# yimin-pan/hair-gs

Measured on AMD Instinct MI355X. Metric: train_iters_per_sec, higher is better.
Workload: dtype f32; 1 GPU; north_star: 100000 strand-Gaussians, 32 views @ 1920x1080, 1 view(s)/GPU/optimizer step (1 views/step), RGB+mask+orientation raster fwd+bwd + L1/DSSIM/mask/orientation/smoothness losses + Adam; gaussians=100000, views=32, width=1920, height=1080, parallelism=view-parallel x1, views_per_optimizer_step=1, forward_mode=async-capacity, dispatch=hip-graph replay, optimizer_steps_per_graph_launch=8, adam_in_backward_lanes=True, raster_passes_per_iter=1

## Files before the change

### hair-gs_amd/csrc/hgs_api.hip

```cpp
#include <stdarg.h>
#include <stdio.h>
#include <string.h>

#include "hgs_common.h"
#include "hgs_prologue.h"

static thread_local char g_err[512] = "";

void hgs_set_error(const char* fmt, ...) {
  va_list ap;
  va_start(ap, fmt);
  vsnprintf(g_err, sizeof(g_err), fmt, ap);
  va_end(ap);
}

#include <vector>
namespace {
struct ProfRec { hipEvent_t a, b; int id; };
bool g_prof_on = false;
std::vector<ProfRec> g_prof_log;
std::vector<hipEvent_t> g_prof_pool;
hipEvent_t g_prof_open = nullptr;
int g_prof_open_id = -1;
const char* kKernelNames[HGS_K_COUNT] = {"preprocess_fwd_kernel", "scan_kernel", "scatter_kernel", "sort_tiles_kernel",
                                         "blend_fwd_kernel", "blend_bwd_kernel", "preprocess_bwd_kernel", "dist2_kernels",
                                         "ssim_l1_fwd_kernel", "ssim_l1_bwd_kernel", "strand_fwd_kernel",
                                         "strand_bwd_kernel", "ori_fwd_kernel", "ori_bwd_kernel", "adam_kernel",
                                         "smooth_kernels", "head_tail_kernel", "misc_kernels"};
hipEvent_t prof_event() {
  if (!g_prof_pool.empty()) { hipEvent_t e = g_prof_pool.back(); g_prof_pool.pop_back(); return e; }
  hipEvent_t e = nullptr;
  (void)hipEventCreate(&e);
  return e;
}
}
void hgs_prof_begin(hipStream_t s, int kernel_id) {
  if (!g_prof_on) return;
  g_prof_open = prof_event();
  g_prof_open_id = kernel_id;
  (void)hipEventRecord(g_prof_open, s);
}
void hgs_prof_end(hipStream_t s) {
  if (!g_prof_on || !g_prof_open) return;
  hipEvent_t b = prof_event();
  (void)hipEventRecord(b, s);
  g_prof_log.push_back({g_prof_open, b, g_prof_open_id});
  g_prof_open = nullptr;
}

__global__ __launch_bounds__(256) void hgs_zero_kernel(uint32_t* __restrict__ p, size_t n_words) {
  const size_t stride = (size_t)gridDim.x * 256;
  for (size_t i = (size_t)blockIdx.x * 256 + threadIdx.x; i < n_words; i += stride) p[i] = 0u;
}
int hgs_zero_async(hipStream_t s, void* ptr, size_t bytes) {
  if (bytes == 0) return 0;
  if (((size_t)ptr & 3) || (bytes & 3)) { hgs_set_error("hgs_zero_async: pointer/size must be 4-byte multiples"); return 1; }
  const size_t n = bytes / 4;
  const unsigned blocks = (unsigned)((n + 255) / 256 < 2048 ? (n + 255) / 256 : 2048);
  hipLaunchKernelGGL(hgs_zero_kernel, dim3(blocks), dim3(256), 0, s, (uint32_t*)ptr, n);
  HGS_CHECK_LAUNCH();
  return 0;
}

__global__ __launch_bounds__(256) void select_view_kernel(HgsPrologue p) { hgs_prologue_block(p, blockIdx.x, gridDim.x); }

struct HgsViewQueueArgs { int v[HGS_VIEW_QUEUE_MAX]; };
__global__ void set_view_queue_kernel(int* __restrict__ queue, int n, HgsViewQueueArgs a, float lr, float* __restrict__ lr_slot) {
  if ((int)threadIdx.x < n) queue[threadIdx.x] = a.v[threadIdx.x];
  if (threadIdx.x == 0 && lr_slot) *lr_slot = lr;
}
__global__ void select_view_queued_kernel(const HgsViewTargets* __restrict__ table, int n_views,
                                          const int* __restrict__ view_index, HgsViewTargets* __restrict__ slot,
                                          const float* __restrict__ lr_slot, float* __restrict__ lr_dst) {
  int view = *view_index;
  if (view < 0 || view >= n_views) view = 0;
  const uint32_t* src = (const uint32_t*)(table + view);
  uint32_t* dst = (uint32_t*)slot;
  for (int i = threadIdx.x; i < (int)(sizeof(HgsViewTargets) / 4); i += 64) dst[i] = src[i];
  if (threadIdx.x == 0 && lr_dst && lr_slot) *lr_dst = *lr_slot;
}

__global__ __launch_bounds__(256) void densify_stats_kernel(int P, const int* __restrict__ radii,
                                                            const float* __restrict__ g, int stride,
                                                            float* __restrict__ max_radii, float* __restrict__ accum,
                                                            float* __restrict__ denom) {
  const int i = blockIdx.x * 256 + threadIdx.x;
  if (i >= P) return;
  const int r = radii[i];
  if (r <= 0) return;
  max_radii[i] = fmaxf(max_radii[i], (float)r);
  const float gx = g[(size_t)i * stride], gy = g[(size_t)i * stride + 1];
  accum[i] += sqrtf(gx * gx + gy * gy);
  denom[i] += 1.f;
}

static int check_aligned(const void* p, const char* what) {
  if (!p || ((size_t)p & (HGS_ALIGN - 1))) {
    hgs_set_error("%s must be a non-null %d-byte aligned device pointer", what, HGS_ALIGN);
    return 1;
  }
  return 0;
}

extern "C" {

int hgs_abi_version(void) { return HGS_ABI_VERSION; }
const char* hgs_last_error(void) { return g_err; }

size_t hgs_geom_bytes(int P) { HgsGeom g; return hgs_geom_carve(nullptr, (size_t)(P > 0 ? P : 0), g, nullptr); }
size_t hgs_image_bytes(int W, int H) { HgsImage im; return hgs_image_carve(nullptr, (size_t)W, (size_t)H, im, nullptr); }
size_t hgs_binning_bytes(int R, int channels) {
  if (channels != 3 && channels != 7) return 0;
  HgsBinning b;
  return hgs_binning_carve(nullptr, (size_t)(R > 0 ? R : 0), b, nullptr, channels);
}
size_t hgs_backward_scratch_bytes(int P, int R, int channels) {
  const size_t p = (size_t)(P > 0 ? P : 0), r = (size_t)(R > 0 ? R : 0);
  if (channels == 3) return hgs_align_up(r * HGS_INST_GRAD_FLOATS * sizeof(float)) + HGS_ALIGN;
  if (channels == 7) return hgs_align_up(r * 16 * sizeof(float)) + hgs_align_up(hgs_row_reduce_floats(p, r) * sizeof(float)) + HGS_ALIGN;
  return 0;
}
int hgs_geom_layout(int P, size_t* offsets) { HgsGeom g; hgs_geom_carve(nullptr, (size_t)P, g, offsets); return 0; }
int hgs_image_zero_range(int W, int H, size_t* offset, size_t* bytes) {
  if (W <= 0 || H <= 0 || !offset || !bytes) { hgs_set_error("hgs_image_zero_range: bad arguments"); return 1; }
  HgsImage im;
  hgs_image_carve(nullptr, (size_t)W, (size_t)H, im, nullptr);
  const size_t T = (size_t)((W + HGS_TILE - 1) / HGS_TILE) * ((H + HGS_TILE - 1) / HGS_TILE);
  *offset = (size_t)((char*)im.tile_count - (char*)nullptr);
  *bytes = hgs_image_zero_words(T) * sizeof(uint32_t);
  return 0;
}
int hgs_image_layout(int W, int H, size_t* offsets) { HgsImage im; hgs_image_carve(nullptr, (size_t)W, (size_t)H, im, offsets); return 0; }
int hgs_binning_layout(int R, size_t* offsets) { HgsBinning b; hgs_binning_carve(nullptr, (size_t)R, b, offsets); return 0; }

static_assert(HGS_FUSED_PREPROCESS_MAX_TILES == HGS_FUSED_SCAN_MAX_T, "include/hgs.h states the scatter kernel's scan limit");
struct HairSrc {
  const float* endpoints; const long long* pairs; const float* width; float f; const float* opacity_raw; const float* mask_raw;
  float* xyz; float* scale; float* quat; float* opacity; float* extra4; const HgsStrandFusion* fusion;
  const float* scaling_raw; const float* rotation_raw;
};
static int forward_preprocess_impl(void* stream, int P, int D, int M, int W, int H, const float* means3D, const float* shs,
                                   const float* colors_precomp, const float* opacities, const float* scales,
                                   float scale_modifier, const float* rotations, const float* cov3D_precomp,
                                   const float* viewmatrix, const float* projmatrix, const float* campos, float tan_fovx,
                                   float tan_fovy, int prefiltered, void* geom_buf, void* image_buf, int* radii,
                                   int* num_rendered_host, unsigned int* max_rendered, const HairSrc* hair);

int hgs_forward_preprocess(void* stream, int P, int D, int M, int W, int H, const float* means3D, const float* shs,
                           const float* colors_precomp, const float* opacities, const float* scales,
                           float scale_modifier, const float* rotations, const float* cov3D_precomp,
                           const float* viewmatrix, const float* projmatrix, const float* campos, float tan_fovx,
                           float tan_fovy, int prefiltered, void* geom_buf, void* image_buf, int* radii,
                           int* num_rendered_host, unsigned int* max_rendered) {
  return forward_preprocess_impl(stream, P, D, M, W, H, means3D, shs, colors_precomp, opacities, scales, scale_modifier,
                                 rotations, cov3D_precomp, viewmatrix, projmatrix, campos, tan_fovx, tan_fovy, prefiltered,
                                 geom_buf, image_buf, radii, num_rendered_host, max_rendered, nullptr);
}

int hgs_hair_forward_preprocess(void* stream, int P, int D, int M, int W, int H, const float* endpoints,
                                const long long* endpoint_pairs, const float* width, float dist_to_scale_factor,
                                const float* opacity_raw, const float* mask_raw, const float* shs, float* xyz, float* scale,
                                float* quat, float* opacity, float* extra4, const float* viewmatrix, const float* projmatrix,
                                const float* campos, float tan_fovx, float tan_fovy, int flags, void* geom_buf,
                                void* image_buf, int* radii, unsigned int* max_rendered, const HgsStrandFusion* fusion) {
  if (P > 0 && (!endpoints || !endpoint_pairs || !width || !opacity_raw || !mask_raw || !xyz || !scale || !quat || !opacity ||
                !extra4 || ((size_t)quat & 15) || ((size_t)extra4 & 15))) {
    hgs_set_error("hgs_hair_forward_preprocess: null (or, quat / extra4, not 16-byte aligned) argument");
    return 1;
  }
  if (!max_rendered) { hgs_set_error("hgs_hair_forward_preprocess: capacity mode only (max_rendered must be given)"); return 1; }
  const HairSrc hair = {endpoints, endpoint_pairs, width, dist_to_scale_factor, opacity_raw, mask_raw, xyz, scale, quat, opacity,
                        extra4, fusion, nullptr, nullptr};
  return forward_preprocess_impl(stream, P, D, M, W, H, xyz, shs, nullptr, opacity, scale, 1.f, quat, nullptr, viewmatrix,
                                 projmatrix, campos, tan_fovx, tan_fovy, flags, geom_buf, image_buf, radii, nullptr,
                                 max_rendered, &hair);
}

int hgs_cloud_forward_preprocess(void* stream, int P, int D, int M, int W, int H, const float* means3D, const float* scaling_raw,
                                 const float* rotation_raw, const float* opacity_raw, const float* mask_raw, const float* shs,
                                 float* scale, float* quat, float* opacity, float* extra4, const float* viewmatrix,
                                 const float* projmatrix, const float* campos, float tan_fovx, float tan_fovy, int flags,
                                 void* geom_buf, void* image_buf, int* radii, unsigned int* max_rendered,
                                 const HgsStrandFusion* fusion) {
  if (P > 0 && (!means3D || !scaling_raw || !rotation_raw || !opacity_raw || !mask_raw || !scale || !quat || !opacity || !extra4 ||
                ((size_t)rotation_raw & 15) || ((size_t)quat & 15) || ((size_t)extra4 & 15))) {
    hgs_set_error("hgs_cloud_forward_preprocess: null (or, rotation_raw / quat / extra4, not 16-byte aligned) argument");
    return 1;
  }
  if (!max_rendered) { hgs_set_error("hgs_cloud_forward_preprocess: capacity mode only (max_rendered must be given)"); return 1; }
  const HairSrc cloud = {nullptr, nullptr, nullptr, 0.f, opacity_raw, mask_raw, nullptr, scale, quat, opacity, extra4, fusion,
                         scaling_raw, rotation_raw};
  return forward_preprocess_impl(stream, P, D, M, W, H, means3D, shs, nullptr, opacity, scale, 1.f, quat, nullptr, viewmatrix,
                                 projmatrix, campos, tan_fovx, tan_fovy, flags, geom_buf, image_buf, radii, nullptr,
                                 max_rendered, &cloud);
}

static int forward_preprocess_impl(void* stream, int P, int D, int M, int W, int H, const float* means3D, const float* shs,
                                   const float* colors_precomp, const float* opacities, const float* scales,
                                   float scale_modifier, const float* rotations, const float* cov3D_precomp,
                                   const float* viewmatrix, const float* projmatrix, const float* campos, float tan_fovx,
                                   float tan_fovy, int prefiltered, void* geom_buf, void* image_buf, int* radii,
                                   int* num_rendered_host, unsigned int* max_rendered, const HairSrc* hair) {
  hipStream_t s = (hipStream_t)stream;
  if (P < 0 || W <= 0 || H <= 0) { hgs_set_error("bad sizes P=%d W=%d H=%d", P, W, H); return 1; }
  if ((size_t)((W + HGS_TILE - 1) / HGS_TILE) * ((H + HGS_TILE - 1) / HGS_TILE) > HGS_MAX_TILES) { hgs_set_error("%dx%d: more than 2^24 tiles", W, H); return 1; }
  if ((unsigned)P > HGS_MAX_GAUSSIANS) { hgs_set_error("P=%d: at most 2^28 Gaussians per pass (instance key layout)", P); return 1; }
  if (D < 0 || D > 3) { hgs_set_error("sh degree %d unsupported (0..3)", D); return 1; }
  if (check_aligned(image_buf, "image_buf")) return 1;
  HgsImage im;
  hgs_image_carve((char*)image_buf, (size_t)W, (size_t)H, im, nullptr);
  const int T = ((W + HGS_TILE - 1) / HGS_TILE) * ((H + HGS_TILE - 1) / HGS_TILE);
  if (!(prefiltered & HGS_IMAGE_PREZEROED) &&
      hgs_zero_async(s, im.tile_count, hgs_image_zero_words((size_t)T) * sizeof(uint32_t))) return 1;
  const HgsPrologue* rider = (hair && hair->fusion && hair->fusion->prologue.table) ? &hair->fusion->prologue : nullptr;
  if (rider && (!rider->slot || rider->view < 0 || ((size_t)rider->zero_ptr & 3) || (rider->zero_bytes & 3) ||
                (rider->zero_bytes && !rider->zero_ptr))) {
    hgs_set_error("hgs_hair/cloud_forward_preprocess: bad prologue group");
    return 1;
  }
  if (hair && T > HGS_FUSED_SCAN_MAX_T) {
    hgs_set_error("hgs_hair_forward_preprocess: %d tiles, at most %d (the tile counters are cleared by the scatter kernel's scan)", T, HGS_FUSED_SCAN_MAX_T);
    return 1;
  }
  if (P == 0 && rider &&
      hgs_iteration_prologue(stream, rider->table, rider->view, rider->slot, rider->lr, rider->lr_dst, rider->zero_ptr, rider->zero_bytes,
                             rider->adam_prep)) return 1;
  if (P == 0) {
    HgsGeom none = {};
    if (hgs_launch_scan(s, 0, T, none, im, nullptr)) return 1;
    if (num_rendered_host) { HGS_CHECK_HIP(hipStreamSynchronize(s)); *num_rendered_host = 0; }
    return 0;
  }
  if (check_aligned(geom_buf, "geom_buf")) return 1;
  if (!means3D || !opacities || !viewmatrix || !projmatrix || !campos || !radii) { hgs_set_error("null required input"); return 1; }
  if ((shs == nullptr) == (colors_precomp == nullptr)) { hgs_set_error("provide exactly one of shs / colors_precomp"); return 1; }
  if (((scales == nullptr) || (rotations == nullptr)) == (cov3D_precomp == nullptr)) {
    hgs_set_error("provide exactly one of (scales, rotations) / cov3D_precomp"); return 1;
  }
  if (shs && M < (D + 1) * (D + 1)) { hgs_set_error("M=%d SH coefficients < (D+1)^2 for D=%d", M, D); return 1; }
  HgsGeom g;
  hgs_geom_carve((char*)geom_buf, (size_t)P, g, nullptr);
  HgsFwdArgs a;
  a.P = P; a.D = D; a.M = M; a.W = W; a.H = H;
  a.means3D = means3D; a.shs = shs; a.colors_precomp = colors_precomp; a.opacities = opacities; a.scales = scales;
  a.rotations = rotations; a.cov3D_precomp = cov3D_precomp; a.viewmatrix = viewmatrix; a.projmatrix = projmatrix;
  a.campos = campos; a.scale_modifier = scale_modifier; a.tan_fovx = tan_fovx; a.tan_fovy = tan_fovy;
  a.prefiltered = prefiltered & 1;
  a.tile_cull = (prefiltered & HGS_TILE_CULL) ? 1 : 0;
  a.row_runs = (prefiltered & HGS_COUNT_ROW_RUNS) ? 1 : 0;
  const bool fused_scan = !num_rendered_host && max_rendered && T <= HGS_FUSED_SCAN_MAX_T && P <= HGS_FUSED_SCAN_MAX_P;
  a.fused_scan_ptr = fused_scan ? (unsigned long long)(size_t)max_rendered : 0ull;
  if (hair) {
    if (!fused_scan) { hgs_set_error("hgs_hair_forward_preprocess: the scan must be the scatter kernel's (sizes beyond its limits)"); return 1; }
    HgsStrandFusion fu = hair->fusion ? *hair->fusion : HgsStrandFusion{};
    if (!(fu.smooth_pairs && fu.n_smooth > 0 && fu.smooth_partials)) fu.n_smooth = 0;
    if (hair->scaling_raw) {
      if (hgs_launch_cloud_preprocess_fwd(s, a, g, im, radii, hair->scaling_raw, hair->rotation_raw, hair->opacity_raw,
                                          hair->mask_raw, hair->scale, hair->quat, hair->opacity, hair->extra4, fu.prologue)) return 1;
    } else if (hgs_launch_hair_preprocess_fwd(s, a, g, im, radii, hair->endpoints, hair->pairs, hair->width, hair->f,
                                              hair->opacity_raw, hair->mask_raw, hair->xyz, hair->scale, hair->quat,
                                              hair->opacity, hair->extra4, fu)) return 1;
  } else if (hgs_launch_preprocess_fwd(s, a, g, im, radii)) return 1;
  if (!fused_scan && hgs_launch_scan(s, P, T, g, im, max_rendered, a.row_runs)) return 1;
  if (num_rendered_host) {
    uint32_t r = 0;
    HGS_CHECK_HIP(hipMemcpyAsync(&r, im.status, sizeof(uint32_t), hipMemcpyDeviceToHost, s));
    HGS_CHECK_HIP(hipStreamSynchronize(s));
    *num_rendered_host = (int)r;
  }
  return 0;
}

int hgs_forward_render(void* stream, int P, int W, int H, int R_capacity, int n_extra, int flags, const float* bg,
                       const float* colors_precomp, const float* extra, void* geom_buf, void* binning_buf, void* image_buf,
                       float* out_color) {
  hipStream_t s = (hipStream_t)stream;
  if (check_aligned(image_buf, "image_buf")) return 1;
  if (!bg || !out_color) { hgs_set_error("null bg/out_color"); return 1; }
  if (n_extra != 0 && n_extra != 4) { hgs_set_error("n_extra must be 0 or 4 (got %d)", n_extra); return 1; }
  if (n_extra && P > 0 && (!extra || ((size_t)extra & 15))) { hgs_set_error("extra colours must be a 16-byte aligned [P,4] array"); return 1; }
  if ((flags & HGS_RECORDS_PACKED) && (flags & HGS_RECORDS_LAZY)) { hgs_set_error("HGS_RECORDS_PACKED and HGS_RECORDS_LAZY exclude each other"); return 1; }
  const int channels = 3 + n_extra;
  HgsImage im;
  hgs_image_carve((char*)image_buf, (size_t)W, (size_t)H, im, nullptr);
  HgsGeom g = {};
  HgsBinning b = {};
  if (P > 0) {
    if (check_aligned(geom_buf, "geom_buf")) return 1;
    hgs_geom_carve((char*)geom_buf, (size_t)P, g, nullptr);
    if (R_capacity > 0) {
      if (check_aligned(binning_buf, "binning_buf")) return 1;
      hgs_binning_carve((char*)binning_buf, (size_t)R_capacity, b, nullptr, channels);
      b.grec = g.grec;
      const long long tiles = (long long)((W + HGS_TILE - 1) / HGS_TILE) * ((H + HGS_TILE - 1) / HGS_TILE);
      b.lazy = (flags & HGS_RECORDS_LAZY) ? 1 : (flags & HGS_RECORDS_PACKED) ? 0 : ((long long)R_capacity >= (long long)HGS_LAZY_MIN_MEAN_LIST * tiles ? 1 : 0);
    }
    const float* feat = colors_precomp ? colors_precomp : g.rgb;
    if (hgs_launch_scatter(s, P, W, H, R_capacity > 0 ? R_capacity : 0, feat, extra, n_extra, g, im, b)) return 1;
  }
  if (hgs_launch_sort_tiles(s, W, H, R_capacity > 0 ? R_capacity : 0, n_extra, g, im, b)) return 1;
  return hgs_launch_blend_fwd(s, W, H, R_capacity > 0 ? R_capacity : 0, channels, bg, im, b, out_color);
}

#define HGS_RR_AUTO_RATIO 8

static int backward_impl(void* stream, int P, int D, int M, int R, int W, int H, int n_extra, int flags, const float* bg,
                         const float* means3D, const float* shs, const float* colors_precomp, const float* scales,
                         float scale_modifier, const float* rotations, const float* cov3D_precomp, const float* viewmatrix,
                         const float* projmatrix, const float* campos, float tan_fovx, float tan_fovy, const int* radii,
                         const void* geom_buf, const void* binning_buf, const void* image_buf,
                         const float* const* dL_dpix_planes, void* scratch, float* dL_dextra, float* dL_dmeans2D, float* dL_dconic,
                         float* dL_dopacity, float* dL_dcolors, float* dL_dmeans3D, float* dL_dcov3D, float* dL_dsh,
                         float* dL_dscales, float* dL_drotations, const HgsParamBackward* pb) {
  hipStream_t s = (hipStream_t)stream;
  if (n_extra != 0 && n_extra != 4) { hgs_set_error("n_extra must be 0 or 4 (got %d)", n_extra); return 1; }
  if ((flags & HGS_ROWS_INLINE) && (flags & HGS_ROWS_REDUCE)) { hgs_set_error("HGS_ROWS_INLINE and HGS_ROWS_REDUCE exclude each other"); return 1; }
  if (P == 0) return 0;
  if (check_aligned(geom_buf, "geom_buf") || check_aligned(image_buf, "image_buf")) return 1;
  if (!dL_dpix_planes || !radii || !means3D || !viewmatrix || !projmatrix || !campos) { hgs_set_error("null required input"); return 1; }
  for (int k = 0; k < 3 + n_extra; k++)
    if (!dL_dpix_planes[k]) { hgs_set_error("null dL_dpix plane %d", k); return 1; }
  if (!pb && (!dL_dmeans2D || !dL_dconic || !dL_dopacity || !dL_dcolors || !dL_dmeans3D || !dL_dcov3D || !dL_dscales ||
              !dL_drotations || (n_extra && !dL_dextra))) { hgs_set_error("null gradient output"); return 1; }
  if (shs && !dL_dsh) { hgs_set_error("null gradient output"); return 1; }
  const int channels = 3 + n_extra;
  HgsGeom g;
  HgsImage im;
  HgsBinning b = {};
  hgs_geom_carve((char*)geom_buf, (size_t)P, g, nullptr);
  hgs_image_carve((char*)image_buf, (size_t)W, (size_t)H, im, nullptr);
  float* inst_grad = nullptr;
  const bool reduce_rows = n_extra && R > 0 &&
                           ((flags & HGS_ROWS_REDUCE) || (!(flags & HGS_ROWS_INLINE) && (long long)R >= (long long)HGS_RR_AUTO_RATIO * P));
  if (R > 0) {
    if (check_aligned(binning_buf, "binning_buf") || check_aligned(scratch, "scratch")) return 1;
    hgs_binning_carve((char*)binning_buf, (size_t)R, b, nullptr, channels);
    b.grec = g.grec;
    inst_grad = (float*)scratch;
    if (hgs_launch_blend_bwd(s, W, H, R, channels, bg, im, b, dL_dpix_planes, inst_grad, reduce_rows ? 1 : 0)) return 1;
  }
  float *row_sums = nullptr, *row_partials = nullptr;
  if (reduce_rows) {
    row_sums = (float*)((char*)scratch + hgs_align_up((size_t)R * 16 * sizeof(float)));
    row_partials = row_sums + (size_t)P * 16;
    if (hgs_launch_row_reduce(s, P, R, inst_grad, im.status, row_sums, row_partials)) return 1;
  }
  HgsBwdArgs a;
  a.P = P; a.D = D; a.M = M; a.W = W; a.H = H;
  a.means3D = means3D; a.shs = shs; a.colors_precomp = colors_precomp; a.scales = scales; a.rotations = rotations;
  a.cov3D_precomp = cov3D_precomp; a.viewmatrix = viewmatrix; a.projmatrix = projmatrix; a.campos = campos;
  a.scale_modifier = scale_modifier; a.tan_fovx = tan_fovx; a.tan_fovy = tan_fovy; a.radii = radii;
  a.dL_dmeans2D = dL_dmeans2D; a.dL_dconic = dL_dconic; a.dL_dopacity = dL_dopacity; a.dL_dcolors = dL_dcolors;
  a.dL_dmeans3D = dL_dmeans3D; a.dL_dcov3D = dL_dcov3D; a.dL_dsh = dL_dsh; a.dL_dscales = dL_dscales;
  a.dL_drotations = dL_drotations;
  a.n_extra = n_extra; a.dL_dextra = dL_dextra;
  a.row_sums = row_sums; a.row_partials = row_partials;
  return hgs_launch_preprocess_bwd(s, a, g, b, inst_grad, R, im.status, pb);
}

size_t hgs_param_backward_bytes(void) { return sizeof(HgsParamBackward); }
size_t hgs_adam_prep_bytes(void) { return sizeof(HgsAdamPrep); }
size_t hgs_adam_inline_bytes(void) { return sizeof(HgsAdamInline); }
static int check_adam_inline(const HgsAdamInline& a, int n_slots, const char* who) {
  for (int k = 0; k < 6; k++) {
    const HgsAdamSlot& sl = a.slot[k];
    if (!sl.p) continue;
    if (k >= n_slots || !sl.m || !sl.v || !sl.coef) { hgs_set_error("%s: incomplete Adam slot %d", who, k); return 1; }
  }
  return 0;
}
int hgs_backward_multi_params(void* stream, int P, int D, int M, int R, int W, int H, int flags, const float* bg7,
                              const float* means3D, const float* shs, const float* scales, const float* rotations,
                              const float* viewmatrix, const float* projmatrix, const float* campos, float tan_fovx,
                              float tan_fovy, const int* radii, const void* geom_buf, const void* binning_buf, const void* image_buf,
                              const float* const* dL_dpix_planes7, void* scratch, float* dL_dsh, const HgsParamBackward* pb) {
  if (!pb || (pb->kind != HGS_PARAMS_HAIR && pb->kind != HGS_PARAMS_CLOUD)) { hgs_set_error("hgs_backward_multi_params: params->kind must be HGS_PARAMS_HAIR or HGS_PARAMS_CLOUD"); return 1; }
  if (P == 0 && pb->head_tail.out) { hgs_set_error("hgs_backward_multi_params: a deferred loss-head tail needs a launch (P > 0)"); return 1; }
  if (P == 0) return 0;
  if (!shs || !scales || !rotations || !dL_dsh) { hgs_set_error("hgs_backward_multi_params: SH colours and (scales, rotations) are required"); return 1; }
  if (!pb->extra4 || !pb->d_opacity_raw || !pb->d_mask_raw || ((size_t)pb->extra4 & 15)) { hgs_set_error("hgs_backward_multi_params: null (or, extra4, unaligned) argument in params"); return 1; }
  if ((pb->max_radii2D || pb->grad_accum || pb->denom) && !(pb->max_radii2D && pb->grad_accum && pb->denom)) {
    hgs_set_error("hgs_backward_multi_params: incomplete statistics group");
    return 1;
  }
  if (pb->kind == HGS_PARAMS_HAIR) {
    if (!pb->endpoints || !pb->endpoint_pairs || !pb->seg_contrib || !pb->d_width || ((size_t)pb->seg_contrib & 15)) {
      hgs_set_error("hgs_backward_multi_params: null (or, seg_contrib, unaligned) hair argument"); return 1;
    }
    if (pb->head_tail.out) { hgs_set_error("hgs_backward_multi_params: the strand model's deferred tail rides in hgs_hair_endpoint_gather"); return 1; }
  } else if (!pb->rotation_raw || !pb->d_means3D || !pb->d_scaling_raw || !pb->d_rotation_raw || ((size_t)pb->rotation_raw & 15) ||
             ((size_t)pb->d_rotation_raw & 15)) {
    hgs_set_error("hgs_backward_multi_params: null (or, rotation_raw / d_rotation_raw, unaligned) cloud argument"); return 1;
  }
  if (check_adam_inline(pb->adam, pb->kind == HGS_PARAMS_HAIR ? 4 : 6, "hgs_backward_multi_params")) return 1;
  HgsParamBackward p = *pb;
  return backward_impl(stream, P, D, M, R, W, H, 4, flags, bg7, means3D, shs, nullptr, scales, 1.f, rotations, nullptr, viewmatrix,
                       projmatrix, campos, tan_fovx, tan_fovy, radii, geom_buf, binning_buf, image_buf, dL_dpix_planes7, scratch,
                       nullptr, p.dL_dmeans2D_rgb, nullptr, nullptr, nullptr, nullptr, nullptr, dL_dsh, nullptr, nullptr, &p);
}

int hgs_backward(void* stream, int P, int D, int M, int R, int W, int H, int n_extra, int flags, const float* bg,
                 const float* means3D, const float* shs, const float* colors_precomp, const float* scales, float scale_modifier,
                 const float* rotations, const float* cov3D_precomp, const float* viewmatrix, const float* projmatrix,
                 const float* campos, float tan_fovx, float tan_fovy, const int* radii, const void* geom_buf,
                 const void* binning_buf, const void* image_buf, const float* const* dL_dpix_planes, void* scratch,
                 float* dL_dextra, float* dL_dmeans2D, float* dL_dconic, float* dL_dopacity, float* dL_dcolors,
                 float* dL_dmeans3D, float* dL_dcov3D, float* dL_dsh, float* dL_dscales, float* dL_drotations) {
  return backward_impl(stream, P, D, M, R, W, H, n_extra, flags, bg, means3D, shs, colors_precomp, scales, scale_modifier,
                       rotations, cov3D_precomp, viewmatrix, projmatrix, campos, tan_fovx, tan_fovy, radii, geom_buf, binning_buf,
                       image_buf, dL_dpix_planes, scratch, dL_dextra, dL_dmeans2D, dL_dconic, dL_dopacity, dL_dcolors,
                       dL_dmeans3D, dL_dcov3D, dL_dsh, dL_dscales, dL_drotations, nullptr);
}

int hgs_mark_visible(void* stream, int P, const float* means3D, const float* viewmatrix, const float* projmatrix,
                     uint8_t* present) {
  (void)projmatrix;
  if (P == 0) return 0;
  if (!means3D || !viewmatrix || !present) { hgs_set_error("null input"); return 1; }
  return hgs_launch_mark_visible((hipStream_t)stream, P, means3D, viewmatrix, present);
}

__global__ void hgs_empty_kernel() {}
static float g_prof_bracket_ms = -1.f;
static int prof_calibrate() {
  hipEvent_t a = nullptr, b = nullptr;
  HGS_CHECK_HIP(hipEventCreate(&a));
  HGS_CHECK_HIP(hipEventCreate(&b));
  float best1 = 1e9f, best2 = 1e9f;
  for (int rep = 0; rep < 24; rep++) {
    for (int n = 1; n <= 2; n++) {
      HGS_CHECK_HIP(hipDeviceSynchronize());
      HGS_CHECK_HIP(hipEventRecord(a, nullptr));
      for (int k = 0; k < n; k++) hipLaunchKernelGGL(hgs_empty_kernel, dim3(1), dim3(64), 0, nullptr);
      HGS_CHECK_HIP(hipEventRecord(b, nullptr));
      HGS_CHECK_HIP(hipEventSynchronize(b));
      float ms = 0.f;
      HGS_CHECK_HIP(hipEventElapsedTime(&ms, a, b));
      if (rep >= 4) { if (n == 1) best1 = ms < best1 ? ms : best1; else best2 = ms < best2 ? ms : best2; }
    }
  }
  (void)hipEventDestroy(a);
  (void)hipEventDestroy(b);
  const float kernel = best2 - best1 > 0.f ? best2 - best1 : 0.f;
  g_prof_bracket_ms = best1 - kernel > 0.f ? best1 - kernel : 0.f;
  return 0;
}
int hgs_prof_enable(int on) {
  if (on && g_prof_bracket_ms < 0.f && prof_calibrate()) return 1;
  g_prof_on = on != 0;
  return 0;
}
double hgs_prof_bracket_overhead_ms(void) { return g_prof_bracket_ms < 0.f ? 0.0 : (double)g_prof_bracket_ms; }
const char* hgs_prof_kernel_name(int id) { return (id >= 0 && id < HGS_K_COUNT) ? kKernelNames[id] : ""; }
int hgs_prof_collect(double* total_ms, long long* launches) {
  for (auto& r : g_prof_log) {
    HGS_CHECK_HIP(hipEventSynchronize(r.b));
    float ms = 0.f;
    HGS_CHECK_HIP(hipEventElapsedTime(&ms, r.a, r.b));
    ms -= g_prof_bracket_ms > 0.f ? g_prof_bracket_ms : 0.f;
    if (ms < 0.f) ms = 0.f;
    if (total_ms) total_ms[r.id] += ms;
    if (launches) launches[r.id] += 1;
    g_prof_pool.push_back(r.a);
    g_prof_pool.push_back(r.b);
  }
  g_prof_log.clear();
  return 0;
}

size_t hgs_dist2_scratch_bytes(int P) { return hgs_dist2_scratch(P > 0 ? P : 0); }
int hgs_dist2(void* stream, int P, const float* points, float* out, void* scratch, size_t scratch_bytes) {
  if (P == 0) return 0;
  if (!points || !out) { hgs_set_error("null input"); return 1; }
  return hgs_launch_dist2((hipStream_t)stream, P, points, out, scratch, scratch_bytes);
}

size_t hgs_view_targets_bytes(void) { return sizeof(HgsViewTargets); }
size_t hgs_head_params_bytes(void) { return sizeof(HgsHeadParams); }
size_t hgs_strand_fusion_bytes(void) { return sizeof(HgsStrandFusion); }

int hgs_iteration_prologue(void* stream, const HgsViewTargets* table, int view, HgsViewTargets* slot, float lr, float* lr_dst,
                           void* zero_ptr, size_t zero_bytes, const HgsAdamPrep* adam_prep) {
  if (!table || !slot || view < 0) { hgs_set_error("hgs_iteration_prologue: bad arguments"); return 1; }
  if (((size_t)zero_ptr & 3) || (zero_bytes & 3) || (zero_bytes && !zero_ptr)) { hgs_set_error("hgs_iteration_prologue: zero range must be 4-byte multiples"); return 1; }
  hipStream_t s = (hipStream_t)stream;
  const HgsPrologue p = {table, view, slot, lr, lr_dst, zero_ptr, zero_bytes, adam_prep};
  {
    HgsProfScope _prof(s, HGS_K_MISC);
    hipLaunchKernelGGL(select_view_kernel, dim3(hgs_prologue_blocks(zero_bytes / 4)), dim3(256), 0, s, p);
  }
  HGS_CHECK_LAUNCH();
  return 0;
}
int hgs_select_view(void* stream, const HgsViewTargets* table, int view, HgsViewTargets* slot, float lr, float* lr_dst) {
  return hgs_iteration_prologue(stream, table, view, slot, lr, lr_dst, nullptr, 0, nullptr);
}

int hgs_graph_find_prologues(void* graph, int max_nodes, void** nodes_out, float* lr_out, int* n_out) {
  if (!graph || !nodes_out || !n_out || max_nodes < 1) { hgs_set_error("hgs_graph_find_prologues: bad arguments"); return 1; }
  size_t n = 0;
  HGS_CHECK_HIP(hipGraphGetNodes((hipGraph_t)graph, nullptr, &n));
  std::vector<hipGraphNode_t> nodes(n);
  if (n) HGS_CHECK_HIP(hipGraphGetNodes((hipGraph_t)graph, nodes.data(), &n));
  int count = 0;
  for (size_t i = 0; i < n; i++) {
    hipGraphNodeType t;
    HGS_CHECK_HIP(hipGraphNodeGetType(nodes[i], &t));
    if (t != hipGraphNodeTypeKernel) continue;
    hipKernelNodeParams kp;
    HGS_CHECK_HIP(hipGraphKernelNodeGetParams(nodes[i], &kp));
    int n_params = 1;
    if (kp.func != (void*)select_view_kernel && !hgs_strands_prologue_kernel(kp.func, &n_params) &&
        !hgs_preprocess_prologue_kernel(kp.func, &n_params)) continue;
    if (!kp.kernelParams) continue;
    const HgsPrologue* pro = (const HgsPrologue*)kp.kernelParams[n_params - 1];
    if (!pro->table) continue;
    if (count < max_nodes) {
      nodes_out[count] = (void*)nodes[i];
      if (lr_out) lr_out[count] = pro->lr;
    }
    count++;
  }
  *n_out = count;
  if (count > max_nodes) { hgs_set_error("hgs_graph_find_prologues: the graph holds %d prologue launches (room for %d)", count, max_nodes); return 1; }
  return 0;
}
int hgs_graph_find_prologue(void* graph, void** node_out) {
  int n = 0;
  if (!node_out) { hgs_set_error("hgs_graph_find_prologue: bad arguments"); return 1; }
  if (hgs_graph_find_prologues(graph, 1, node_out, nullptr, &n)) return 1;
  if (n != 1) { hgs_set_error("hgs_graph_find_prologue: the graph holds %d prologue launches (need exactly 1)", n); return 1; }
  return 0;
}
int hgs_graph_set_prologue(void* graph_exec, void* node, const HgsViewTargets* table, int view, HgsViewTargets* slot, float lr,
                           float* lr_dst, void* zero_ptr, size_t zero_bytes) {
  if (!graph_exec || !node || !table || !slot || view < 0) { hgs_set_error("hgs_graph_set_prologue: bad arguments"); return 1; }
  hipKernelNodeParams kp;
  HGS_CHECK_HIP(hipGraphKernelNodeGetParams((hipGraphNode_t)node, &kp));
  int n_params = 1;
  if (kp.func != (void*)select_view_kernel && !hgs_strands_prologue_kernel(kp.func, &n_params) &&
      !hgs_preprocess_prologue_kernel(kp.func, &n_params)) {
    hgs_set_error("hgs_graph_set_prologue: not a prologue node");
    return 1;
  }
  if (((const HgsPrologue*)kp.kernelParams[n_params - 1])->zero_bytes != zero_bytes) {
    hgs_set_error("hgs_graph_set_prologue: the zero range differs from the captured one");
    return 1;
  }
  HgsPrologue p = {table, view, slot, lr, lr_dst, zero_ptr, zero_bytes,
                   ((const HgsPrologue*)kp.kernelParams[n_params - 1])->adam_prep};
  void* args[32];
  for (int i = 0; i < n_params - 1; i++) args[i] = kp.kernelParams[i];
  args[n_params - 1] = &p;
  kp.kernelParams = args;
  kp.extra = nullptr;
  HGS_CHECK_HIP(hipGraphExecKernelNodeSetParams((hipGraphExec_t)graph_exec, (hipGraphNode_t)node, &kp));
  return 0;
}

int hgs_set_view_queue(void* stream, int* queue, int n, const int* views_host, float lr, float* lr_slot) {
  if (!queue || !views_host || n < 1 || n > HGS_VIEW_QUEUE_MAX) { hgs_set_error("hgs_set_view_queue: bad arguments (1 <= n <= %d)", HGS_VIEW_QUEUE_MAX); return 1; }
  HgsViewQueueArgs a = {};
  for (int i = 0; i < n; i++) a.v[i] = views_host[i];
  hipStream_t s = (hipStream_t)stream;
  {
    HgsProfScope _prof(s, HGS_K_MISC);
    hipLaunchKernelGGL(set_view_queue_kernel, dim3(1), dim3(64), 0, s, queue, n, a, lr, lr_slot);
  }
  HGS_CHECK_LAUNCH();
  return 0;
}

int hgs_select_view_queued(void* stream, const HgsViewTargets* table, int n_views, const int* view_index,
                           HgsViewTargets* slot, const float* lr_slot, float* lr_dst) {
  if (!table || !slot || !view_index || n_views < 1) { hgs_set_error("hgs_select_view_queued: bad arguments"); return 1; }
  hipStream_t s = (hipStream_t)stream;
  {
    HgsProfScope _prof(s, HGS_K_MISC);
    hipLaunchKernelGGL(select_view_queued_kernel, dim3(1), dim3(64), 0, s, table, n_views, view_index, slot, lr_slot, lr_dst);
  }
  HGS_CHECK_LAUNCH();
  return 0;
}

int hgs_densify_stats(void* stream, int P, const int* radii, const float* dL_dmean2D, int stride, float* max_radii2D,
                      float* xyz_gradient_accum, float* denom) {
  if (P <= 0) return 0;
  if (!radii || !dL_dmean2D || stride < 2 || !max_radii2D || !xyz_gradient_accum || !denom) {
    hgs_set_error("hgs_densify_stats: bad arguments");
    return 1;
  }
  hipStream_t s = (hipStream_t)stream;
  {
    HgsProfScope _prof(s, HGS_K_MISC);
    hipLaunchKernelGGL(densify_stats_kernel, dim3((P + 255) / 256), dim3(256), 0, s, P, radii, dL_dmean2D, stride, max_radii2D,
                       xyz_gradient_accum, denom);
  }
  HGS_CHECK_LAUNCH();
  return 0;
}

}
```

### hair-gs_amd/csrc/hgs_losses.hip

```cpp
#include "hgs_common.h"
#include "hgs_head_tail.h"

namespace {

#define LT 32
#define HALO 5
#define TILE (LT + 2 * HALO)
#define HP (LT + 1)

struct SsimWin { float w[11]; };

#ifndef HGS_SSIM_TRACE
#define HGS_SSIM_TRACE 0
#endif
#if HGS_SSIM_TRACE
__device__ unsigned long long* g_ssim_trace[2] = {nullptr, nullptr};
struct SsimTrace {
  unsigned long long* buf; unsigned long long last, acc[8], first; unsigned nb = 0, nf = 0;
  __device__ SsimTrace(int which) : buf(g_ssim_trace[which] ? g_ssim_trace[which] + 16 * (size_t)blockIdx.x : nullptr) {
    for (int i = 0; i < 8; i++) acc[i] = 0;
    first = last = __builtin_amdgcn_s_memrealtime();
  }
  __device__ void phase(int k) { const unsigned long long n = __builtin_amdgcn_s_memrealtime(); acc[k] += n - last; last = n; }
  __device__ void block(bool filtered) { nb++; nf += filtered ? 1u : 0u; }
  __device__ ~SsimTrace() {
    if (buf && threadIdx.x == 0) {
      buf[0] = nb; buf[1] = nf;
      for (int i = 0; i < 8; i++) buf[2 + i] = acc[i];
      buf[10] = first; buf[11] = __builtin_amdgcn_s_memrealtime();
    }
  }
};
#else
struct SsimTrace {
  __device__ SsimTrace(int) {}
  __device__ void phase(int) {}
  __device__ void block(bool) {}
};
#endif

__device__ __forceinline__ float block_sum(float v, float* red4) {
#pragma unroll
  for (int d = 32; d >= 1; d >>= 1) v += __shfl_xor(v, d, 64);
  __syncthreads();
  if ((threadIdx.x & 63) == 0) red4[threadIdx.x >> 6] = v;
  __syncthreads();
  return (red4[0] + red4[1]) + (red4[2] + red4[3]);
}
__device__ __forceinline__ void block_sum2(float& a, float& b, float* red) {
#pragma unroll
  for (int d = 32; d >= 1; d >>= 1) { a += __shfl_xor(a, d, 64); b += __shfl_xor(b, d, 64); }
  __syncthreads();
  if ((threadIdx.x & 63) == 0) { red[threadIdx.x >> 6] = a; red[4 + (threadIdx.x >> 6)] = b; }
  __syncthreads();
  a = (red[0] + red[1]) + (red[2] + red[3]);
  b = (red[4] + red[5]) + (red[6] + red[7]);
}

#define XOFF 8
#define TW (LT + 2 * XOFF)
#define TPW (TW + 1)
template <int NP, typename PtrOf>
__device__ __forceinline__ void load_tiles(float (*t)[TILE][TPW], int H, int W, int bx0, int by0, PtrOf plane_ptr) {
  if ((W & 3) == 0) {
    for (int i = threadIdx.x; i < TILE * (TW / 4); i += 256) {
      const int r = i / (TW / 4), c4 = (i - r * (TW / 4)) * 4;
      const int y = by0 + r - HALO, x = bx0 - XOFF + c4;
      const bool in = (unsigned)y < (unsigned)H && x >= 0 && x < W;
#pragma unroll
      for (int p = 0; p < NP; p++) {
        float4 v = make_float4(0.f, 0.f, 0.f, 0.f);
        if (in) v = hgs_load4(plane_ptr(p) + (size_t)y * W + x);
        t[p][r][c4] = v.x; t[p][r][c4 + 1] = v.y; t[p][r][c4 + 2] = v.z; t[p][r][c4 + 3] = v.w;
      }
    }
  } else {
    for (int i = threadIdx.x; i < TILE * TW; i += 256) {
      const int r = i / TW, c = i - r * TW;
      const int y = by0 + r - HALO, x = bx0 - XOFF + c;
      const bool in = (unsigned)y < (unsigned)H && (unsigned)x < (unsigned)W;
#pragma unroll
      for (int p = 0; p < NP; p++) t[p][r][c] = in ? plane_ptr(p)[(size_t)y * W + x] : 0.f;
    }
  }
}

template <int NQ, int NO, typename F>
__device__ __forceinline__ void row_item(const SsimWin& win, float (*hz)[TILE][HP], F load, int r, int x0) {
  float acc[NQ][NO];
#pragma unroll
  for (int q = 0; q < NQ; q++)
#pragma unroll
    for (int o = 0; o < NO; o++) acc[q][o] = 0.f;
#pragma unroll
  for (int k = 0; k < NO + 10; k++) {
    float val[NQ];
    load(r, x0 + k, val);
#pragma unroll
    for (int o = 0; o < NO; o++) {
      const int tap = k - o;
      if (tap >= 0 && tap < 11) {
#pragma unroll
        for (int q = 0; q < NQ; q++) acc[q][o] += win.w[tap] * val[q];
      }
    }
  }
#pragma unroll
  for (int q = 0; q < NQ; q++)
#pragma unroll
    for (int o = 0; o < NO; o++) hz[q][r][x0 + o] = acc[q][o];
}
template <int NQ, typename F>
__device__ __forceinline__ void row_pass(const SsimWin& win, float (*hz)[TILE][HP], F load) {
  constexpr int ITEMS = TILE * (LT / 4);
  static_assert(ITEMS > 256 && 2 * (ITEMS - 256) <= 256, "row-pass split assumes 256 < items <= 384");
  {
    const int it = threadIdx.x;
    const int r = it / (LT / 4), x0 = (it - r * (LT / 4)) * 4;
    row_item<NQ, 4>(win, hz, load, r, x0);
  }
  if (threadIdx.x < 2 * (ITEMS - 256)) {
    const int it = 256 + (threadIdx.x >> 1);
    const int r = it / (LT / 4), x0 = (it - r * (LT / 4)) * 4 + 2 * (threadIdx.x & 1);
    row_item<NQ, 2>(win, hz, load, r, x0);
  }
}
template <int NQ, int NO, typename F>
__device__ __forceinline__ void row_item_regs(const SsimWin& win, F load, int r, int x0, float (*acc)[NO]) {
#pragma unroll
  for (int q = 0; q < NQ; q++)
#pragma unroll
    for (int o = 0; o < NO; o++) acc[q][o] = 0.f;
#pragma unroll
  for (int k = 0; k < NO + 10; k++) {
    float val[NQ];
    load(r, x0 + k, val);
#pragma unroll
    for (int o = 0; o < NO; o++) {
      const int tap = k - o;
      if (tap >= 0 && tap < 11) {
#pragma unroll
        for (int q = 0; q < NQ; q++) acc[q][o] += win.w[tap] * val[q];
      }
    }
  }
}
template <int NQ> struct RowRegs { float a4[NQ][4], a2[NQ][2]; };
template <int NQ, typename F>
__device__ __forceinline__ void row_pass_regs(const SsimWin& win, F load, RowRegs<NQ>& rr) {
  constexpr int ITEMS = TILE * (LT / 4);
  {
    const int it = threadIdx.x;
    const int r = it / (LT / 4), x0 = (it - r * (LT / 4)) * 4;
    row_item_regs<NQ, 4>(win, load, r, x0, rr.a4);
  }
  if (threadIdx.x < 2 * (ITEMS - 256)) {
    const int it = 256 + (threadIdx.x >> 1);
    const int r = it / (LT / 4), x0 = (it - r * (LT / 4)) * 4 + 2 * (threadIdx.x & 1);
    row_item_regs<NQ, 2>(win, load, r, x0, rr.a2);
  }
}
template <int NQ>
__device__ __forceinline__ void row_store(float (*hz)[TILE][HP], const RowRegs<NQ>& rr) {
  constexpr int ITEMS = TILE * (LT / 4);
  {
    const int it = threadIdx.x;
    const int r = it / (LT / 4), x0 = (it - r * (LT / 4)) * 4;
#pragma unroll
    for (int q = 0; q < NQ; q++)
#pragma unroll
      for (int o = 0; o < 4; o++) hz[q][r][x0 + o] = rr.a4[q][o];
  }
  if (threadIdx.x < 2 * (ITEMS - 256)) {
    const int it = 256 + (threadIdx.x >> 1);
    const int r = it / (LT / 4), x0 = (it - r * (LT / 4)) * 4 + 2 * (threadIdx.x & 1);
#pragma unroll
    for (int q = 0; q < NQ; q++)
#pragma unroll
      for (int o = 0; o < 2; o++) hz[q][r][x0 + o] = rr.a2[q][o];
  }
}
template <int NQ>
__device__ __forceinline__ void col_pass(const SsimWin& win, float (*hz)[TILE][HP], int lx, int y0, float (*out)[4]) {
#pragma unroll
  for (int q = 0; q < NQ; q++)
#pragma unroll
    for (int o = 0; o < 4; o++) out[q][o] = 0.f;
#pragma unroll
  for (int k = 0; k < 14; k++) {
#pragma unroll
    for (int q = 0; q < NQ; q++) {
      const float v = hz[q][y0 + k][lx];
#pragma unroll
      for (int o = 0; o < 4; o++) {
        const int tap = k - o;
        if (tap >= 0 && tap < 11) out[q][o] += win.w[tap] * v;
      }
    }
  }
}

struct SsimGrid { int nbx, nby, C, chunk, total, sub; };
struct SsimBlock { int c, bx0, by0, logical; };
__device__ __forceinline__ void ssim_block_decode(const SsimGrid& gd, int logical, SsimBlock& o) {
  o.logical = logical;
  const int per = gd.nbx * gd.nby;
  o.c = logical / per;
  const int r = logical - o.c * per;
  const int by = r / gd.nbx;
  o.by0 = by * LT;
  o.bx0 = (r - by * gd.nbx) * LT;
}
__device__ __forceinline__ bool ssim_block(const SsimGrid& gd, int j, SsimBlock& o) {
  const int q = j / gd.sub;
  o.logical = (q * 8 + (int)(blockIdx.x & 7)) * gd.sub + (j - q * gd.sub);
  if (j >= gd.chunk || o.logical >= gd.total) return false;
  const int per = gd.nbx * gd.nby;
  o.c = o.logical / per;
  const int r = o.logical - o.c * per;
  const int by = r / gd.nbx;
  o.by0 = by * LT;
  o.bx0 = (r - by * gd.nbx) * LT;
  return true;
}
#ifndef SSIM_SUBBANDS
#define SSIM_SUBBANDS 32
#endif
static inline SsimGrid ssim_grid(int C, int H, int W) {
  SsimGrid gd;
  gd.nbx = (W + LT - 1) / LT; gd.nby = (H + LT - 1) / LT; gd.C = C;
  gd.total = gd.nbx * gd.nby * C;
  gd.sub = (gd.total + SSIM_SUBBANDS - 1) / SSIM_SUBBANDS;
  gd.chunk = gd.sub * (SSIM_SUBBANDS / 8);
  return gd;
}
#ifndef HGS_SSIM_FWD_WAVES
#define HGS_SSIM_FWD_WAVES 5
#endif
#ifndef HGS_SSIM_FWD_ALIAS
#define HGS_SSIM_FWD_ALIAS 1
#endif
#define SSIM_FWD_WG_PER_XCD (32 * HGS_SSIM_FWD_WAVES)
#ifndef HGS_SSIM_BWD_WAVES
#define HGS_SSIM_BWD_WAVES 4
#endif
#define SSIM_BWD_WG_PER_XCD (32 * HGS_SSIM_BWD_WAVES)
static inline unsigned ssim_grid_size(const SsimGrid& gd, int per_xcd) { return 8u * (unsigned)(gd.chunk < per_xcd ? gd.chunk : per_xcd); }

#define ST_F4 (TILE * (TW / 4))
template <int NP> struct TileStage { float4 v[NP][2]; unsigned in; };
template <int NP, typename PtrOf>
__device__ __forceinline__ void stage_load(TileStage<NP>& st, int H, int W, int bx0, int by0, PtrOf plane_ptr) {
  st.in = 0u;
#pragma unroll
  for (int u = 0; u < 2; u++) {
    const int i = threadIdx.x + 256 * u;
    const int r = i / (TW / 4), c4 = (i - r * (TW / 4)) * 4;
    const int y = by0 + r - HALO, x = bx0 - XOFF + c4;
    const bool in = i < ST_F4 && (unsigned)y < (unsigned)H && x >= 0 && x < W;
    st.in |= in ? 1u << u : 0u;
    const size_t at = (size_t)min(max(y, 0), H - 1) * W + min(max(x, 0), W - 4);
#pragma unroll
    for (int p = 0; p < NP; p++) st.v[p][u] = hgs_load4(plane_ptr(p) + at);
  }
}
template <int NP>
__device__ __forceinline__ void stage_store(const TileStage<NP>& st, float (*t)[TILE][TPW]) {
#pragma unroll
  for (int u = 0; u < 2; u++) {
    const int i = threadIdx.x + 256 * u;
    if (i < ST_F4) {
      const int r = i / (TW / 4), c4 = (i - r * (TW / 4)) * 4;
      const bool in = (st.in >> u) & 1u;
#pragma unroll
      for (int p = 0; p < NP; p++) {
        const float4 v = st.v[p][u];
        t[p][r][c4] = in ? v.x : 0.f; t[p][r][c4 + 1] = in ? v.y : 0.f; t[p][r][c4 + 2] = in ? v.z : 0.f; t[p][r][c4 + 3] = in ? v.w : 0.f;
      }
    }
  }
}

__device__ __forceinline__ void ssim_zero_maps(float* m) {
  float C1 = 0.01f * 0.01f, C2 = 0.03f * 0.03f;
  asm volatile("" : "+v"(C1), "+v"(C2));
  const float iB1 = __builtin_amdgcn_rcpf(C1), iB2 = __builtin_amdgcn_rcpf(C2);
  const float inv = iB1 * iB2;
  const float S = (C1 * C2) * inv;
  m[0] = 0.f; m[1] = -S * iB2; m[2] = 2.f * C1 * inv;
}

__global__ __launch_bounds__(256) __attribute__((amdgpu_waves_per_eu(HGS_SSIM_FWD_WAVES, HGS_SSIM_FWD_WAVES))) void ssim_l1_fwd_kernel(int H, int W, SsimGrid gd, SsimWin win, const float* __restrict__ img1,
                                                          const float* __restrict__ img2_, const HgsViewTargets* __restrict__ tgt,
                                                          float* __restrict__ dmap, float* __restrict__ partials,
                                                          unsigned char* __restrict__ zero_flags) {
#if HGS_SSIM_FWD_ALIAS
  __shared__ float smem[4 * TILE * HP];
  static_assert(4 * TILE * HP >= 2 * TILE * TPW, "filtered planes cover the tile");
  float (*t)[TILE][TPW] = (float (*)[TILE][TPW])smem;
  float (*hz)[TILE][HP] = (float (*)[TILE][HP])smem;
#else
  __shared__ float t[2][TILE][TPW];
  __shared__ float hz[4][TILE][HP];
#endif
  __shared__ float red[8];
  const size_t plane = (size_t)H * W, cp = (size_t)gd.C * plane;
  const HGS_GLOBAL float* im1 = hgs_global(img1);
  const HGS_GLOBAL float* im2 = tgt ? hgs_global(tgt->image) : hgs_global(img2_);
  const bool fast = (W & 3) == 0;
  const int nwg = gridDim.x >> 3;
  int j = blockIdx.x >> 3;
  SsimBlock bk, nx;
  bool have = ssim_block(gd, j, bk);
  TileStage<2> st;
  if (fast && have) stage_load<2>(st, H, W, bk.bx0, bk.by0, [&](int p) { return (p == 0 ? im1 : im2) + bk.c * plane; });
  const int lx = threadIdx.x & (LT - 1), y0 = (threadIdx.x >> 5) * 4;
  SsimTrace tr(0);
  while (have) {
    tr.phase(7);
    int nz = 1;
#if HGS_SSIM_FWD_ALIAS
    __syncthreads();
#endif
    if (fast) {
      stage_store<2>(st, t);
      if (zero_flags) {
        nz = 0;
#pragma unroll
        for (int p = 0; p < 2; p++)
#pragma unroll
          for (int u = 0; u < 2; u++)
            if ((st.in >> u) & 1u) nz |= (st.v[p][u].x != 0.f) | (st.v[p][u].y != 0.f) | (st.v[p][u].z != 0.f) | (st.v[p][u].w != 0.f);
      }
    } else {
      load_tiles<2>(t, H, W, bk.bx0, bk.by0, [&](int p) { return (p == 0 ? im1 : im2) + bk.c * plane; });
    }
    const int any_nz = __syncthreads_or(nz);
    tr.phase(0);
    tr.block(any_nz != 0);
    j += nwg;
    const bool have_next = ssim_block(gd, j, nx);
    if (fast && have_next) stage_load<2>(st, H, W, nx.bx0, nx.by0, [&](int p) { return (p == 0 ? im1 : im2) + nx.c * plane; });
    float f[4][4];
#if HGS_SSIM_FWD_ALIAS
    float l1c[4];
#pragma unroll
    for (int o = 0; o < 4; o++) l1c[o] = fabsf(t[0][y0 + o + HALO][lx + XOFF] - t[1][y0 + o + HALO][lx + XOFF]);
#endif
    if (any_nz) {
#if HGS_SSIM_FWD_ALIAS
      {
        RowRegs<4> rr;
        row_pass_regs<4>(win, [&](int r, int x, float* v) {
          const float a = t[0][r][x + XOFF - HALO], b = t[1][r][x + XOFF - HALO];
          v[0] = a; v[1] = b; v[2] = a * a + b * b; v[3] = a * b;
        }, rr);
        __syncthreads();
        row_store<4>(hz, rr);
      }
#else
      row_pass<4>(win, hz, [&](int r, int x, float* v) {
        const float a = t[0][r][x + XOFF - HALO], b = t[1][r][x + XOFF - HALO];
        v[0] = a; v[1] = b; v[2] = a * a + b * b; v[3] = a * b;
      });
#endif
      __syncthreads();
      tr.phase(1);
      col_pass<4>(win, hz, lx, y0, f);
      tr.phase(2);
    } else {
#pragma unroll
      for (int q = 0; q < 4; q++)
#pragma unroll
        for (int o = 0; o < 4; o++) f[q][o] = 0.f;
    }
    if (zero_flags && threadIdx.x == 0) zero_flags[bk.logical] = any_nz ? 0 : 1;
    const float C1 = 0.01f * 0.01f, C2 = 0.03f * 0.03f;
    const int px = bk.bx0 + lx;
    float ssim_v = 0.f, l1_v = 0.f;
#pragma unroll
    for (int o = 0; o < 4; o++) {
      const int py = bk.by0 + y0 + o;
      if (px < W && py < H) {
        const float mu1 = f[0][o], mu2 = f[1][o];
        const float mu1_sq = mu1 * mu1, mu2_sq = mu2 * mu2, mu12 = mu1 * mu2;
        const float s_sum = f[2][o] - (mu1_sq + mu2_sq), s12 = f[3][o] - mu12;
        const float A1 = 2.f * mu12 + C1, A2 = 2.f * s12 + C2, B1 = mu1_sq + mu2_sq + C1, B2 = s_sum + C2;
        const float iB1 = __builtin_amdgcn_rcpf(B1), iB2 = __builtin_amdgcn_rcpf(B2);
        const float inv = iB1 * iB2;
        const float S = (A1 * A2) * inv;
        ssim_v += S;
#if HGS_SSIM_FWD_ALIAS
        l1_v += l1c[o];
#else
        l1_v += fabsf(t[0][y0 + o + HALO][lx + XOFF] - t[1][y0 + o + HALO][lx + XOFF]);
#endif
        if (any_nz) {
          const size_t oo = bk.c * plane + (size_t)py * W + px;
          dmap[oo] = 2.f * mu2 * (A2 - A1) * inv - S * (2.f * mu1 * iB1 - 2.f * mu1 * iB2);
          dmap[cp + oo] = -S * iB2;
          dmap[2 * cp + oo] = 2.f * A1 * inv;
        }
      }
    }
    tr.phase(3);
    block_sum2(ssim_v, l1_v, red);
    if (threadIdx.x == 0) {
      partials[2 * (size_t)bk.logical] = ssim_v;
      partials[2 * (size_t)bk.logical + 1] = l1_v;
    }
    tr.phase(4);
    bk = nx;
    have = have_next;
  }
}


__global__ __launch_bounds__(256) __attribute__((amdgpu_waves_per_eu(HGS_SSIM_BWD_WAVES, HGS_SSIM_BWD_WAVES))) void ssim_l1_bwd_kernel(int H, int W, SsimGrid gd, SsimWin win, const float* __restrict__ img1,
                                                          const float* __restrict__ img2_, const HgsViewTargets* __restrict__ tgt,
                                                          const float* __restrict__ dmap,
                                                          const float* __restrict__ g_ssim_mean,
                                                          const float* __restrict__ g_l1_mean, const float* __restrict__ go,
                                                          float* __restrict__ dimg1, float* __restrict__ zero_buf,
                                                          int zero_n, const int* __restrict__ lists,
                                                          const unsigned char* __restrict__ zero_flags) {
  for (int i = blockIdx.x * 256 + threadIdx.x; i < zero_n; i += gridDim.x * 256) zero_buf[i] = 0.f;
#ifndef HGS_SSIM_BWD_ALIAS
#define HGS_SSIM_BWD_ALIAS 1
#endif
#if HGS_SSIM_BWD_ALIAS
  __shared__ float smem[3 * TILE * TPW];
  float (*t)[TILE][TPW] = (float (*)[TILE][TPW])smem;
  float (*hz)[TILE][HP] = (float (*)[TILE][HP])smem;
#else
  __shared__ float t[3][TILE][TPW];
  __shared__ float hz[3][TILE][HP];
#endif
  const HGS_GLOBAL float* im1 = hgs_global(img1);
  const HGS_GLOBAL float* im2 = tgt ? hgs_global(tgt->image) : hgs_global(img2_);
  const HGS_GLOBAL float* dmg = hgs_global(dmap);
  const size_t plane = (size_t)H * W, cp = (size_t)gd.C * plane;
  const float n = 1.f / (float)((size_t)gd.C * plane);
  const float up = go ? *go : 1.f;
  const float gs = *g_ssim_mean * up * n, gl = *g_l1_mean * up * n;
  const bool fast = (W & 3) == 0;
  const int nwg = gridDim.x >> 3;
  const int lx = threadIdx.x & (LT - 1), y0 = (threadIdx.x >> 5) * 4;
  int j = blockIdx.x >> 3;
  SsimBlock bk, nx;
  const int xcd = blockIdx.x & 7;
  int lo = 0, hi = 0;
  const int* work = nullptr;
  if (lists) {
    const int n_work = lists[0], n_skip = lists[1];
    work = lists + 4;
    const int* skipped = work + gd.total;
    lo = (int)(((long long)n_work * xcd) >> 3);
    hi = (int)(((long long)n_work * (xcd + 1)) >> 3);
    for (int q = blockIdx.x; q < n_skip; q += gridDim.x) {
      SsimBlock z;
      ssim_block_decode(gd, skipped[q], z);
      const int px = z.bx0 + lx;
#pragma unroll
      for (int o = 0; o < 4; o++) {
        const int py = z.by0 + y0 + o;
        if (px < W && py < H) dimg1[z.c * plane + (size_t)py * W + px] = 0.f;
      }
    }
  }
  const int jstep = nwg, j0 = j;
  int idv = 0, idbase = 0;
  auto refill = [&](int k0) {
    idbase = k0;
    const int jj = j0 + (k0 + (int)(threadIdx.x & 63)) * jstep;
    idv = (work && lo + jj < hi) ? work[lo + jj] : 0;
  };
  int kblk = 0;
  auto block_at = [&](int jj, int k, SsimBlock& o) {
    if (!work) return ssim_block(gd, jj, o);
    if (lo + jj >= hi) return false;
    if (k - idbase >= 64) refill(k);
    ssim_block_decode(gd, __builtin_amdgcn_readlane(idv, k - idbase), o);
    return true;
  };
  refill(0);
  bool have = block_at(j, 0, bk);
  TileStage<3> st;
  float x1[4], x2[4];
  auto centre = [&](const SsimBlock& q) {
#pragma unroll
    for (int o = 0; o < 4; o++) {
      const int px = q.bx0 + lx, py = q.by0 + y0 + o;
      x1[o] = 0.f; x2[o] = 0.f;
      if (px < W && py < H) { const size_t oo = q.c * plane + (size_t)py * W + px; x1[o] = im1[oo]; x2[o] = im2[oo]; }
    }
  };
  float zm[3];
  ssim_zero_maps(zm);
  unsigned char fl[2] = {0, 0};
  auto stage = [&](const SsimBlock& q) {
    stage_load<3>(st, H, W, q.bx0, q.by0, [&](int p) { return dmg + p * cp + q.c * plane; });
    if (!zero_flags) return;
    const int per = gd.nbx * gd.nby;
#pragma unroll
    for (int u = 0; u < 2; u++) {
      const int i = threadIdx.x + 256 * u;
      const int r = i / (TW / 4), c4 = (i - r * (TW / 4)) * 4;
      const int y = q.by0 + r - HALO, x = q.bx0 - XOFF + c4;
      fl[u] = zero_flags[q.c * per + (min(max(y, 0), H - 1) / LT) * gd.nbx + min(max(x, 0), W - 4) / LT];
    }
  };
  auto apply_flags = [&]() {
#pragma unroll
    for (int u = 0; u < 2; u++)
      if (fl[u] && ((st.in >> u) & 1u)) {
#pragma unroll
        for (int p = 0; p < 3; p++) st.v[p][u] = make_float4(zm[p], zm[p], zm[p], zm[p]);
      }
  };
  if (have && fast) stage(bk);
  SsimTrace tr(1);
  while (have) {
    tr.phase(7);
    tr.block(true);
#if HGS_SSIM_BWD_ALIAS
    __syncthreads();
#endif
    if (fast) { apply_flags(); stage_store<3>(st, t); }
    else load_tiles<3>(t, H, W, bk.bx0, bk.by0, [&](int p) { return dmg + p * cp + bk.c * plane; });
    __syncthreads();
    tr.phase(0);
    centre(bk);
    j += nwg;
    kblk++;
    const bool have_next = block_at(j, kblk, nx);
    if (have_next && fast) stage(nx);
#if HGS_SSIM_BWD_ALIAS
    {
      RowRegs<3> rr;
      row_pass_regs<3>(win, [&](int r, int x, float* v) {
        v[0] = t[0][r][x + XOFF - HALO]; v[1] = t[1][r][x + XOFF - HALO]; v[2] = t[2][r][x + XOFF - HALO];
      }, rr);
      __syncthreads();
      row_store<3>(hz, rr);
    }
#else
    row_pass<3>(win, hz, [&](int r, int x, float* v) {
      v[0] = t[0][r][x + XOFF - HALO]; v[1] = t[1][r][x + XOFF - HALO]; v[2] = t[2][r][x + XOFF - HALO];
    });
#endif
    __syncthreads();
    tr.phase(1);
    float f[3][4];
    col_pass<3>(win, hz, lx, y0, f);
    tr.phase(2);
    const int px = bk.bx0 + lx;
#pragma unroll
    for (int o = 0; o < 4; o++) {
      const int py = bk.by0 + y0 + o;
      if (px < W && py < H) {
        const size_t oo = bk.c * plane + (size_t)py * W + px;
        const float d = x1[o] - x2[o];
        const float sgn = d > 0.f ? 1.f : (d < 0.f ? -1.f : 0.f);
        dimg1[oo] = gs * (f[0][o] + 2.f * x1[o] * f[1][o] + x2[o] * f[2][o]) + gl * sgn;
      }
    }
    tr.phase(4);
    bk = nx;
    have = have_next;
  }
}

struct OriParams { const float* view; float bg0, bg1, bg2; float min_val; int has_mask; };

__device__ __forceinline__ bool ori_pixel(const OriParams& p, float o0, float o1, float o2, float& px, float& py, float& r,
                                          float& n, float& x, float& y, float& yq, float& theta) {
  const float* v = p.view;
  px = o0 * v[0] + o1 * v[4] + o2 * v[8];
  py = o0 * v[1] + o1 * v[5] + o2 * v[9];
  r = sqrtf(px * px + py * py);
  n = r + p.min_val;
  const float in = __builtin_amdgcn_rcpf(n);
  x = px * in;
  y = py * in;
  yq = y < p.min_val ? y + p.min_val : y;
  theta = atan2f(x, yq);
  if (theta < 0.f) theta += 3.14159265358979323846f;
  return true;
}

__global__ __launch_bounds__(256) void ori_fwd_kernel(int N, OriParams p, const float* __restrict__ omap,
                                                      const float* __restrict__ gt, const float* __restrict__ conf,
                                                      const uint8_t* __restrict__ mask, float* __restrict__ partials) {
  __shared__ float red[4];
  const int i = blockIdx.x * 256 + threadIdx.x;
  float s = 0.f, cnt = 0.f;
  if (i < N) {
    const float o0 = omap[i], o1 = omap[(size_t)N + i], o2 = omap[2 * (size_t)N + i];
    const bool m = p.has_mask ? mask[i] != 0 : (o0 != p.bg0 || o1 != p.bg1 || o2 != p.bg2);
    if (m) {
      float px, py, r, n, x, y, yq, th;
      ori_pixel(p, o0, o1, o2, px, py, r, n, x, y, yq, th);
      const float hp = 1.57079632679489661923f;
      const float diff = hp - fabsf(fabsf(th - gt[i]) - hp);
      s = diff * conf[i];
      cnt = 1.f;
    }
  }
  const float bs = block_sum(s, red);
  const float bc = block_sum(cnt, red);
  if (threadIdx.x == 0) { partials[2 * blockIdx.x] = bs; partials[2 * blockIdx.x + 1] = bc; }
}

__global__ __launch_bounds__(256) void ori_bwd_kernel(int N, OriParams p, const float* __restrict__ omap,
                                                      const float* __restrict__ gt, const float* __restrict__ conf,
                                                      const uint8_t* __restrict__ mask, const float* __restrict__ g_loss,
                                                      const float* __restrict__ mask_count, float* __restrict__ d_omap) {
  const int i = blockIdx.x * 256 + threadIdx.x;
  if (i >= N) return;
  const float o0 = omap[i], o1 = omap[(size_t)N + i], o2 = omap[2 * (size_t)N + i];
  const bool m = p.has_mask ? mask[i] != 0 : (o0 != p.bg0 || o1 != p.bg1 || o2 != p.bg2);
  float g0 = 0.f, g1 = 0.f, g2 = 0.f;
  if (m) {
    float px, py, r, n, x, y, yq, th;
    ori_pixel(p, o0, o1, o2, px, py, r, n, x, y, yq, th);
    {
      const float hp = 1.57079632679489661923f;
      const float e = th - gt[i];
      const float u = fabsf(e) - hp;
      const float sg = (u > 0.f ? 1.f : (u < 0.f ? -1.f : 0.f)) * (e > 0.f ? 1.f : (e < 0.f ? -1.f : 0.f));
      const float dth = -sg * conf[i] * (*g_loss) / (*mask_count);
      const float den = x * x + yq * yq;
      const float dx = dth * (yq / den), dy = dth * (-x / den);
      const float inv_n = 1.f / n, inv_n2 = inv_n * inv_n, ir = r > 0.f ? 1.f / r : 0.f;
      const float dn = -(dx * px + dy * py) * inv_n2;
      const float dpx = dx * inv_n + dn * px * ir, dpy = dy * inv_n + dn * py * ir;
      const float* v = p.view;
      g0 = dpx * v[0] + dpy * v[1]; g1 = dpx * v[4] + dpy * v[5]; g2 = dpx * v[8] + dpy * v[9];
    }
  }
  d_omap[i] = g0; d_omap[(size_t)N + i] = g1; d_omap[2 * (size_t)N + i] = g2;
}


struct HeadFlags { int bce, ori; };

__device__ __forceinline__ void ori_pixel_grad(const OriParams& p, float px, float py, float r, float n, float x, float yq,
                                               float th, float gt, float conf, float scale, float& g0, float& g1, float& g2) {
  const float hp = 1.57079632679489661923f;
  const float e = th - gt;
  const float u = fabsf(e) - hp;
  const float sg = (u > 0.f ? 1.f : (u < 0.f ? -1.f : 0.f)) * (e > 0.f ? 1.f : (e < 0.f ? -1.f : 0.f));
  const float dth = -sg * conf * scale;
  const float iden = __builtin_amdgcn_rcpf(x * x + yq * yq);
  const float dx = dth * (yq * iden), dy = dth * (-x * iden);
  const float inv_n = __builtin_amdgcn_rcpf(n), inv_n2 = inv_n * inv_n, ir = r > 0.f ? __builtin_amdgcn_rcpf(r) : 0.f;
  const float dn = -(dx * px + dy * py) * inv_n2;
  const float dpx = dx * inv_n + dn * px * ir, dpy = dy * inv_n + dn * py * ir;
  const float* v = p.view;
  g0 = dpx * v[0] + dpy * v[1]; g1 = dpx * v[4] + dpy * v[5]; g2 = dpx * v[8] + dpy * v[9];
}

struct HeadReduce { int nb_ssim, nb_pix, nb_smooth; float inv_chw, inv_hw; float l_dssim, l_mask, l_ori, l_smooth; int bce, ori; };

__device__ __forceinline__ void head_part1(const HeadReduce& h, const float* __restrict__ p_ssim,
                                           const float* __restrict__ p_smooth, float* __restrict__ out) {
  __shared__ float red4[4][4];
  float sv[4] = {0.f, 0.f, 0.f, 0.f};
  const float2* ps = (const float2*)p_ssim;
  const float2* pm = (const float2*)p_smooth;
  float2 w[4];
#pragma unroll
  for (int u = 0; u < 4; u++) {
    const int i = u * 256 + (int)threadIdx.x;
    w[u] = h.nb_smooth > 0 ? pm[min(i, h.nb_smooth - 1)] : make_float2(0.f, 0.f);
  }
  for (int base = 0; base < h.nb_ssim; base += 12 * 256) {
    float2 v[12];
#pragma unroll
    for (int u = 0; u < 12; u++) v[u] = ps[min(base + u * 256 + (int)threadIdx.x, h.nb_ssim - 1)];
#pragma unroll
    for (int u = 0; u < 12; u++)
      if (base + u * 256 + (int)threadIdx.x < h.nb_ssim) { sv[0] += v[u].x; sv[1] += v[u].y; }
  }
#pragma unroll
  for (int u = 0; u < 4; u++)
    if (u * 256 + (int)threadIdx.x < h.nb_smooth) { sv[2] += w[u].x; sv[3] += w[u].y; }
  for (int i = 4 * 256 + (int)threadIdx.x; i < h.nb_smooth; i += 256) { sv[2] += pm[i].x; sv[3] += pm[i].y; }
#pragma unroll
  for (int q = 0; q < 4; q++)
#pragma unroll
    for (int d = 32; d >= 1; d >>= 1) sv[q] += __shfl_xor(sv[q], d, 64);
  if ((threadIdx.x & 63) == 0)
#pragma unroll
    for (int q = 0; q < 4; q++) red4[q][threadIdx.x >> 6] = sv[q];
  __syncthreads();
  if (threadIdx.x != 0) return;
#pragma unroll
  for (int q = 0; q < 4; q++) sv[q] = (red4[q][0] + red4[q][1]) + (red4[q][2] + red4[q][3]);
  const float ssim_s = sv[0], l1_s = sv[1], sm_s = sv[2], sm_c = sv[3];
  const float l1 = l1_s * h.inv_chw, dssim = 1.f - ssim_s * h.inv_chw;
  const float w_l1 = fmaxf(0.f, 1.f - h.l_dssim);
  out[HGS_HEAD_TOTAL] = out[HGS_HEAD_TOTAL_FWD] = fmaf(h.l_dssim, dssim, w_l1 * l1);
  out[HGS_HEAD_L1] = l1; out[HGS_HEAD_DSSIM] = dssim;
  out[HGS_HEAD_SMOOTH] = h.nb_smooth > 0 ? sm_s / fmaxf(sm_c, 1.f) : 0.f;
  out[HGS_HEAD_SMOOTH_COUNT] = sm_c;
  out[HGS_HEAD_G_SSIM] = -h.l_dssim; out[HGS_HEAD_G_L1] = w_l1;
  out[HGS_HEAD_G_MASK] = h.bce ? h.l_mask * h.inv_hw : 0.f;
  out[HGS_HEAD_G_ORI] = h.ori ? h.l_ori : 0.f;
  out[HGS_HEAD_G_SMOOTH] = h.nb_smooth > 0 ? h.l_smooth : 0.f;
}

#ifndef HGS_PIX_TRACE
#define HGS_PIX_TRACE 0
#endif
#define HEAD_MAX_TILES 45056
#define HEAD_MAX_FLAGGED 32768
static_assert(HEAD_MAX_FLAGGED % (32 * 256) == 0, "whole 32-block words per thread of the list builder");
static_assert(HEAD_MAX_TILES % 32 == 0 && HEAD_MAX_TILES >= 4 * (HEAD_MAX_FLAGGED / 3), "2 x 2 tiles per block of 3 channels");
__device__ __forceinline__ unsigned even_bits(unsigned long long x) {
  x &= 0x5555555555555555ull;
  x = (x | (x >> 1)) & 0x3333333333333333ull;
  x = (x | (x >> 2)) & 0x0F0F0F0F0F0F0F0Full;
  x = (x | (x >> 4)) & 0x00FF00FF00FF00FFull;
  x = (x | (x >> 8)) & 0x0000FFFF0000FFFFull;
  x = (x | (x >> 16)) & 0x00000000FFFFFFFFull;
  return (unsigned)x;
}

__device__ __forceinline__ void build_block_lists(const SsimGrid& gd, const unsigned char* __restrict__ zero_flags,
                                                  int* __restrict__ lists, const unsigned int* __restrict__ tile_used,
                                                  int tiles_x, int tiles_y) {
#if HGS_PIX_TRACE
#define BL_STAMP(k) do { __syncthreads(); if (threadIdx.x == 0) lists[4 + 2 * gd.total + 7 + (k)] = (int)(unsigned)__builtin_amdgcn_s_memrealtime(); } while (0)
#else
#define BL_STAMP(k) do { } while (0)
#endif
  constexpr int WPT = HEAD_MAX_FLAGGED / 32 / 256;
  __shared__ unsigned zbits[HEAD_MAX_FLAGGED / 32];
  __shared__ unsigned tbits[HEAD_MAX_TILES / 32 + 2];
  __shared__ int wsum[4], zsum[4];
  const int total = gd.total, nwords = (total + 31) >> 5;
  const unsigned* zf = (const unsigned*)zero_flags;
  const int n_tiles = tiles_x * tiles_y;
  const uint4* tu4 = (const uint4*)tile_used;
  const int n4 = (n_tiles + 3) >> 2;
  uint4 tv[8];
  if (tile_used) {
    for (int i = threadIdx.x; i < HEAD_MAX_TILES / 32 + 2; i += 256) tbits[i] = 0u;
#pragma unroll
    for (int u = 0; u < 8; u++) tv[u] = tu4[min(u * 256 + (int)threadIdx.x, n4 - 1)];
  }
#pragma unroll 1
  for (int w = threadIdx.x; w < nwords; w += 256) {
    unsigned v[8];
#pragma unroll
    for (int u = 0; u < 8; u++) v[u] = zf[8 * w + u];
    unsigned bits = 0;
#pragma unroll
    for (int u = 0; u < 8; u++) bits |= (((v[u] & 0x01010101u) * 0x00204081u) >> 21 & 0xFu) << (4 * u);
    const int left = total - 32 * w;
    if (left < 32) bits |= ~((1u << left) - 1u);
    zbits[w] = bits;
  }
  if (tile_used) {
    __syncthreads();
    for (int base = 0; base < n4; base += 8 * 256) {
      if (base) {
#pragma unroll
        for (int u = 0; u < 8; u++) tv[u] = tu4[min(base + u * 256 + (int)threadIdx.x, n4 - 1)];
      }
#pragma unroll
      for (int u = 0; u < 8; u++) {
        const int q = base + u * 256 + (int)threadIdx.x, t = 4 * q;
        if (q < n4) {
          unsigned nib = (tv[u].x != 0u ? 1u : 0u) | (tv[u].y != 0u ? 2u : 0u) | (tv[u].z != 0u ? 4u : 0u) | (tv[u].w != 0u ? 8u : 0u);
          if (t + 4 > n_tiles) nib &= (1u << (n_tiles - t)) - 1u;
          if (nib) atomicOr(&tbits[t >> 5], nib << (t & 31));
        }
      }
    }
  }
  __syncthreads();
  BL_STAMP(0);
  const int per = gd.nbx * gd.nby, nbx = gd.nbx;
  auto zfetch = [&](int start) -> unsigned {
    const int wi = start >> 5, sh = start & 31;
    const unsigned lo = (wi >= 0 && wi < nwords) ? zbits[wi] : 0xFFFFFFFFu;
    const unsigned hi = (wi + 1 >= 0 && wi + 1 < nwords) ? zbits[wi + 1] : 0xFFFFFFFFu;
    return sh ? (lo >> sh) | (hi << (32 - sh)) : lo;
  };
  auto tfetch = [&](int start) -> unsigned long long {
    const int wi = start >> 5, sh = start & 31;
    const unsigned long long a = tbits[wi], b = tbits[wi + 1], c = tbits[wi + 2];
    const unsigned long long lo = a | (b << 32);
    return sh ? (lo >> sh) | (c << (64 - sh)) : lo;
  };
  unsigned work_w[WPT], fill_w[WPT];
  int cnt = 0, cnt_z = 0;
  const int wpt = (nwords + 255) >> 8, w_first = threadIdx.x * wpt;
#pragma unroll
  for (int q = 0; q < WPT; q++) {
    work_w[q] = 0u; fill_w[q] = 0u;
    const int w = w_first + q;
    if (q >= wpt || w >= nwords) continue;
    const int b0 = 32 * w;
    unsigned L = 0u, R = 0u, T = 0u, Bm = 0u, used = tile_used ? 0u : 0xFFFFFFFFu;
    int r = b0 % per, by = r / nbx, bx = r - by * nbx;
    for (int i = 0; i < 32;) {
      const int len = min(32 - i, nbx - bx);
      const unsigned seg = (len == 32 ? 0xFFFFFFFFu : ((1u << len) - 1u)) << i;
      if (bx == 0) L |= 1u << i;
      if (bx + len == nbx) R |= 1u << (i + len - 1);
      if (by == 0) T |= seg;
      if (by == gd.nby - 1) Bm |= seg;
      if (tile_used) {
#pragma unroll
        for (int ty = 0; ty < 2; ty++) {
          const int Y = 2 * by + ty;
          if (Y < tiles_y) {
            unsigned long long v = tfetch(Y * tiles_x + 2 * bx);
            const int nt = min(2 * len, tiles_x - 2 * bx);
            if (nt < 64) v &= (1ull << nt) - 1ull;
            used |= (even_bits(v | (v >> 1)) & (len == 32 ? 0xFFFFFFFFu : ((1u << len) - 1u))) << i;
          }
        }
      }
      i += len; bx = 0;
      if (++by == gd.nby) by = 0;
    }
    auto H = [&](int start) { return zfetch(start) & (zfetch(start - 1) | L) & (zfetch(start + 1) | R); };
    const unsigned zero = H(b0) & (H(b0 - nbx) | T) & (H(b0 + nbx) | Bm);
    const int left = total - b0;
    const unsigned valid = left >= 32 ? 0xFFFFFFFFu : ((1u << left) - 1u);
    work_w[q] = used & ~zero & valid;
    fill_w[q] = used & zero & valid;
    cnt += __popc(work_w[q]); cnt_z += __popc(fill_w[q]);
  }
  BL_STAMP(1);
  int inc = cnt, inc_z = cnt_z;
#pragma unroll
  for (int d = 1; d < 64; d <<= 1) {
    const int v = __shfl_up(inc, d, 64), vz = __shfl_up(inc_z, d, 64);
    if ((int)(threadIdx.x & 63) >= d) { inc += v; inc_z += vz; }
  }
  if ((threadIdx.x & 63) == 63) { wsum[threadIdx.x >> 6] = inc; zsum[threadIdx.x >> 6] = inc_z; }
  __syncthreads();
  int base = 0, all = 0, base_z = 0, all_z = 0;
#pragma unroll
  for (int k = 0; k < 4; k++) {
    const int v = wsum[k], vz = zsum[k];
    if (k < (int)(threadIdx.x >> 6)) { base += v; base_z += vz; }
    all += v; all_z += vz;
  }
  int w = base + inc - cnt, z = base_z + inc_z - cnt_z;
  int* work = lists + 4;
  int* skipped = work + total;
  BL_STAMP(2);
#pragma unroll
  for (int q = 0; q < WPT; q++) {
    unsigned mw = work_w[q], mz = fill_w[q];
    const int id0 = 32 * (w_first + q);
    while (mw) { const int bpos = __ffs(mw) - 1; mw &= mw - 1u; work[w++] = id0 + bpos; }
    while (mz) { const int bpos = __ffs(mz) - 1; mz &= mz - 1u; skipped[z++] = id0 + bpos; }
  }
  if (threadIdx.x == 0) { lists[0] = all; lists[1] = all_z; }
}

#define PIX_SIDE_WGS 2
__global__ __launch_bounds__(256) __attribute__((amdgpu_waves_per_eu(8))) void pix_fwd_kernel(int N, HeadFlags fl, float bg0, float bg1, float bg2, float min_val,
                                                      const float* __restrict__ mask_img, const float* __restrict__ omap,
                                                      const HgsViewTargets* __restrict__ tgt, float* __restrict__ partials,
                                                      float g_mask, float g_ori, float* __restrict__ d_unit, SsimGrid gd,
                                                      const unsigned char* __restrict__ zero_flags,
                                                      int* __restrict__ lists, HeadReduce h,
                                                      const float* __restrict__ p_ssim, const float* __restrict__ p_smooth,
                                                      float* __restrict__ out, const unsigned int* __restrict__ tile_used,
                                                      int tiles_x, int tiles_y, int W, float inv_w) {
  __shared__ float red[4];
  if (blockIdx.x < PIX_SIDE_WGS) {
#if HGS_PIX_TRACE
    const unsigned long long t0 = __builtin_amdgcn_s_memrealtime();
#endif
    if (blockIdx.x == 0) { if (lists) build_block_lists(gd, zero_flags, lists, tile_used, tiles_x, tiles_y); }
    else head_part1(h, p_ssim, p_smooth, out);
#if HGS_PIX_TRACE
    __syncthreads();
    if (threadIdx.x == 0 && lists) { lists[4 + 2 * gd.total + 2 * blockIdx.x] = (int)(unsigned)t0; lists[4 + 2 * gd.total + 2 * blockIdx.x + 1] = (int)(unsigned)__builtin_amdgcn_s_memrealtime(); }
#endif
    return;
  }
  const int blk = blockIdx.x - PIX_SIDE_WGS;
  const int i = blk * 256 + threadIdx.x;
  float s = 0.f, cnt = 0.f, b = 0.f;
  if (i < N) {
    const bool has_mask = tgt->mask != nullptr;
    float xm = 0.f, ym = 0.f, o0 = 0.f, o1 = 0.f, o2 = 0.f, gt = 0.f, cf = 0.f;
    unsigned char mk = 0;
    unsigned used = 1u;
    if (fl.bce) { xm = mask_img[i]; ym = hgs_global(tgt->float_mask)[i]; }
    if (fl.ori) {
      o0 = omap[i]; o1 = omap[(size_t)N + i]; o2 = omap[2 * (size_t)N + i];
      gt = hgs_global(tgt->orientation)[i]; cf = hgs_global(tgt->confidence)[i];
      mk = (has_mask ? hgs_global(tgt->mask) : (const HGS_GLOBAL unsigned char*)hgs_global(omap))[i];
    }
    if (d_unit && tile_used) {
      int y = N < (1 << 24) ? (int)(((float)i + 0.5f) * inv_w) : i / W;
      int x = i - y * W;
      if (x < 0) { y--; x += W; } else if (x >= W) { y++; x -= W; }
      static_assert(HGS_TILE == 16, "pixel -> tile by a shift of 4");
      used = tile_used[(y >> 4) * tiles_x + (x >> 4)];
    }
    float gm = 0.f, g0 = 0.f, g1 = 0.f, g2 = 0.f;
    if (fl.bce) {
      const float x = xm, y = ym;
      const float en = __expf(-fabsf(x));
      b = fmaxf(x, 0.f) - x * y + __logf(1.f + en);
      if (d_unit) { const float r1 = __builtin_amdgcn_rcpf(1.f + en); gm = g_mask * ((x >= 0.f ? r1 : en * r1) - y); }
    }
    if (fl.ori) {
      OriParams p;
      p.view = tgt->viewmatrix; p.bg0 = bg0; p.bg1 = bg1; p.bg2 = bg2; p.min_val = min_val; p.has_mask = has_mask;
      const bool m = p.has_mask ? mk != 0 : (o0 != p.bg0 || o1 != p.bg1 || o2 != p.bg2);
      if (m) {
        float px, py, r, n, x, y, yq, th;
        ori_pixel(p, o0, o1, o2, px, py, r, n, x, y, yq, th);
        const float hp = 1.57079632679489661923f;
        s = (hp - fabsf(fabsf(th - gt) - hp)) * cf;
        cnt = 1.f;
        if (d_unit) ori_pixel_grad(p, px, py, r, n, x, yq, th, gt, cf, g_ori / tgt->mask_count, g0, g1, g2);
      }
    }
    if (d_unit && used) {
      d_unit[i] = gm; d_unit[(size_t)N + i] = g0; d_unit[2 * (size_t)N + i] = g1; d_unit[3 * (size_t)N + i] = g2;
    }
  }
  const float bs = block_sum(s, red);
  const float bc = block_sum(cnt, red);
  const float bb = block_sum(b, red);
  if (threadIdx.x == 0) { partials[3 * blk] = bs; partials[3 * blk + 1] = bc; partials[3 * blk + 2] = bb; }
#if HGS_PIX_TRACE
  if (threadIdx.x == 0 && lists && (blk == 0 || blk == (int)gridDim.x - PIX_SIDE_WGS - 1 || blk == 4000))
    lists[4 + 2 * gd.total + 4 + (blk == 0 ? 0 : (blk == 4000 ? 1 : 2))] = (int)(unsigned)__builtin_amdgcn_s_memrealtime();
#endif
}

__global__ __launch_bounds__(256) void pix_bwd_kernel(int N, HeadFlags fl, float bg0, float bg1, float bg2, float min_val,
                                                      const float* __restrict__ mask_img, const float* __restrict__ omap,
                                                      const HgsViewTargets* __restrict__ tgt, const float* __restrict__ out,
                                                      const float* __restrict__ go, float* __restrict__ d_mask_img,
                                                      float* __restrict__ d_omap) {
  const int i = blockIdx.x * 256 + threadIdx.x;
  if (i >= N) return;
  const float up = *go;
  float gm = 0.f;
  if (fl.bce) {
    const float x = mask_img[i], y = hgs_global(tgt->float_mask)[i];
    gm = out[HGS_HEAD_G_MASK] * up * (1.f / (1.f + expf(-x)) - y);
  }
  d_mask_img[i] = gm;
  float g0 = 0.f, g1 = 0.f, g2 = 0.f;
  if (fl.ori) {
    OriParams p;
    p.view = tgt->viewmatrix; p.bg0 = bg0; p.bg1 = bg1; p.bg2 = bg2; p.min_val = min_val; p.has_mask = tgt->mask != nullptr;
    const float o0 = omap[i], o1 = omap[(size_t)N + i], o2 = omap[2 * (size_t)N + i];
    const bool m = p.has_mask ? hgs_global(tgt->mask)[i] != 0 : (o0 != p.bg0 || o1 != p.bg1 || o2 != p.bg2);
    if (m) {
      float px, py, r, n, x, y, yq, th;
      ori_pixel(p, o0, o1, o2, px, py, r, n, x, y, yq, th);
      ori_pixel_grad(p, px, py, r, n, x, yq, th, hgs_global(tgt->orientation)[i], hgs_global(tgt->confidence)[i],
                     (out[HGS_HEAD_G_ORI] * up) / out[HGS_HEAD_ORI_COUNT], g0, g1, g2);
    }
  }
  d_omap[i] = g0; d_omap[(size_t)N + i] = g1; d_omap[2 * (size_t)N + i] = g2;
}


__global__ __launch_bounds__(256) void head_tail_kernel(HgsHeadTail t) { hgs_head_tail_block(t); }

}

#if HGS_SSIM_TRACE
extern "C" int hgs_debug_set_ssim_trace(void* fwd, void* bwd) {
  void* p[2] = {fwd, bwd};
  HGS_CHECK_HIP(hipMemcpyToSymbol(HIP_SYMBOL(g_ssim_trace), p, sizeof(p)));
  return 0;
}
#endif

extern "C" {

size_t hgs_ssim_l1_scratch_floats(int C, int H, int W) {
  const size_t nb = (size_t)((W + LT - 1) / LT) * ((H + LT - 1) / LT) * C;
  return 3 * (size_t)C * H * W + 2 * nb;
}
int hgs_ssim_l1_num_blocks(int C, int H, int W) { return ((W + LT - 1) / LT) * ((H + LT - 1) / LT) * C; }

int hgs_ssim_l1_forward(void* stream, int C, int H, int W, const float* window11_host, const float* img1, const float* img2,
                        float* dmaps, float* partials) {
  if (!window11_host || !img1 || !img2 || !dmaps || !partials || C <= 0 || H <= 0 || W <= 0) {
    hgs_set_error("hgs_ssim_l1_forward: bad arguments");
    return 1;
  }
  SsimWin win;
  for (int k = 0; k < 11; k++) win.w[k] = window11_host[k];
  hipStream_t s = (hipStream_t)stream;
  {
    HgsProfScope _prof(s, HGS_K_SSIM_FWD);
    hipLaunchKernelGGL(ssim_l1_fwd_kernel, dim3(ssim_grid_size(ssim_grid(C, H, W), SSIM_FWD_WG_PER_XCD)), dim3(256), 0, s, H, W, ssim_grid(C, H, W), win, img1,
                       img2, (const HgsViewTargets*)nullptr, dmaps, partials, (unsigned char*)nullptr);
  }
  HGS_CHECK_LAUNCH();
  return 0;
}

int hgs_ssim_l1_backward(void* stream, int C, int H, int W, const float* window11_host, const float* img1, const float* img2,
                         const float* dmaps, const float* g_ssim_mean, const float* g_l1_mean, float* dL_dimg1) {
  if (!window11_host || !img1 || !img2 || !dmaps || !g_ssim_mean || !g_l1_mean || !dL_dimg1) {
    hgs_set_error("hgs_ssim_l1_backward: bad arguments");
    return 1;
  }
  SsimWin win;
  for (int k = 0; k < 11; k++) win.w[k] = window11_host[k];
  hipStream_t s = (hipStream_t)stream;
  {
    HgsProfScope _prof(s, HGS_K_SSIM_BWD);
    hipLaunchKernelGGL(ssim_l1_bwd_kernel, dim3(ssim_grid_size(ssim_grid(C, H, W), SSIM_BWD_WG_PER_XCD)), dim3(256), 0, s, H, W, ssim_grid(C, H, W), win, img1,
                       img2, (const HgsViewTargets*)nullptr, dmaps, g_ssim_mean, g_l1_mean, (const float*)nullptr, dL_dimg1,
                       (float*)nullptr, 0, (const int*)nullptr, (const unsigned char*)nullptr);
  }
  HGS_CHECK_LAUNCH();
  return 0;
}

static OriParams ori_params(const float* viewmatrix, const float* bg3_host, float min_val, const uint8_t* mask) {
  OriParams p;
  p.view = viewmatrix;
  p.bg0 = bg3_host[0]; p.bg1 = bg3_host[1]; p.bg2 = bg3_host[2];
  p.min_val = min_val;
  p.has_mask = mask != nullptr;
  return p;
}

int hgs_orientation_loss_num_blocks(int H, int W) { return (int)(((size_t)H * W + 255) / 256); }

int hgs_orientation_loss_forward(void* stream, int H, int W, const float* omap, const float* viewmatrix,
                                 const float* bg3_host, float min_val, const float* gt_theta, const float* confidence,
                                 const uint8_t* mask, float* partials) {
  if (!omap || !viewmatrix || !bg3_host || !gt_theta || !confidence || !partials) { hgs_set_error("hgs_orientation_loss_forward: null argument"); return 1; }
  const int N = H * W;
  hipStream_t s = (hipStream_t)stream;
  {
    HgsProfScope _prof(s, HGS_K_ORI_FWD);
    hipLaunchKernelGGL(ori_fwd_kernel, dim3((N + 255) / 256), dim3(256), 0, s, N, ori_params(viewmatrix, bg3_host, min_val, mask),
                       omap, gt_theta, confidence, mask, partials);
  }
  HGS_CHECK_LAUNCH();
  return 0;
}

int hgs_orientation_loss_backward(void* stream, int H, int W, const float* omap, const float* viewmatrix,
                                  const float* bg3_host, float min_val, const float* gt_theta, const float* confidence,
                                  const uint8_t* mask, const float* g_loss, const float* mask_count, float* d_omap) {
  if (!omap || !viewmatrix || !bg3_host || !gt_theta || !confidence || !g_loss || !mask_count || !d_omap) { hgs_set_error("hgs_orientation_loss_backward: null argument"); return 1; }
  const int N = H * W;
  hipStream_t s = (hipStream_t)stream;
  {
    HgsProfScope _prof(s, HGS_K_ORI_BWD);
    hipLaunchKernelGGL(ori_bwd_kernel, dim3((N + 255) / 256), dim3(256), 0, s, N, ori_params(viewmatrix, bg3_host, min_val, mask),
                       omap, gt_theta, confidence, mask, g_loss, mask_count, d_omap);
  }
  HGS_CHECK_LAUNCH();
  return 0;
}

static inline int head_nb_ssim(const HgsHeadParams* p) { return ((p->W + LT - 1) / LT) * ((p->H + LT - 1) / LT) * 3; }
static inline int head_nb_pix(const HgsHeadParams* p) { return (int)(((size_t)p->H * p->W + 255) / 256); }
static inline int head_nb_smooth(const HgsHeadParams* p) { return p->lambda_smooth > 0.f ? (p->n_smooth + 255) / 256 : 0; }
static inline size_t head_flags_offset(const HgsHeadParams* p) {
  return 9 * (size_t)p->H * p->W + 2 * (size_t)head_nb_ssim(p) + 3 * (size_t)head_nb_pix(p) + 2 * (size_t)head_nb_smooth(p) + 8;
}
static inline size_t head_flag_floats(const HgsHeadParams* p) { return ((size_t)head_nb_ssim(p) + 3) / 4 + 4; }
static inline unsigned char* head_zero_flags(const HgsHeadParams* p, float* scratch) { return (unsigned char*)(scratch + head_flags_offset(p)); }
static inline int* head_block_lists(const HgsHeadParams* p, float* scratch) {
  if (head_nb_ssim(p) > HEAD_MAX_FLAGGED) return nullptr;
  return (int*)(scratch + head_flags_offset(p) + 2 * head_flag_floats(p));
}
size_t hgs_loss_head_scratch_floats(const HgsHeadParams* p) {
  return head_flags_offset(p) + 2 * head_flag_floats(p) + 4 + 2 * (size_t)head_nb_ssim(p) + 12;
}

int hgs_loss_head_tail(const HgsHeadParams* p, const float* scratch, float* out, HgsHeadTail* tail) {
  if (!p || !scratch || !out || !tail) { hgs_set_error("hgs_loss_head_tail: null argument"); return 1; }
  tail->pix_partials = scratch + 9 * (size_t)p->H * p->W + 2 * (size_t)head_nb_ssim(p);
  tail->nb_pix = head_nb_pix(p);
  tail->out = out;
  tail->inv_hw = 1.f / (float)((size_t)p->H * p->W);
  tail->l_mask = p->lambda_mask; tail->l_ori = p->lambda_orientation; tail->l_smooth = p->lambda_smooth;
  tail->bce = p->lambda_mask > 0.f; tail->ori = p->lambda_orientation > 0.f; tail->smooth = head_nb_smooth(p) > 0;
  return 0;
}

int hgs_loss_head_forward(void* stream, const HgsHeadParams* p, const float* image, const float* mask_img,
                          const float* omap, const HgsViewTargets* targets, const float* endpoints,
                          const long long* smooth_pairs, float* scratch, float* out, float* d_extra_unit,
                          const float* smooth_partials_ext) {
  if (!p || !image || !mask_img || !omap || !targets || !scratch || !out || p->H <= 0 || p->W <= 0) {
    hgs_set_error("hgs_loss_head_forward: bad arguments");
    return 1;
  }
  const int H = p->H, W = p->W, N = H * W;
  if (p->tile_used && (p->tiles_x != (W + HGS_TILE - 1) / HGS_TILE || p->tiles_y != (H + HGS_TILE - 1) / HGS_TILE)) {
    hgs_set_error("hgs_loss_head_forward: tile_used given with tiles_x / tiles_y = %d x %d, the %d x %d frame has %d x %d tiles", p->tiles_x,
                  p->tiles_y, W, H, (W + HGS_TILE - 1) / HGS_TILE, (H + HGS_TILE - 1) / HGS_TILE);
    return 1;
  }
  if (p->tile_used && (((size_t)p->tile_used & 15) ||
                       (head_nb_ssim(p) <= HEAD_MAX_FLAGGED && (size_t)p->tiles_x * p->tiles_y > HEAD_MAX_TILES))) {
    hgs_set_error("hgs_loss_head_forward: tile_used %p covers %d x %d tiles, it must be 16-byte aligned and cover at most %d", (const void*)p->tile_used,
                  p->tiles_x, p->tiles_y, HEAD_MAX_TILES);
    return 1;
  }
  const int nbs = head_nb_ssim(p), nbp = head_nb_pix(p), nbm = head_nb_smooth(p);
  if (nbm > 0 && !smooth_partials_ext && (!endpoints || !smooth_pairs)) { hgs_set_error("hgs_loss_head_forward: smoothness term without endpoints"); return 1; }
  float* dmaps = scratch;
  float* p_ssim = dmaps + 9 * (size_t)N;
  float* p_pix = p_ssim + 2 * (size_t)nbs;
  const float* p_smooth = smooth_partials_ext ? smooth_partials_ext : p_pix + 3 * (size_t)nbp;
  SsimWin win;
  for (int k = 0; k < 11; k++) win.w[k] = p->window[k];
  hipStream_t s = (hipStream_t)stream;
  int* lists = head_block_lists(p, scratch);
  {
    HgsProfScope _prof(s, HGS_K_SSIM_FWD);
    hipLaunchKernelGGL(ssim_l1_fwd_kernel, dim3(ssim_grid_size(ssim_grid(3, H, W), SSIM_FWD_WG_PER_XCD)), dim3(256), 0, s, H, W, ssim_grid(3, H, W), win, image,
                       (const float*)nullptr, targets, dmaps, p_ssim, lists ? head_zero_flags(p, scratch) : nullptr);
  }
  HeadFlags fl;
  fl.bce = p->lambda_mask > 0.f; fl.ori = p->lambda_orientation > 0.f;
  if (nbm > 0 && !smooth_partials_ext &&
      hgs_launch_smooth_fwd(s, p->n_smooth, endpoints, smooth_pairs, p->cos_threshold, p->eps, p_pix + 3 * (size_t)nbp)) return 1;
  HeadReduce h;
  h.nb_ssim = nbs; h.nb_pix = nbp; h.nb_smooth = nbm;
  h.inv_chw = 1.f / (3.f * (float)N); h.inv_hw = 1.f / (float)N;
  h.l_dssim = p->lambda_dssim; h.l_mask = p->lambda_mask; h.l_ori = p->lambda_orientation; h.l_smooth = p->lambda_smooth;
  h.bce = fl.bce; h.ori = fl.ori;
  {
    HgsProfScope _prof(s, HGS_K_ORI_FWD);
    hipLaunchKernelGGL(pix_fwd_kernel, dim3(nbp + PIX_SIDE_WGS), dim3(256), 0, s, N, fl, p->bg[0], p->bg[1], p->bg[2], p->min_val, mask_img,
                       omap, targets, p_pix, fl.bce ? p->lambda_mask / (float)N : 0.f, fl.ori ? p->lambda_orientation : 0.f,
                       d_extra_unit, ssim_grid(3, H, W), (const unsigned char*)head_zero_flags(p, scratch), lists, h,
                       (const float*)p_ssim, p_smooth, out, p->tile_used, p->tiles_x, p->tiles_y, W, 1.f / (float)W);
  }
  if (!p->defer_tail) {
    HgsHeadTail t;
    hgs_loss_head_tail(p, scratch, out, &t);
    HgsProfScope _prof(s, HGS_K_HEAD);
    hipLaunchKernelGGL(head_tail_kernel, dim3(1), dim3(256), 0, s, t);
  }
  HGS_CHECK_LAUNCH();
  return 0;
}

int hgs_loss_head_backward(void* stream, const HgsHeadParams* p, const float* image, const float* mask_img,
                           const float* omap, const HgsViewTargets* targets, const float* endpoints,
                           const long long* smooth_pairs, const float* scratch, const float* out,
                           const float* grad_out, int skip, float* d_image, float* d_mask_img,
                           float* d_omap, float* d_endpoints) {
  const int skip_pixel_pass = skip & HGS_HEAD_SKIP_PIXELS;
  if (!p || !image || !mask_img || !omap || !targets || !scratch || !out || !grad_out || !d_image ||
      (!skip_pixel_pass && (!d_mask_img || !d_omap))) {
    hgs_set_error("hgs_loss_head_backward: bad arguments");
    return 1;
  }
  const int H = p->H, W = p->W, N = H * W;
  const int nbp = head_nb_pix(p), nbm = head_nb_smooth(p);
  const float* dmaps = scratch;
  SsimWin win;
  for (int k = 0; k < 11; k++) win.w[k] = p->window[k];
  hipStream_t s = (hipStream_t)stream;
  if (p->defer_tail && !skip_pixel_pass) {
    HgsHeadTail t;
    hgs_loss_head_tail(p, scratch, (float*)out, &t);
    HgsProfScope _prof(s, HGS_K_HEAD);
    hipLaunchKernelGGL(head_tail_kernel, dim3(1), dim3(256), 0, s, t);
  }
  {
    HgsProfScope _prof(s, HGS_K_SSIM_BWD);
    hipLaunchKernelGGL(ssim_l1_bwd_kernel, dim3(ssim_grid_size(ssim_grid(3, H, W), SSIM_BWD_WG_PER_XCD)), dim3(256), 0, s, H, W, ssim_grid(3, H, W), win, image,
                       (const float*)nullptr, targets, dmaps, out + HGS_HEAD_G_SSIM, out + HGS_HEAD_G_L1, grad_out, d_image,
                       d_endpoints, d_endpoints ? p->n_endpoints * 3 : 0, head_block_lists(p, (float*)scratch),
                       head_block_lists(p, (float*)scratch) ? (const unsigned char*)head_zero_flags(p, (float*)scratch) : nullptr);
  }
  HeadFlags fl;
  fl.bce = p->lambda_mask > 0.f; fl.ori = p->lambda_orientation > 0.f;
  if (!skip_pixel_pass) {
    HgsProfScope _prof(s, HGS_K_ORI_BWD);
    hipLaunchKernelGGL(pix_bwd_kernel, dim3(nbp), dim3(256), 0, s, N, fl, p->bg[0], p->bg[1], p->bg[2], p->min_val, mask_img,
                       omap, targets, out, grad_out, d_mask_img, d_omap);
  }
  if (d_endpoints && !(skip & HGS_HEAD_SKIP_SMOOTH)) {
    if (nbm > 0 && hgs_launch_smooth_bwd(s, p->n_smooth, endpoints, smooth_pairs, p->cos_threshold, p->eps,
                                         out + HGS_HEAD_G_SMOOTH, out + HGS_HEAD_SMOOTH_COUNT, grad_out, d_endpoints)) return 1;
  }
  HGS_CHECK_LAUNCH();
  return 0;
}

}
```

### hair-gs_amd/csrc/hgs_prologue.h

```cpp
#pragma once
#include "hgs_common.h"
#include "hgs_adam.h"

__host__ __device__ static inline unsigned hgs_prologue_blocks(size_t zero_words) {
  const size_t b = (zero_words + 1023) / 1024;
  return 1u + (unsigned)(b < 1024 ? b : 1024);
}

__device__ __forceinline__ void hgs_prologue_block(const HgsPrologue& p, unsigned wg, unsigned nwg, const uint32_t* keep = nullptr) {
  if (wg == 0) {
    const uint32_t* src = (const uint32_t*)(p.table + p.view);
    uint32_t* dst = (uint32_t*)p.slot;
    for (int i = threadIdx.x; i < (int)(sizeof(HgsViewTargets) / 4); i += 256) dst[i] = src[i];
    if (threadIdx.x == 0 && p.lr_dst) *p.lr_dst = p.lr;
    if (p.adam_prep) {
      __syncthreads();
      hgs_adam_prepare_block(p.adam_prep);
    }
    return;
  }
  uint32_t* z = (uint32_t*)p.zero_ptr;
  const size_t words = p.zero_bytes / 4, stride = (size_t)(nwg - 1) * 256;
  const uint32_t* keep1 = keep ? keep + 1 : nullptr;
  for (size_t i = (size_t)(wg - 1) * 256 + threadIdx.x; i < words; i += stride)
    if (z + i != keep && z + i != keep1) z[i] = 0u;
}

bool hgs_strands_prologue_kernel(const void* func, int* n_params);
bool hgs_preprocess_prologue_kernel(const void* func, int* n_params);
```

### hair-gs_amd/hgs_runtime/__init__.py

```python
import ctypes as C
import os
import subprocess

_PKG_ROOT = os.path.dirname(os.path.dirname(os.path.abspath(__file__)))
LIB_PATH = os.environ.get("HGS_LIB") or os.path.join(_PKG_ROOT, "libhgs.so")
CSRC = os.path.join(_PKG_ROOT, "csrc")
_lib = None

vp, ci, cf, sz = C.c_void_p, C.c_int, C.c_float, C.c_size_t

SIGNATURES = {
    "hgs_abi_version": (ci, []),
    "hgs_last_error": (C.c_char_p, []),
    "hgs_geom_bytes": (sz, [ci]),
    "hgs_image_bytes": (sz, [ci, ci]),
    "hgs_binning_bytes": (sz, [ci, ci]),
    "hgs_backward_scratch_bytes": (sz, [ci, ci, ci]),
    "hgs_forward_preprocess": (ci, [vp, ci, ci, ci, ci, ci, vp, vp, vp, vp, vp, cf, vp, vp, vp, vp, vp, cf, cf, ci,
                                    vp, vp, vp, vp, vp]),
    "hgs_forward_render": (ci, [vp, ci, ci, ci, ci, ci, ci, vp, vp, vp, vp, vp, vp, vp]),
    "hgs_backward": (ci, [vp, ci, ci, ci, ci, ci, ci, ci, ci, vp, vp, vp, vp, vp, cf, vp, vp, vp, vp, vp, cf, cf, vp, vp, vp,
                          vp, vp, vp, vp, vp, vp, vp, vp, vp, vp, vp, vp, vp]),
    "hgs_param_backward_bytes": (sz, []),
    "hgs_backward_multi_params": (ci, [vp, ci, ci, ci, ci, ci, ci, ci, vp, vp, vp, vp, vp, vp, vp, vp, cf, cf, vp, vp, vp, vp, vp,
                                       vp, vp, vp]),
    "hgs_hair_endpoint_gather": (ci, [vp, ci, vp, vp, vp, vp, vp]),
    "hgs_mark_visible": (ci, [vp, ci, vp, vp, vp, vp]),
    "hgs_dist2_scratch_bytes": (sz, [ci]),
    "hgs_dist2": (ci, [vp, ci, vp, vp, vp, sz]),
    "hgs_ssim_l1_scratch_floats": (sz, [ci, ci, ci]),
    "hgs_ssim_l1_num_blocks": (ci, [ci, ci, ci]),
    "hgs_ssim_l1_forward": (ci, [vp, ci, ci, ci, vp, vp, vp, vp, vp]),
    "hgs_ssim_l1_backward": (ci, [vp, ci, ci, ci, vp, vp, vp, vp, vp, vp, vp]),
    "hgs_orientation_loss_num_blocks": (ci, [ci, ci]),
    "hgs_orientation_loss_forward": (ci, [vp, ci, ci, vp, vp, vp, cf, vp, vp, vp, vp]),
    "hgs_orientation_loss_backward": (ci, [vp, ci, ci, vp, vp, vp, cf, vp, vp, vp, vp, vp, vp]),
    "hgs_adam_step": (ci, [vp, ci, vp, vp, vp, vp, vp, vp, vp, cf, cf, cf, vp]),
    "hgs_smoothness_num_blocks": (ci, [ci]),
    "hgs_smoothness_forward": (ci, [vp, ci, vp, vp, cf, cf, vp]),
    "hgs_smoothness_backward": (ci, [vp, ci, ci, vp, vp, cf, cf, vp, vp, vp]),
    "hgs_strand_geometry_forward": (ci, [vp, ci, vp, vp, vp, cf, vp, vp, vp, vp]),
    "hgs_strand_geometry_backward": (ci, [vp, ci, ci, vp, vp, vp, cf, vp, vp, vp, vp, vp, vp]),
    "hgs_view_targets_bytes": (sz, []),
    "hgs_head_params_bytes": (sz, []),
    "hgs_strand_fusion_bytes": (sz, []),
    "hgs_select_view": (ci, [vp, vp, ci, vp, cf, vp]),
    "hgs_iteration_prologue": (ci, [vp, vp, ci, vp, cf, vp, vp, sz, vp]),
    "hgs_adam_prep_bytes": (sz, []),
    "hgs_adam_inline_bytes": (sz, []),
    "hgs_image_zero_range": (ci, [ci, ci, vp, vp]),
    "hgs_graph_find_prologue": (ci, [vp, vp]),
    "hgs_graph_find_prologues": (ci, [vp, ci, vp, vp, vp]),
    "hgs_graph_set_prologue": (ci, [vp, vp, vp, ci, vp, cf, vp, vp, sz]),
    "hgs_set_view_queue": (ci, [vp, vp, ci, vp, cf, vp]),
    "hgs_select_view_queued": (ci, [vp, vp, ci, vp, vp, vp, vp]),
    "hgs_hair_params_forward": (ci, [vp, ci, vp, vp, vp, cf, vp, vp, vp, vp, vp, vp, vp, vp, vp]),
    "hgs_hair_params_backward": (ci, [vp, ci, ci, vp, vp, vp, cf, vp, vp, vp, vp, vp, vp, vp, vp, ci, vp, vp, vp, vp, vp]),
    "hgs_cloud_params_forward": (ci, [vp, ci, vp, vp, vp, vp, vp, vp, vp, vp, vp]),
    "hgs_cloud_forward_preprocess": (ci, [vp, ci, ci, ci, ci, ci, vp, vp, vp, vp, vp, vp, vp, vp, vp, vp, vp, vp, vp,
                                          cf, cf, ci, vp, vp, vp, vp, vp]),
    "hgs_hair_forward_preprocess": (ci, [vp, ci, ci, ci, ci, ci, vp, vp, vp, cf, vp, vp, vp, vp, vp, vp, vp, vp, vp, vp, vp,
                                         cf, cf, ci, vp, vp, vp, vp, vp]),
    "hgs_cloud_params_backward": (ci, [vp, ci, vp, vp, vp, vp, vp, vp, vp, vp, vp, vp, vp, vp, vp]),
    "hgs_loss_head_scratch_floats": (sz, [vp]),
    "hgs_loss_head_tail": (ci, [vp, vp, vp, vp]),
    "hgs_loss_head_forward": (ci, [vp, vp, vp, vp, vp, vp, vp, vp, vp, vp, vp, vp]),
    "hgs_loss_head_backward": (ci, [vp, vp, vp, vp, vp, vp, vp, vp, vp, vp, vp, ci, vp, vp, vp, vp]),
    "hgs_densify_stats": (ci, [vp, ci, vp, vp, ci, vp, vp, vp]),
    "hgs_radius_pairs": (ci, [vp, ci, vp, vp, cf, cf, ci, ci, vp, vp, vp, ci]),
    "hgs_knn3": (ci, [vp, ci, vp, vp, vp]),
    "hgs_nearest_distance_f64": (ci, [vp, ci, ci, vp, vp, vp]),
    "hgs_pointcloud_normals_scratch_bytes": (sz, [ci, ci]),
    "hgs_pointcloud_normals": (ci, [vp, ci, ci, vp, vp, vp, vp, sz]),
    "hgs_strand_walk_ends": (ci, [vp, ci, ci, vp, vp, vp, vp, vp, vp]),
    "hgs_strand_walk_fill": (ci, [vp, ci, vp, vp, vp, vp, vp, vp, vp]),
    "hgs_strand_grow_plan": (ci, [vp, ci, vp, vp, vp, ci, vp, ci, ci, ci, cf, vp, vp, vp]),
    "hgs_strand_grow_fill": (ci, [vp, ci, vp, vp, vp, ci, vp, vp, vp, ci, vp, ci, cf, vp, vp, vp, ci, vp, vp, vp, vp, vp, vp, vp, vp,
                                  vp, vp]),
    "hgs_oriented_match_scratch_bytes": (sz, [ci]),
    "hgs_oriented_match": (ci, [vp, ci, ci, ci, vp, vp, vp, vp, vp, ci, vp, vp, vp, sz]),
    "hgs_strand_votes": (ci, [vp, ci, ci, ci, vp, vp, vp, vp, vp, ci, vp, vp, ci, vp, vp, vp]),
    "hgs_orientation_scratch_bytes": (sz, [ci, ci, ci, ci, ci]),
    "hgs_orientation_field": (ci, [vp, ci, ci, ci, vp, ci, ci, vp, vp, vp, vp, vp, vp, vp, sz]),
    "hgs_orientation_confidence": (ci, [vp, ci, ci, ci, vp, vp, vp]),
    "hgs_view_stats_num_blocks": (ci, [ci, ci]),
    "hgs_view_stats": (ci, [vp, ci, ci, ci, vp, vp, vp, vp, cf, vp, vp, vp, vp, cf, vp, vp]),
    "hgs_raster_model_bytes": (sz, []),
    "hgs_raster_vertex_bytes": (sz, []),
    "hgs_raster_tiles": (ci, [ci, ci]),
    "hgs_raster_vertices": (ci, [vp, ci, ci, ci, ci, vp, vp, vp, vp]),
    "hgs_raster_count": (ci, [vp, ci, ci, ci, ci, vp, C.c_longlong, vp, ci, vp, vp, vp]),
    "hgs_raster_fill": (ci, [vp, ci, ci, ci, ci, vp, C.c_longlong, vp, ci, vp, vp, vp, vp, vp]),
    "hgs_raster_resolve": (ci, [vp, ci, ci, ci, ci, vp, vp, ci, vp, vp, vp, vp, vp, vp, vp, vp, vp, vp, vp]),
    "hgs_set_segment_policy": (ci, [ci, ci, ci]),
    "hgs_debug_set_wg_trace": (ci, [vp, vp]),
    "hgs_prof_enable": (ci, [ci]),
    "hgs_prof_bracket_overhead_ms": (C.c_double, []),
    "hgs_prof_collect": (ci, [vp, vp]),
    "hgs_prof_kernel_name": (C.c_char_p, [ci]),
    "hgs_geom_layout": (ci, [ci, vp]),
    "hgs_image_layout": (ci, [ci, ci, vp]),
    "hgs_binning_layout": (ci, [ci, vp]),
}
GEOM_FIELDS = ["depths", "clamped", "means2D", "cov3D", "conic_opacity", "rgb", "tiles_touched", "point_offsets", "rect",
               "block_sums"]
IMG_FIELDS = ["final_T", "n_contrib", "ranges", "tile_count", "tile_cursor", "tile_maxc", "status", "tile_order"]
BIN_FIELDS = ["keys", "point_list", "packed", "inv", "keys_sorted"]
PACKED_FLOATS = 12
INST_GRAD_FLOATS = 12


class HgsError(RuntimeError):
    pass


class ViewTargets(C.Structure):
    _fields_ = [("image", vp), ("float_mask", vp), ("orientation", vp), ("confidence", vp), ("mask", vp),
                ("viewmatrix", cf * 16), ("projmatrix", cf * 16), ("campos", cf * 3), ("mask_count", cf)]


class HeadParams(C.Structure):
    _fields_ = [("H", ci), ("W", ci), ("lambda_dssim", cf), ("lambda_mask", cf), ("lambda_orientation", cf),
                ("lambda_smooth", cf), ("bg", cf * 3), ("min_val", cf), ("window", cf * 11), ("n_smooth", ci),
                ("cos_threshold", cf), ("eps", cf), ("n_endpoints", ci), ("defer_tail", ci), ("tile_used", vp),
                ("tiles_x", ci), ("tiles_y", ci)]


class HeadTail(C.Structure):
    _fields_ = [("pix_partials", vp), ("nb_pix", ci), ("out", vp), ("inv_hw", cf), ("l_mask", cf), ("l_ori", cf),
                ("l_smooth", cf), ("bce", ci), ("ori", ci), ("smooth", ci)]


class Prologue(C.Structure):
    _fields_ = [("table", vp), ("view", ci), ("slot", vp), ("lr", cf), ("lr_dst", vp), ("zero_ptr", vp), ("zero_bytes", sz),
                ("adam_prep", vp)]


ADAM_MAX_TENSORS = 8


class AdamSlot(C.Structure):
    _fields_ = [("p", vp), ("m", vp), ("v", vp), ("coef", vp)]


class AdamPrep(C.Structure):
    _fields_ = [("n", ci), ("lr", vp * ADAM_MAX_TENSORS), ("step", vp * ADAM_MAX_TENSORS), ("beta1", cf), ("beta2", cf), ("coef", vp)]


class RasterModel(C.Structure):
    _fields_ = [("draw_base", C.c_longlong), ("idx_offset", C.c_longlong), ("n_prims", ci), ("kind", ci), ("width", ci), ("lit", ci),
                ("ka", C.c_double), ("kd", C.c_double)]


class AdamInline(C.Structure):
    _fields_ = [("slot", AdamSlot * 6), ("beta1", cf), ("beta2", cf), ("eps", cf)]


class StrandFusion(C.Structure):
    _fields_ = [("smooth_pairs", vp), ("n_smooth", ci), ("cos_threshold", cf), ("eps", cf), ("smooth_partials", vp),
                ("smooth_pair_grads", vp), ("head_out", vp), ("grad_out", vp), ("radii", vp), ("dmean2D", vp), ("dmean2D_stride", ci),
                ("max_radii2D", vp), ("grad_accum", vp), ("denom", vp), ("ep_segments", vp), ("ep_pairs", vp),
                ("n_endpoints", ci), ("head_tail", HeadTail), ("prologue", Prologue)]


class ParamBackward(C.Structure):
    _fields_ = [("kind", ci), ("endpoints", vp), ("endpoint_pairs", vp), ("dist_to_scale_factor", cf), ("seg_contrib", vp),
                ("d_width", vp), ("rotation_raw", vp), ("d_means3D", vp), ("d_scaling_raw", vp), ("d_rotation_raw", vp),
                ("extra4", vp), ("d_opacity_raw", vp), ("d_mask_raw", vp), ("dL_dmeans2D_rgb", vp), ("max_radii2D", vp),
                ("grad_accum", vp), ("denom", vp), ("head_tail", HeadTail), ("adam", AdamInline)]


PARAMS_HAIR, PARAMS_CLOUD = 1, 2
HEAD_SKIP_PIXELS, HEAD_SKIP_SMOOTH = 1, 2
VIEW_QUEUE_MAX = 16
HEAD_OUT = ["total", "l1", "dssim", "mask", "orientation", "smooth", "ori_count", "smooth_count", "g_ssim", "g_l1", "g_mask",
            "g_ori", "g_smooth", "total_fwd"]
HEAD_NOUT = 16
FUSED_PREPROCESS_MAX_TILES = 8192
ABI_VERSION = 10


def build(verbose=False):
    subprocess.check_call(["make", "-s", "-j8", "-C", CSRC], stdout=None if verbose else subprocess.DEVNULL)
    import c_utils
    c_utils.build()
    return LIB_PATH


def lib():
    global _lib
    if _lib is None:
        if not os.path.exists(LIB_PATH):
            raise HgsError(f"{LIB_PATH} not found: run hgs_runtime.build() (hipcc --offload-arch=gfx950). "
                           "There is no CPU fallback.")
        import torch
        L = C.CDLL(LIB_PATH)
        for name, (res, args) in SIGNATURES.items():
            fn = getattr(L, name)
            fn.restype = res
            fn.argtypes = args
        if L.hgs_abi_version() != ABI_VERSION:
            raise HgsError(f"{LIB_PATH}: ABI version {L.hgs_abi_version()}, this binding needs {ABI_VERSION}: "
                           "rebuild with hgs_runtime.build()")
        for fn, st in (("hgs_view_targets_bytes", ViewTargets), ("hgs_head_params_bytes", HeadParams),
                       ("hgs_strand_fusion_bytes", StrandFusion), ("hgs_param_backward_bytes", ParamBackward),
                       ("hgs_adam_prep_bytes", AdamPrep), ("hgs_adam_inline_bytes", AdamInline),
                       ("hgs_raster_model_bytes", RasterModel)):
            if getattr(L, fn)() != C.sizeof(st):
                raise HgsError(f"{LIB_PATH}: {fn}() = {getattr(L, fn)()} but the binding's struct has {C.sizeof(st)} bytes: "
                               "rebuild with hgs_runtime.build()")
        _lib = L
    return _lib


def check(status):
    if status != 0:
        raise HgsError(lib().hgs_last_error().decode())


def ptr(t):
    if t is None or t.numel() == 0:
        return None
    return t.data_ptr()


def current_stream():
    import torch
    return torch.cuda.current_stream().cuda_stream


def require_gpu_tensor(t, name, dtype=None):
    import torch
    if not t.is_cuda:
        raise HgsError(f"{name} must be a CUDA(HIP) tensor: libhgs.so only runs on the GPU, there is no CPU path")
    if dtype is not None and t.dtype != dtype:
        raise HgsError(f"{name} must be {dtype}, got {t.dtype}")
    return t.contiguous()


KERNEL_COUNT = 18


def prof_enable(on=True):
    lib().hgs_prof_enable(int(bool(on)))


def prof_collect():
    ms = (C.c_double * KERNEL_COUNT)()
    n = (C.c_longlong * KERNEL_COUNT)()
    check(lib().hgs_prof_collect(ms, n))
    return {lib().hgs_prof_kernel_name(i).decode(): (ms[i], n[i]) for i in range(KERNEL_COUNT)}


def layout(kind, *dims):
    n = {"geom": len(GEOM_FIELDS), "image": len(IMG_FIELDS), "binning": len(BIN_FIELDS)}[kind]
    arr = (C.c_size_t * n)()
    getattr(lib(), f"hgs_{kind}_layout")(*dims, arr)
    names = {"geom": GEOM_FIELDS, "image": IMG_FIELDS, "binning": BIN_FIELDS}[kind]
    return dict(zip(names, list(arr)))
```

### hair-gs_amd/hgs_runtime/strand_step.py

```python
import ctypes as C
import os
import math

import numpy as np
import torch

import hgs_runtime as rt
from hgs_runtime.fused import gaussian_window11

_SLOT_BYTES = C.sizeof(rt.ViewTargets)
_F_VIEW, _F_PROJ, _F_CAM = (rt.ViewTargets.viewmatrix.offset // 4, rt.ViewTargets.projmatrix.offset // 4,
                            rt.ViewTargets.campos.offset // 4)


class ViewTable:

    def __init__(self, cameras, device=None, targets=True):
        if len(cameras) == 0:
            raise rt.HgsError("ViewTable needs at least one camera")
        c0 = cameras[0]
        self.has_targets = bool(targets)
        if device is not None:
            self.device = torch.device(device)
        elif targets:
            self.device = c0.original_image.device
        else:
            self.device = c0.world_view_transform.device
        self.H, self.W = int(c0.image_height), int(c0.image_width)
        self.tanfovx, self.tanfovy = math.tan(c0.FoVx * 0.5), math.tan(c0.FoVy * 0.5)
        self.has_float_mask = targets and getattr(c0, "float_mask", None) is not None
        self.has_mask = targets and getattr(c0, "mask", None) is not None
        rows = (rt.ViewTargets * len(cameras))()
        self._keep = []
        for i, c in enumerate(cameras):
            if (int(c.image_height), int(c.image_width), c.FoVx, c.FoVy) != (self.H, self.W, c0.FoVx, c0.FoVy):
                raise rt.HgsError("all views of a ViewTable must share resolution and field of view")
            if targets and ((getattr(c, "float_mask", None) is not None) != self.has_float_mask or
                            (getattr(c, "mask", None) is not None) != self.has_mask):
                raise rt.HgsError("either every view has a mask or none")
            r = rows[i]
            keep = []
            if targets:
                img = rt.require_gpu_tensor(c.original_image, "original_image", torch.float32)
                ori = rt.require_gpu_tensor(c.orientation_field, "orientation_field", torch.float32)
                conf = rt.require_gpu_tensor(c.orientation_confidence, "orientation_confidence", torch.float32)
                keep = [img, ori, conf]
                r.image, r.orientation, r.confidence = img.data_ptr(), ori.data_ptr(), conf.data_ptr()
            if self.has_float_mask:
                fm = rt.require_gpu_tensor(c.float_mask, "float_mask", torch.float32)
                keep.append(fm)
                r.float_mask = fm.data_ptr()
            if self.has_mask:
                m = rt.require_gpu_tensor(c.mask, "mask")
                m = m.view(torch.uint8) if m.dtype == torch.bool else m.to(torch.uint8)
                keep.append(m)
                r.mask = m.data_ptr()
                r.mask_count = float(m.sum().item())
            for k, v in enumerate(c.world_view_transform.detach().float().cpu().reshape(-1).tolist()):
                r.viewmatrix[k] = v
            for k, v in enumerate(c.full_proj_transform.detach().float().cpu().reshape(-1).tolist()):
                r.projmatrix[k] = v
            for k, v in enumerate(c.camera_center.detach().float().cpu().reshape(-1).tolist()):
                r.campos[k] = v
            self._keep.append(keep)
        host = torch.from_numpy(np.frombuffer(bytes(rows), dtype=np.uint8).copy())
        self.table = host.to(self.device)
        self.slot = torch.zeros(_SLOT_BYTES, dtype=torch.uint8, device=self.device)
        f = self.slot.view(torch.float32)
        self.viewmatrix, self.projmatrix, self.campos = f[_F_VIEW:_F_VIEW + 16], f[_F_PROJ:_F_PROJ + 16], f[_F_CAM:_F_CAM + 3]
        self._cameras = list(cameras)
        self.index = {id(c): i for i, c in enumerate(cameras)}
        self.n = len(cameras)
        self.current = -1
        self.queue = torch.zeros(rt.VIEW_QUEUE_MAX, dtype=torch.int32, device=self.device)
        self.queue_lr = torch.zeros((), dtype=torch.float32, device=self.device)
        self._image, self._zero, self._image_ready = None, None, False
        self._rider = None
        self.counts_clean = False
        self._fill_behind = False
        self.adam_prep = None

    def select(self, view, lr=0.0, lr_dst=None):
        if not 0 <= int(view) < self.n:
            raise rt.HgsError(f"view {view} outside the table (0..{self.n - 1})")
        with torch.cuda.device(self.device):
            rt.check(rt.lib().hgs_select_view(rt.current_stream(), self.table.data_ptr(), int(view), self.slot.data_ptr(),
                                              float(lr), None if lr_dst is None else lr_dst.data_ptr()))
        self.current = int(view)
        self._rider = None

    def _image_zero_range(self, behind_counts=False):
        if self._image is None:
            L = rt.lib()
            self._image = torch.zeros((L.hgs_image_bytes(self.W, self.H),), dtype=torch.uint8, device=self.device)
            self.counts_clean = True
            off, nbytes = C.c_size_t(0), C.c_size_t(0)
            rt.check(L.hgs_image_zero_range(self.W, self.H, C.addressof(off), C.addressof(nbytes)))
            lay = rt.layout("image", self.W, self.H)
            assert lay["tile_count"] == off.value and off.value < lay["tile_cursor"] < off.value + nbytes.value
            skip = lay["tile_cursor"] - off.value
            self._zero = ((self._image.data_ptr() + off.value, nbytes.value),
                          (self._image.data_ptr() + off.value + skip, nbytes.value - skip))
        return self._zero[1 if behind_counts else 0]

    def fused_preprocess_possible(self):
        return ((self.W + 15) // 16) * ((self.H + 15) // 16) <= rt.FUSED_PREPROCESS_MAX_TILES

    def prologue(self, view, lr=0.0, lr_dst=None, ride=False):
        if not 0 <= int(view) < self.n:
            raise rt.HgsError(f"view {view} outside the table (0..{self.n - 1})")
        zp, zb = self._image_zero_range()
        if ride:
            self._rider = (int(view), float(lr), None if lr_dst is None else lr_dst.data_ptr())
        else:
            self._rider = None
            with torch.cuda.device(self.device):
                rt.check(rt.lib().hgs_iteration_prologue(rt.current_stream(), self.table.data_ptr(), int(view),
                                                         self.slot.data_ptr(), float(lr),
                                                         None if lr_dst is None else lr_dst.data_ptr(), zp, zb, self.adam_prep))
            self.counts_clean = True
        self.current = int(view)
        self._image_ready = True

    def fill_prologue(self, fu, behind_counts=False):
        if self._rider is None:
            return
        view, lr, lr_dst = self._rider
        adam_prep = self.adam_prep
        self._rider = None
        self._fill_behind = bool(behind_counts)
        zp, zb = self._image_zero_range(behind_counts)
        pro = fu.prologue
        pro.table, pro.view, pro.slot, pro.lr, pro.lr_dst = self.table.data_ptr(), view, self.slot.data_ptr(), lr, lr_dst
        pro.zero_ptr, pro.zero_bytes, pro.adam_prep = zp, zb, adam_prep

    def flush_prologue(self):
        if self._rider is None:
            return
        view, lr, lr_dst = self._rider
        adam_prep = self.adam_prep
        self._rider = None
        self._fill_behind = False
        zp, zb = self._image_zero_range()
        with torch.cuda.device(self.device):
            rt.check(rt.lib().hgs_iteration_prologue(rt.current_stream(), self.table.data_ptr(), view, self.slot.data_ptr(), lr,
                                                     lr_dst, zp, zb, adam_prep))
        self.counts_clean = True

    def ensure_counts_clean(self):
        if self.counts_clean or self._image is None:
            return
        (p0, _), (p1, _) = self._image_zero_range(False), self._image_zero_range(True)
        off = p0 - self._image.data_ptr()
        self._image[off:off + (p1 - p0)].zero_()
        self.counts_clean = True

    def take_image(self):
        if not self._image_ready:
            return None
        self._image_ready = False
        return self._image

    def graph_bind(self, cuda_graph, count=1):
        nodes, tags, n = (C.c_void_p * count)(), (C.c_float * count)(), C.c_int(0)
        rt.check(rt.lib().hgs_graph_find_prologues(C.c_void_p(int(cuda_graph.raw_cuda_graph())), count, nodes, tags, C.addressof(n)))
        order = sorted(range(n.value), key=lambda i: tags[i])
        if n.value != count or (count > 1 and [int(tags[i]) for i in order] != list(range(count))):
            raise rt.HgsError(f"graph_bind: expected {count} tagged prologue nodes, found {n.value} with tags {[tags[i] for i in order]}")
        return (cuda_graph, [nodes[i] for i in order], self._fill_behind)

    def graph_set(self, binding, view, lr=0.0, lr_dst=None, k=0):
        if not 0 <= int(view) < self.n:
            raise rt.HgsError(f"view {view} outside the table (0..{self.n - 1})")
        graph, nodes, behind = binding
        zp, zb = self._image_zero_range(behind)
        rt.check(rt.lib().hgs_graph_set_prologue(C.c_void_p(int(graph.raw_cuda_graph_exec())), C.c_void_p(nodes[k]),
                                                 self.table.data_ptr(), int(view), self.slot.data_ptr(), float(lr),
                                                 None if lr_dst is None else lr_dst.data_ptr(), zp, zb))
        self.current = int(view)

    def set_queue(self, views, lr=0.0):
        views = [int(v) for v in views]
        if not 1 <= len(views) <= rt.VIEW_QUEUE_MAX or any(not 0 <= v < self.n for v in views):
            raise rt.HgsError(f"view queue {views}: 1..{rt.VIEW_QUEUE_MAX} views inside the table (0..{self.n - 1})")
        arr = (C.c_int * len(views))(*views)
        with torch.cuda.device(self.device):
            rt.check(rt.lib().hgs_set_view_queue(rt.current_stream(), self.queue.data_ptr(), len(views), arr, float(lr),
                                                 self.queue_lr.data_ptr()))

    def select_queued(self, k, lr_dst=None):
        with torch.cuda.device(self.device):
            rt.check(rt.lib().hgs_select_view_queued(rt.current_stream(), self.table.data_ptr(), self.n,
                                                     self.queue[k:].data_ptr(), self.slot.data_ptr(), self.queue_lr.data_ptr(),
                                                     None if lr_dst is None else lr_dst.data_ptr()))
        self.current = -1


def _adjacency(member_ids, roles, n_targets, max_degree):
    ids = member_ids.to(torch.int64)
    if ids.numel() == 0:
        return torch.full((n_targets, max_degree), -1, dtype=torch.int32, device=ids.device)
    order = torch.argsort(ids, stable=True)
    ids_s = ids[order]
    first = torch.searchsorted(ids_s, ids_s, right=False)
    slot = torch.arange(ids.numel(), device=ids.device) - first
    if int(slot.max()) >= max_degree:
        return None
    table = torch.full((n_targets, max_degree), -1, dtype=torch.int32, device=ids.device)
    table[ids_s, slot] = order.to(torch.int32)
    return table.contiguous()


def head_params(H, W, opt, n_smooth, n_endpoints, min_val, has_float_mask, threshold_deg=30.0, eps=1e-6):
    p = rt.HeadParams()
    p.H, p.W = int(H), int(W)
    p.lambda_dssim = float(opt.lambda_dssim)
    p.lambda_mask = float(opt.lambda_mask) if has_float_mask else 0.0
    p.lambda_orientation = float(opt.lambda_orientation)
    p.lambda_smooth = float(getattr(opt, "lambda_smooth", 0.0)) if n_smooth > 0 else 0.0
    p.bg[0] = p.bg[1] = p.bg[2] = 0.0
    p.min_val = float(min_val)
    win = gaussian_window11()
    for k in range(11):
        p.window[k] = win[k]
    p.n_smooth = int(n_smooth)
    p.cos_threshold = float(np.cos(threshold_deg * np.pi / 180))
    p.eps = float(eps)
    p.n_endpoints = int(n_endpoints)
    return p


def _raster_head_forward(step, xyz, scale, quat, opacity, extra4, shs, endpoints, smooth_idx, smooth_partials, n_endpoints,
                         hair=None):
    from diff_gaussian_rasterization import _C as raster
    g, vt, hp, L = step.gaussians, step.views, step.head, rt.lib()
    dev = xyz.device
    f32 = dict(dtype=torch.float32, device=dev)
    empty = step.empty
    own_image = vt.take_image()
    R, planes, radii, geom, binning, img = raster.rasterize_gaussians_multi(
        step.bg7, xyz, empty, extra4, opacity, scale, quat, 1.0, empty, vt.viewmatrix, vt.projmatrix, vt.tanfovx,
        vt.tanfovy, vt.H, vt.W, shs, g.active_sh_degree, vt.campos, False, False, image_buffer=own_image, hair=hair)
    if own_image is not None and xyz.shape[0] > 0:
        vt.counts_clean = raster._state["last_counts_clean"]
    hp.n_endpoints = n_endpoints
    if step.skip_unread_blocks:
        if step._tile_maxc_offset is None:
            step._tile_maxc_offset = rt.layout("image", vt.W, vt.H)["tile_maxc"]
        hp.tile_used = img.data_ptr() + step._tile_maxc_offset
        hp.tiles_x, hp.tiles_y = (vt.W + 15) // 16, (vt.H + 15) // 16
    else:
        hp.tile_used = None
    scratch = torch.empty((L.hgs_loss_head_scratch_floats(C.byref(hp)),), **f32)
    out = torch.empty((rt.HEAD_NOUT,), **f32)
    d_extra = torch.empty((4, vt.H, vt.W), **f32) if (step.one_pass_pixels and vt.has_mask) else None
    if step.poison_unwritten and d_extra is not None:
        d_extra.fill_(float("nan"))
    hp.defer_tail = 1 if (step.defer_tail and xyz.shape[0] > 0) else 0
    with torch.cuda.device(dev):
        rt.check(L.hgs_loss_head_forward(rt.current_stream(), C.byref(hp), planes[0:3].data_ptr(), planes[3].data_ptr(),
                                         planes[4:7].data_ptr(), vt.slot.data_ptr(), rt.ptr(endpoints), rt.ptr(smooth_idx),
                                         rt.ptr(scratch), rt.ptr(out), rt.ptr(d_extra), rt.ptr(smooth_partials)))
    return R, planes, radii, geom, binning, img, scratch, out, d_extra


def _head_raster_backward(ctx, step, go, xyz, scale, quat, shs, planes, radii, geom, binning, img, scratch, out, endpoints,
                          d_ep, n_endpoints, params=None):
    from diff_gaussian_rasterization import _C as raster
    g, vt, hp, L = step.gaussians, step.views, step.head, rt.lib()
    dev = xyz.device
    f32 = dict(dtype=torch.float32, device=dev)
    unit_go = go is not None and go.data_ptr() == step.one.data_ptr()
    unit = ctx.d_extra is not None and unit_go
    go = step.one if go is None else go.contiguous().to(torch.float32)
    hp.n_endpoints = n_endpoints
    hp.defer_tail = 1 if ctx.defer_tail else 0
    if unit:
        d_image, d_extra = torch.empty((3, vt.H, vt.W), **f32), ctx.d_extra
    else:
        dplanes = torch.empty_like(planes)
        d_image, d_extra = dplanes[0:3], dplanes[3:7]
    if step.poison_unwritten:
        d_image.fill_(float("nan"))
    with torch.cuda.device(dev):
        rt.check(L.hgs_loss_head_backward(rt.current_stream(), C.byref(hp), planes[0:3].data_ptr(), planes[3].data_ptr(),
                                          planes[4:7].data_ptr(), vt.slot.data_ptr(), rt.ptr(endpoints),
                                          rt.ptr(step.smooth_pairs), rt.ptr(scratch), rt.ptr(out), rt.ptr(go),
                                          (rt.HEAD_SKIP_PIXELS if unit else 0) | (rt.HEAD_SKIP_SMOOTH if ctx.fused_smooth else 0),
                                          d_image.data_ptr(), d_extra[0].data_ptr(), d_extra[1:4].data_ptr(), rt.ptr(d_ep)))
    grad_planes = [d_image[k] for k in range(3)] + [d_extra[k] for k in range(4)]
    if params is not None:
        g_means2D = torch.empty((xyz.shape[0], 3), **f32)
        params.dL_dmeans2D_rgb = rt.ptr(g_means2D)
        g_sh = raster.rasterize_gaussians_multi_backward_params(
            step.bg7_backward, xyz, radii, scale, quat, vt.viewmatrix, vt.projmatrix, vt.tanfovx, vt.tanfovy, grad_planes, shs,
            g.active_sh_degree, vt.campos, geom, ctx.R, binning, img, params)
        return go, (g_means2D, None, None, None, g_sh, None, None)
    empty = step.empty
    (g_means2D, _gc, g_ex, g_opac, g_means3D, _gcov, g_sh, g_scales, g_rot) = raster.rasterize_gaussians_multi_backward(
        step.bg7_backward, xyz, radii, empty, scale, quat, 1.0, empty, vt.viewmatrix, vt.projmatrix, vt.tanfovx, vt.tanfovy,
        grad_planes, shs, g.active_sh_degree, vt.campos, geom, ctx.R, binning, img, False)
    return go, (g_means2D, g_ex, g_opac, g_means3D, g_sh, g_scales, g_rot)


def _params_stats(step, pb):
    g = step.gaussians
    step.last["stats_done"] = False
    if step.stats_in_backward:
        pb.max_radii2D, pb.grad_accum, pb.denom = g.max_radii2D.data_ptr(), g.xyz_gradient_accum.data_ptr(), g.denom.data_ptr()
        step.last["stats_done"] = True


def _tail_group(ctx, step, fu, scratch, out):
    if ctx.defer_tail:
        rt.check(rt.lib().hgs_loss_head_tail(C.byref(step.head), rt.ptr(scratch), rt.ptr(out), C.byref(fu.head_tail)))


def _stats_group(step, fu, radii, g_means2D):
    g = step.gaussians
    step.last["stats_done"] = False
    if step.stats_in_backward:
        fu.radii, fu.dmean2D, fu.dmean2D_stride = radii.data_ptr(), g_means2D.data_ptr(), int(g_means2D.shape[1])
        fu.max_radii2D, fu.grad_accum, fu.denom = g.max_radii2D.data_ptr(), g.xyz_gradient_accum.data_ptr(), g.denom.data_ptr()
        step.last["stats_done"] = True


class _StrandIteration(torch.autograd.Function):
    @staticmethod
    def forward(ctx, endpoints, width, opacity_raw, mask_raw, f_dc, f_rest, step):
        from diff_gaussian_rasterization import _C as raster
        g, vt, L = step.gaussians, step.views, rt.lib()
        endpoints = rt.require_gpu_tensor(endpoints, "endpoints", torch.float32)
        width = rt.require_gpu_tensor(width, "width", torch.float32)
        opacity_raw = rt.require_gpu_tensor(opacity_raw, "opacity", torch.float32)
        mask_raw = rt.require_gpu_tensor(mask_raw, "mask", torch.float32)
        pairs = rt.require_gpu_tensor(g.endpoint_pairs, "endpoint_pairs", torch.int64)
        dev, P, E = endpoints.device, pairs.shape[0], endpoints.shape[0]
        f32 = dict(dtype=torch.float32, device=dev)
        xyz, scale, quat = torch.empty((P, 3), **f32), torch.empty((P, 3), **f32), torch.empty((P, 4), **f32)
        opacity, extra4 = torch.empty((P, 1), **f32), torch.empty((P, 4), **f32)
        factor = float(g.dist_to_scale_factor)
        stream = rt.current_stream()
        step.refresh_inline_plan()
        ctx.use_inline = step.inline_plan() is not None
        if ctx.use_inline:
            step.inline_adam._inline_done = False
            if not (step.fuse_param_backward and P > 0 and step.ep_segments is not None and step.ep_segments.shape[0] == E):
                raise rt.HgsError("in-lane Adam is enabled but this iteration's backward cannot apply it (no segments, the fused "
                                  "parameter backward off, or an endpoint adjacency that predates a topology change: call "
                                  "refresh()); disable it with enable_inline_adam(False)")
        idx = step.smooth_pairs
        hp = step.head
        fu = rt.StrandFusion()
        smooth_partials = pair_grads = None
        if idx is not None and hp.lambda_smooth > 0:
            smooth_partials = torch.empty((2 * ((idx.shape[0] + 255) // 256),), **f32)
            fu.smooth_pairs, fu.n_smooth = idx.data_ptr(), int(idx.shape[0])
            fu.cos_threshold, fu.eps = hp.cos_threshold, hp.eps
            fu.smooth_partials = smooth_partials.data_ptr()
            if step.fuse_param_backward and step.ep_pairs is not None:
                pair_grads = torch.empty((idx.shape[0], 2, 4), **f32)
                fu.smooth_pair_grads = pair_grads.data_ptr()
        shs = f_dc if f_rest.numel() == 0 else torch.cat((f_dc, f_rest), dim=1)
        if step.fuse_preprocess:
            def fill(fused):
                if fused and not vt.counts_clean:
                    vt.flush_prologue()
                vt.fill_prologue(fu, behind_counts=fused)
            hair = raster.HairSource(endpoints, pairs, width, factor, opacity_raw, mask_raw, fu, fill)
        else:
            hair = None
            vt.fill_prologue(fu)
            with torch.cuda.device(dev):
                rt.check(L.hgs_hair_params_forward(stream, P, rt.ptr(endpoints), rt.ptr(pairs), rt.ptr(width), factor,
                                                   rt.ptr(opacity_raw), rt.ptr(mask_raw), rt.ptr(xyz), rt.ptr(scale),
                                                   rt.ptr(quat), None, rt.ptr(opacity), rt.ptr(extra4), C.byref(fu)))
        R, planes, radii, geom, binning, img, scratch, out, d_extra = _raster_head_forward(
            step, xyz, scale, quat, opacity, extra4, shs, endpoints, idx, smooth_partials, E, hair=hair)
        ctx.d_extra = d_extra
        ctx.defer_tail = bool(step.head.defer_tail)
        ctx.fused_smooth = smooth_partials is not None
        ctx.step, ctx.R, ctx.f_rest_k = step, R, f_rest.shape[1]
        ctx.set_materialize_grads(False)
        ctx.save_for_backward(endpoints, width, pairs, xyz, scale, quat, opacity, extra4, shs, planes, radii, geom, binning,
                              img, scratch, out)
        ctx.pair_grads = pair_grads
        step.last = {"planes": planes, "radii": radii, "terms": out}
        terms = out.detach()
        ctx.mark_non_differentiable(terms)
        return out[0], terms

    @staticmethod
    def backward(ctx, go, _):
        from diff_gaussian_rasterization import _C as raster
        step, L = ctx.step, rt.lib()
        g, vt, hp = step.gaussians, step.views, step.head
        (endpoints, width, pairs, xyz, scale, quat, opacity, extra4, shs, planes, radii, geom, binning, img, scratch,
         out) = ctx.saved_tensors
        dev, P, E = endpoints.device, pairs.shape[0], endpoints.shape[0]
        f32 = dict(dtype=torch.float32, device=dev)
        d_ep = torch.empty((E, 3), **f32)
        gather = step.ep_segments is not None and step.ep_segments.shape[0] == E
        d_w, d_o, d_m = torch.empty((P, 1), **f32), torch.empty((P, 1), **f32), torch.empty((P, 1), **f32)
        if gather and step.fuse_param_backward and P > 0:
            pb = rt.ParamBackward()
            seg_contrib = torch.empty((P, 2, 4), **f32)
            pb.kind, pb.endpoints, pb.endpoint_pairs = rt.PARAMS_HAIR, rt.ptr(endpoints), rt.ptr(pairs)
            pb.dist_to_scale_factor = float(g.dist_to_scale_factor)
            pb.seg_contrib, pb.d_width, pb.extra4 = rt.ptr(seg_contrib), rt.ptr(d_w), rt.ptr(extra4)
            pb.d_opacity_raw, pb.d_mask_raw = rt.ptr(d_o), rt.ptr(d_m)
            _params_stats(step, pb)
            plan = step.inline_plan() if ctx.use_inline else None
            ep_adam = None
            if plan is not None:
                plan.fill(pb.adam, (g._width, g._opacity, g._mask, g._features_dc))
                ep_adam = rt.AdamInline()
                plan.fill(ep_adam, (g._endpoints,))
            go, (g_means2D, _, _, _, g_sh, _, _) = _head_raster_backward(
                ctx, step, go, xyz, scale, quat, shs, planes, radii, geom, binning, img, scratch, out, endpoints, None, E,
                params=pb)
            fu = rt.StrandFusion()
            if ctx.fused_smooth:
                idx = step.smooth_pairs
                fu.smooth_pairs, fu.n_smooth = idx.data_ptr(), int(idx.shape[0])
                fu.cos_threshold, fu.eps = hp.cos_threshold, hp.eps
                fu.head_out, fu.grad_out = out.data_ptr(), go.data_ptr()
                if ctx.pair_grads is not None:
                    fu.smooth_pair_grads = ctx.pair_grads.data_ptr()
            _tail_group(ctx, step, fu, scratch, out)
            fu.ep_segments, fu.n_endpoints = step.ep_segments.data_ptr(), E
            fu.ep_pairs = None if step.ep_pairs is None else step.ep_pairs.data_ptr()
            with torch.cuda.device(dev):
                rt.check(L.hgs_hair_endpoint_gather(rt.current_stream(), E, rt.ptr(seg_contrib), rt.ptr(endpoints), rt.ptr(d_ep),
                                                    C.byref(fu), None if ep_adam is None else C.byref(ep_adam)))
            if plan is not None:
                plan.applied()
            step.last["dmean2D"] = g_means2D
            if ctx.f_rest_k == 0:
                d_dc, d_rest = g_sh, None
            else:
                d_dc, d_rest = g_sh[:, :1], g_sh[:, 1:]
            return d_ep, d_w, d_o, d_m, d_dc, d_rest, None
        if ctx.use_inline:
            raise rt.HgsError("the forward's prologue advanced Adam's step counters for an in-lane update this backward cannot apply")
        go, (g_means2D, g_ex, g_opac, g_means3D, g_sh, g_scales, g_rot) = _head_raster_backward(
            ctx, step, go, xyz, scale, quat, shs, planes, radii, geom, binning, img, scratch, out, endpoints,
            None if gather else d_ep, E)
        stream = rt.current_stream()
        fu = rt.StrandFusion()
        if ctx.fused_smooth:
            idx = step.smooth_pairs
            fu.smooth_pairs, fu.n_smooth = idx.data_ptr(), int(idx.shape[0])
            fu.cos_threshold, fu.eps = hp.cos_threshold, hp.eps
            fu.head_out, fu.grad_out = out.data_ptr(), go.data_ptr()
        _stats_group(step, fu, radii, g_means2D)
        _tail_group(ctx, step, fu, scratch, out)
        if gather:
            fu.ep_segments, fu.n_endpoints = step.ep_segments.data_ptr(), E
            fu.ep_pairs = None if step.ep_pairs is None else step.ep_pairs.data_ptr()
        with torch.cuda.device(dev):
            rt.check(L.hgs_hair_params_backward(stream, P, E, rt.ptr(endpoints), rt.ptr(pairs), rt.ptr(width),
                                                float(g.dist_to_scale_factor), rt.ptr(opacity), rt.ptr(extra4),
                                                rt.ptr(g_means3D), rt.ptr(g_scales), rt.ptr(g_rot), None, rt.ptr(g_opac),
                                                rt.ptr(g_ex), 1, rt.ptr(d_ep), rt.ptr(d_w), rt.ptr(d_o), rt.ptr(d_m),
                                                C.byref(fu)))
        step.last["dmean2D"] = g_means2D
        if ctx.f_rest_k == 0:
            d_dc, d_rest = g_sh, None
        else:
            d_dc, d_rest = g_sh[:, :1], g_sh[:, 1:]
        return d_ep, d_w, d_o, d_m, d_dc, d_rest, None


class FusedStrandStep:

    def __init__(self, gaussians, cameras, opt, bg):
        self.gaussians, self.opt = gaussians, opt
        self.views = cameras if isinstance(cameras, ViewTable) else ViewTable(cameras)
        if not self.views.has_targets:
            raise rt.HgsError("the training iteration needs a ViewTable built with the views' targets")
        dev = self.views.device
        self.bg7 = torch.cat([bg.to(dev, torch.float32), torch.zeros(4, device=dev)]).contiguous()
        self.bg7_backward = None if (bool((self.bg7 == 0).all()) and os.environ.get("HGS_BLACK_BG", "1") != "0") else self.bg7
        self.empty = torch.empty(0, device=dev)
        self.one = torch.ones((), dtype=torch.float32, device=dev)
        self.one_pass_pixels = True
        self.stats_in_backward = True
        self.skip_unread_blocks = bool(getattr(opt, "skip_unread_blocks", True))
        self._tile_maxc_offset = None
        self.poison_unwritten = False
        self.fuse_preprocess = bool(getattr(opt, "fuse_preprocess", True)) and os.environ.get("HGS_FUSE_PREPROCESS", "1") != "0"
        self.fuse_param_backward = bool(getattr(opt, "fuse_param_backward", True)) and os.environ.get("HGS_FUSE_PARAM_BACKWARD", "1") != "0"
        self.inline_adam = None
        self.defer_tail = False
        self.last = {}
        self.refresh()

    def inline_adam_possible(self):
        from hgs_runtime.fused import FusedAdam
        g = self.gaussians
        return (self.fuse_param_backward and isinstance(getattr(g, "optimizer", None), FusedAdam)
                and g._features_rest.numel() == 0 and getattr(self, "ep_segments", True) is not None
                and bool(getattr(self.opt, "inline_adam", True)) and os.environ.get("HGS_INLINE_ADAM", "1") != "0"
                and not (torch.distributed.is_available() and torch.distributed.is_initialized() and torch.distributed.get_world_size() > 1))

    def enable_inline_adam(self, on=True):
        on = bool(on) and self.inline_adam_possible()
        self.inline_adam = self.gaussians.optimizer if on else None
        self.views.adam_prep = self.inline_plan().prep_ptr if on else None
        return on

    def inline_plan(self):
        return None if self.inline_adam is None else self.inline_adam.inline_plan()

    def refresh_inline_plan(self):
        if self.inline_adam is not None:
            self.views.adam_prep = self.inline_plan().prep_ptr

    def refresh(self):
        g = self.gaussians
        idx = g.smoothness_index_pairs() if float(getattr(self.opt, "lambda_smooth", 0.0)) > 0 else None
        n = 0 if idx is None else int(idx.shape[0])
        self.smooth_pairs = rt.require_gpu_tensor(idx, "index_pairs", torch.int64) if n > 0 else None
        self.head = head_params(self.views.H, self.views.W, self.opt, n, g._endpoints.shape[0], g.min_val,
                                self.views.has_float_mask)
        E = g._endpoints.shape[0]
        cached = getattr(g, "_adjacency_cache", None)
        if cached is not None and cached[0] is g.endpoint_pairs and cached[1] is self.smooth_pairs and cached[2] == E:
            self.ep_segments, self.ep_pairs = cached[3], cached[4]
            return
        self.ep_segments = _adjacency(g.endpoint_pairs.reshape(-1), 2, E, 2)
        self.ep_pairs = None
        if self.ep_segments is not None and self.smooth_pairs is not None:
            self.ep_pairs = _adjacency(self.smooth_pairs.reshape(-1), 4, E, 4)
            if self.ep_pairs is None:
                self.ep_segments = None
        g._adjacency_cache = (g.endpoint_pairs, self.smooth_pairs, E, self.ep_segments, self.ep_pairs)

    def loss(self):
        g = self.gaussians
        return _StrandIteration.apply(g._endpoints, g._width, g._opacity, g._mask, g._features_dc, g._features_rest, self)

    def backward(self, loss):
        loss.backward(self.one)

    def terms(self):
        t = self.last["terms"]
        return {k: t[i] for i, k in enumerate(rt.HEAD_OUT[1:6], start=1)}

    def update_densification_stats(self):
        g, last = self.gaussians, self.last
        if last.get("stats_done"):
            return
        gm, radii = last["dmean2D"], last["radii"]
        with torch.cuda.device(gm.device):
            rt.check(rt.lib().hgs_densify_stats(rt.current_stream(), gm.shape[0], rt.ptr(radii), rt.ptr(gm), gm.shape[1],
                                                rt.ptr(g.max_radii2D), rt.ptr(g.xyz_gradient_accum), rt.ptr(g.denom)))


class _CloudIteration(torch.autograd.Function):

    @staticmethod
    def forward(ctx, xyz, scaling_raw, rotation_raw, opacity_raw, mask_raw, f_dc, f_rest, step):
        L = rt.lib()
        xyz = rt.require_gpu_tensor(xyz, "xyz", torch.float32)
        scaling_raw = rt.require_gpu_tensor(scaling_raw, "scaling", torch.float32)
        rotation_raw = rt.require_gpu_tensor(rotation_raw, "rotation", torch.float32)
        opacity_raw = rt.require_gpu_tensor(opacity_raw, "opacity", torch.float32)
        mask_raw = rt.require_gpu_tensor(mask_raw, "mask", torch.float32)
        dev, P = xyz.device, xyz.shape[0]
        f32 = dict(dtype=torch.float32, device=dev)
        scale, quat = torch.empty((P, 3), **f32), torch.empty((P, 4), **f32)
        opacity, extra4 = torch.empty((P, 1), **f32), torch.empty((P, 4), **f32)
        from diff_gaussian_rasterization import _C as raster
        fu = rt.StrandFusion()
        vt = step.views
        step.refresh_inline_plan()
        ctx.use_inline = step.inline_plan() is not None
        if ctx.use_inline:
            step.inline_adam._inline_done = False
            if not (step.fuse_param_backward and P > 0):
                raise rt.HgsError("in-lane Adam is enabled but this iteration's backward cannot apply it (no Gaussians, or the "
                                  "fused parameter backward off); disable it with enable_inline_adam(False)")
        if step.fuse_preprocess:
            def fill(fused):
                if fused and not vt.counts_clean:
                    vt.flush_prologue()
                vt.fill_prologue(fu, behind_counts=fused)
            src = raster.CloudSource(scaling_raw, rotation_raw, opacity_raw, mask_raw, fu, fill)
        else:
            src = None
            vt.fill_prologue(fu)
            with torch.cuda.device(dev):
                rt.check(L.hgs_cloud_params_forward(rt.current_stream(), P, rt.ptr(scaling_raw), rt.ptr(rotation_raw),
                                                    rt.ptr(opacity_raw), rt.ptr(mask_raw), rt.ptr(scale), rt.ptr(quat),
                                                    rt.ptr(opacity), rt.ptr(extra4), C.byref(fu)))
        shs = f_dc if f_rest.numel() == 0 else torch.cat((f_dc, f_rest), dim=1)
        R, planes, radii, geom, binning, img, scratch, out, d_extra = _raster_head_forward(
            step, xyz, scale, quat, opacity, extra4, shs, None, None, None, 0, hair=src)
        ctx.d_extra, ctx.fused_smooth = d_extra, True
        ctx.defer_tail = bool(step.head.defer_tail)
        ctx.step, ctx.R, ctx.f_rest_k = step, R, f_rest.shape[1]
        ctx.set_materialize_grads(False)
        ctx.save_for_backward(xyz, scaling_raw, rotation_raw, scale, quat, opacity, extra4, shs, planes, radii, geom, binning,
                              img, scratch, out)
        step.last = {"planes": planes, "radii": radii, "terms": out}
        terms = out.detach()
        ctx.mark_non_differentiable(terms)
        return out[0], terms

    @staticmethod
    def backward(ctx, go, _):
        step, L = ctx.step, rt.lib()
        (xyz, scaling_raw, rotation_raw, scale, quat, opacity, extra4, shs, planes, radii, geom, binning, img, scratch,
         out) = ctx.saved_tensors
        dev, P = xyz.device, xyz.shape[0]
        f32 = dict(dtype=torch.float32, device=dev)
        d_s, d_r = torch.empty((P, 3), **f32), torch.empty((P, 4), **f32)
        d_o, d_m = torch.empty((P, 1), **f32), torch.empty((P, 1), **f32)
        if step.fuse_param_backward and P > 0:
            pb = rt.ParamBackward()
            g_means3D = torch.empty((P, 3), **f32)
            pb.kind, pb.rotation_raw, pb.extra4 = rt.PARAMS_CLOUD, rt.ptr(rotation_raw), rt.ptr(extra4)
            pb.d_means3D, pb.d_scaling_raw, pb.d_rotation_raw = rt.ptr(g_means3D), rt.ptr(d_s), rt.ptr(d_r)
            pb.d_opacity_raw, pb.d_mask_raw = rt.ptr(d_o), rt.ptr(d_m)
            _params_stats(step, pb)
            plan = step.inline_plan() if ctx.use_inline else None
            if plan is not None:
                gm = step.gaussians
                plan.fill(pb.adam, (gm._xyz, gm._scaling, gm._rotation, gm._opacity, gm._mask, gm._features_dc))
            if ctx.defer_tail:
                rt.check(L.hgs_loss_head_tail(C.byref(step.head), rt.ptr(scratch), rt.ptr(out), C.byref(pb.head_tail)))
            go, (g_means2D, _, _, _, g_sh, _, _) = _head_raster_backward(
                ctx, step, go, xyz, scale, quat, shs, planes, radii, geom, binning, img, scratch, out, None, None, 0, params=pb)
            if plan is not None:
                plan.applied()
            step.last["dmean2D"] = g_means2D
            if ctx.f_rest_k == 0:
                d_dc, d_rest = g_sh, None
            else:
                d_dc, d_rest = g_sh[:, :1], g_sh[:, 1:]
            return g_means3D, d_s, d_r, d_o, d_m, d_dc, d_rest, None
        if ctx.use_inline:
            raise rt.HgsError("the forward's prologue advanced Adam's step counters for an in-lane update this backward cannot apply")
        go, (g_means2D, g_ex, g_opac, g_means3D, g_sh, g_scales, g_rot) = _head_raster_backward(
            ctx, step, go, xyz, scale, quat, shs, planes, radii, geom, binning, img, scratch, out, None, None, 0)
        fu = rt.StrandFusion()
        _stats_group(step, fu, radii, g_means2D)
        _tail_group(ctx, step, fu, scratch, out)
        with torch.cuda.device(dev):
            rt.check(L.hgs_cloud_params_backward(rt.current_stream(), P, rt.ptr(scaling_raw), rt.ptr(rotation_raw),
                                                 rt.ptr(opacity), rt.ptr(extra4), rt.ptr(g_scales), rt.ptr(g_rot),
                                                 rt.ptr(g_opac), rt.ptr(g_ex), rt.ptr(d_s), rt.ptr(d_r), rt.ptr(d_o),
                                                 rt.ptr(d_m), C.byref(fu)))
        step.last["dmean2D"] = g_means2D
        if ctx.f_rest_k == 0:
            d_dc, d_rest = g_sh, None
        else:
            d_dc, d_rest = g_sh[:, :1], g_sh[:, 1:]
        return g_means3D, d_s, d_r, d_o, d_m, d_dc, d_rest, None


class FusedCloudStep(FusedStrandStep):

    def refresh(self):
        g = self.gaussians
        self.smooth_pairs = None
        self.head = head_params(self.views.H, self.views.W, self.opt, 0, 0, getattr(g, "min_val", 1e-7),
                                self.views.has_float_mask)

    def loss(self):
        g = self.gaussians
        return _CloudIteration.apply(g._xyz, g._scaling, g._rotation, g._opacity, g._mask, g._features_dc, g._features_rest, self)


def fused_step_for(gaussians, views, opt, bg):
    from scene.hair_gaussian_model import HairGaussianModel
    cls = FusedStrandStep if isinstance(gaussians, HairGaussianModel) else FusedCloudStep
    return cls(gaussians, views, opt, bg)
```

### include/hgs.h

```cpp
#ifndef HGS_H_INCLUDED
#define HGS_H_INCLUDED

#include <stddef.h>
#include <stdint.h>

#ifdef __cplusplus
extern "C" {
#endif

#define HGS_ABI_VERSION 10
#define HGS_TILE 16

int hgs_abi_version(void);
const char* hgs_last_error(void);

size_t hgs_geom_bytes(int P);
size_t hgs_image_bytes(int W, int H);
size_t hgs_binning_bytes(int R, int channels);
size_t hgs_backward_scratch_bytes(int P, int R, int channels);

#define HGS_IMAGE_PREZEROED 2
#define HGS_COUNT_ROW_RUNS 4
#define HGS_TILE_CULL 8
#define HGS_WAIT_TIMED_OUT 0xFFFFFFFFu
int hgs_forward_preprocess(void* stream, int P, int D, int M, int W, int H,
                           const float* means3D, const float* shs, const float* colors_precomp,
                           const float* opacities, const float* scales, float scale_modifier,
                           const float* rotations, const float* cov3D_precomp,
                           const float* viewmatrix, const float* projmatrix, const float* campos,
                           float tan_fovx, float tan_fovy, int prefiltered,
                           void* geom_buf, void* image_buf, int* radii, int* num_rendered_host,
                           unsigned int* max_rendered);

#define HGS_RECORDS_PACKED 16
#define HGS_RECORDS_LAZY 32
int hgs_forward_render(void* stream, int P, int W, int H, int R_capacity, int n_extra, int flags,
                       const float* bg, const float* colors_precomp, const float* extra,
                       void* geom_buf, void* binning_buf, void* image_buf, float* out_color);

#define HGS_ROWS_INLINE 64
#define HGS_ROWS_REDUCE 128
int hgs_backward(void* stream, int P, int D, int M, int R, int W, int H, int n_extra, int flags, const float* bg,
                 const float* means3D, const float* shs, const float* colors_precomp,
                 const float* scales, float scale_modifier, const float* rotations,
                 const float* cov3D_precomp, const float* viewmatrix, const float* projmatrix,
                 const float* campos, float tan_fovx, float tan_fovy, const int* radii,
                 const void* geom_buf, const void* binning_buf, const void* image_buf,
                 const float* const* dL_dpix_planes, void* scratch, float* dL_dextra,
                 float* dL_dmeans2D, float* dL_dconic, float* dL_dopacity, float* dL_dcolors,
                 float* dL_dmeans3D, float* dL_dcov3D, float* dL_dsh, float* dL_dscales,
                 float* dL_drotations);

int hgs_mark_visible(void* stream, int P, const float* means3D, const float* viewmatrix,
                     const float* projmatrix, uint8_t* present);

size_t hgs_dist2_scratch_bytes(int P);
int hgs_dist2(void* stream, int P, const float* points, float* out, void* scratch, size_t scratch_bytes);

size_t hgs_ssim_l1_scratch_floats(int C, int H, int W);
int hgs_ssim_l1_num_blocks(int C, int H, int W);
int hgs_ssim_l1_forward(void* stream, int C, int H, int W, const float* window11_host, const float* img1,
                        const float* img2, float* dmaps, float* partials);
int hgs_ssim_l1_backward(void* stream, int C, int H, int W, const float* window11_host, const float* img1,
                         const float* img2, const float* dmaps, const float* g_ssim_mean, const float* g_l1_mean,
                         float* dL_dimg1);
int hgs_orientation_loss_num_blocks(int H, int W);
int hgs_orientation_loss_forward(void* stream, int H, int W, const float* omap, const float* viewmatrix,
                                 const float* bg3_host, float min_val, const float* gt_theta, const float* confidence,
                                 const uint8_t* mask, float* partials);
int hgs_orientation_loss_backward(void* stream, int H, int W, const float* omap, const float* viewmatrix,
                                  const float* bg3_host, float min_val, const float* gt_theta, const float* confidence,
                                  const uint8_t* mask, const float* g_loss, const float* mask_count, float* d_omap);
int hgs_adam_step(void* stream, int n_tensors, float* const* params, const float* const* grads, float* const* exp_avg,
                  float* const* exp_avg_sq, const float* const* lr, float* const* step, const long long* numel,
                  float beta1, float beta2, float eps, unsigned int* tickets);
int hgs_smoothness_num_blocks(int N);
int hgs_smoothness_forward(void* stream, int N, const float* endpoints, const long long* index_pairs,
                           float cos_threshold, float eps, float* partials);
int hgs_smoothness_backward(void* stream, int N, int E, const float* endpoints, const long long* index_pairs,
                            float cos_threshold, float eps, const float* g_loss, const float* count, float* d_endpoints);
int hgs_strand_geometry_forward(void* stream, int P, const float* endpoints, const long long* endpoint_pairs,
                                const float* width, float dist_to_scale_factor, float* xyz, float* scale, float* quat,
                                float* dir);
int hgs_strand_geometry_backward(void* stream, int P, int E, const float* endpoints, const long long* endpoint_pairs,
                                 const float* width, float dist_to_scale_factor, const float* g_xyz, const float* g_scale,
                                 const float* g_quat, const float* g_dir, float* d_endpoints, float* d_width);

typedef struct HgsViewTargets {
  const float* image;
  const float* float_mask;
  const float* orientation;
  const float* confidence;
  const unsigned char* mask;
  float viewmatrix[16];
  float projmatrix[16];
  float campos[3];
  float mask_count;
} HgsViewTargets;
size_t hgs_view_targets_bytes(void);
size_t hgs_head_params_bytes(void);
size_t hgs_strand_fusion_bytes(void);
#define HGS_ADAM_MAX_TENSORS 8
typedef struct HgsAdamSlot { float* p; float* m; float* v; const float* coef; } HgsAdamSlot;
typedef struct HgsAdamPrep {
  int n; const float* lr[HGS_ADAM_MAX_TENSORS]; float* step[HGS_ADAM_MAX_TENSORS]; float beta1, beta2;
  float* coef;
} HgsAdamPrep;
typedef struct HgsAdamInline { HgsAdamSlot slot[6]; float beta1, beta2, eps; } HgsAdamInline;
size_t hgs_adam_prep_bytes(void);
size_t hgs_adam_inline_bytes(void);

int hgs_select_view(void* stream, const HgsViewTargets* table, int view, HgsViewTargets* slot, float lr, float* lr_dst);
int hgs_iteration_prologue(void* stream, const HgsViewTargets* table, int view, HgsViewTargets* slot, float lr, float* lr_dst,
                           void* zero_ptr, size_t zero_bytes, const HgsAdamPrep* adam_prep );
int hgs_image_zero_range(int W, int H, size_t* offset, size_t* bytes);
typedef struct HgsPrologue {
  const HgsViewTargets* table; int view; HgsViewTargets* slot; float lr; float* lr_dst;
  void* zero_ptr; size_t zero_bytes;
  const HgsAdamPrep* adam_prep;
} HgsPrologue;
int hgs_graph_find_prologue(void* graph, void** node_out);
int hgs_graph_find_prologues(void* graph, int max_nodes, void** nodes_out, float* lr_out, int* n_out);
int hgs_graph_set_prologue(void* graph_exec, void* node, const HgsViewTargets* table, int view, HgsViewTargets* slot, float lr,
                           float* lr_dst, void* zero_ptr, size_t zero_bytes);
#define HGS_VIEW_QUEUE_MAX 16
int hgs_set_view_queue(void* stream, int* queue, int n, const int* views_host, float lr, float* lr_slot);
int hgs_select_view_queued(void* stream, const HgsViewTargets* table, int n_views, const int* view_index,
                           HgsViewTargets* slot, const float* lr_slot, float* lr_dst);

typedef struct HgsHeadTail {
  const float* pix_partials; int nb_pix;
  float* out;
  float inv_hw, l_mask, l_ori, l_smooth;
  int bce, ori, smooth;
} HgsHeadTail;

typedef struct HgsStrandFusion {
  const long long* smooth_pairs; int n_smooth; float cos_threshold, eps;
  float* smooth_partials;
  float* smooth_pair_grads;
  const float* head_out; const float* grad_out;
  const int* radii; const float* dmean2D; int dmean2D_stride;
  float* max_radii2D; float* grad_accum; float* denom;
  const int* ep_segments; const int* ep_pairs; int n_endpoints;
  HgsHeadTail head_tail;
  HgsPrologue prologue;
} HgsStrandFusion;
int hgs_hair_params_forward(void* stream, int P, const float* endpoints, const long long* endpoint_pairs,
                            const float* width, float dist_to_scale_factor, const float* opacity_raw,
                            const float* mask_raw, float* xyz, float* scale, float* quat, float* dir, float* opacity,
                            float* extra4, const HgsStrandFusion* fusion);
#define HGS_FUSED_PREPROCESS_MAX_TILES 8192
int hgs_hair_forward_preprocess(void* stream, int P, int D, int M, int W, int H, const float* endpoints,
                                const long long* endpoint_pairs, const float* width, float dist_to_scale_factor,
                                const float* opacity_raw, const float* mask_raw, const float* shs, float* xyz, float* scale,
                                float* quat, float* opacity, float* extra4, const float* viewmatrix, const float* projmatrix,
                                const float* campos, float tan_fovx, float tan_fovy, int flags, void* geom_buf,
                                void* image_buf, int* radii, unsigned int* max_rendered, const HgsStrandFusion* fusion);
int hgs_cloud_forward_preprocess(void* stream, int P, int D, int M, int W, int H, const float* means3D, const float* scaling_raw,
                                 const float* rotation_raw, const float* opacity_raw, const float* mask_raw, const float* shs,
                                 float* scale, float* quat, float* opacity, float* extra4, const float* viewmatrix,
                                 const float* projmatrix, const float* campos, float tan_fovx, float tan_fovy, int flags,
                                 void* geom_buf, void* image_buf, int* radii, unsigned int* max_rendered,
                                 const HgsStrandFusion* fusion);
int hgs_hair_params_backward(void* stream, int P, int E, const float* endpoints, const long long* endpoint_pairs,
                             const float* width, float dist_to_scale_factor, const float* opacity, const float* extra4,
                             const float* g_xyz, const float* g_scale, const float* g_quat, const float* g_dir,
                             const float* g_opacity, const float* g_extra4, int accumulate_endpoints,
                             float* d_endpoints, float* d_width, float* d_opacity_raw, float* d_mask_raw,
                             const HgsStrandFusion* fusion);

enum { HGS_PARAMS_HAIR = 1, HGS_PARAMS_CLOUD = 2 };
typedef struct HgsParamBackward {
  int kind;
  const float* endpoints; const long long* endpoint_pairs; float dist_to_scale_factor;
  float* seg_contrib; float* d_width;
  const float* rotation_raw;
  float* d_means3D; float* d_scaling_raw; float* d_rotation_raw;
  const float* extra4;
  float* d_opacity_raw; float* d_mask_raw;
  float* dL_dmeans2D_rgb;
  float* max_radii2D; float* grad_accum; float* denom;
  HgsHeadTail head_tail;
  HgsAdamInline adam;
} HgsParamBackward;
size_t hgs_param_backward_bytes(void);
int hgs_backward_multi_params(void* stream, int P, int D, int M, int R, int W, int H, int flags, const float* bg7,
                              const float* means3D, const float* shs, const float* scales, const float* rotations,
                              const float* viewmatrix, const float* projmatrix, const float* campos, float tan_fovx,
                              float tan_fovy, const int* radii, const void* geom_buf, const void* binning_buf, const void* image_buf,
                              const float* const* dL_dpix_planes7, void* scratch, float* dL_dsh, const HgsParamBackward* params);
int hgs_hair_endpoint_gather(void* stream, int E, const float* seg_contrib, const float* endpoints, float* d_endpoints,
                             const HgsStrandFusion* fusion, const HgsAdamInline* adam);

int hgs_cloud_params_forward(void* stream, int P, const float* scaling_raw, const float* rotation_raw,
                             const float* opacity_raw, const float* mask_raw, float* scale, float* quat, float* opacity,
                             float* extra4, const HgsStrandFusion* fusion );
int hgs_cloud_params_backward(void* stream, int P, const float* scaling_raw, const float* rotation_raw,
                              const float* opacity, const float* extra4, const float* g_scale, const float* g_quat,
                              const float* g_opacity, const float* g_extra4, float* d_scaling_raw, float* d_rotation_raw,
                              float* d_opacity_raw, float* d_mask_raw, const HgsStrandFusion* fusion);

enum { HGS_HEAD_SKIP_PIXELS = 1, HGS_HEAD_SKIP_SMOOTH = 2 };
typedef struct HgsHeadParams {
  int H, W;
  float lambda_dssim, lambda_mask, lambda_orientation, lambda_smooth;
  float bg[3];
  float min_val;
  float window[11];
  int n_smooth;
  float cos_threshold, eps;
  int n_endpoints;
  int defer_tail;
  const unsigned int* tile_used; int tiles_x, tiles_y;
} HgsHeadParams;
enum { HGS_HEAD_TOTAL = 0, HGS_HEAD_L1, HGS_HEAD_DSSIM, HGS_HEAD_MASK, HGS_HEAD_ORIENTATION, HGS_HEAD_SMOOTH,
       HGS_HEAD_ORI_COUNT, HGS_HEAD_SMOOTH_COUNT, HGS_HEAD_G_SSIM, HGS_HEAD_G_L1, HGS_HEAD_G_MASK, HGS_HEAD_G_ORI,
       HGS_HEAD_G_SMOOTH, HGS_HEAD_TOTAL_FWD, HGS_HEAD_NOUT = 16 };
size_t hgs_loss_head_scratch_floats(const HgsHeadParams* p);
int hgs_loss_head_tail(const HgsHeadParams* p, const float* scratch, float* out, HgsHeadTail* tail);
int hgs_loss_head_forward(void* stream, const HgsHeadParams* p, const float* image, const float* mask_img,
                          const float* omap, const HgsViewTargets* targets, const float* endpoints,
                          const long long* smooth_pairs, float* scratch, float* out, float* d_extra_unit,
                          const float* smooth_partials_ext);
int hgs_loss_head_backward(void* stream, const HgsHeadParams* p, const float* image, const float* mask_img,
                           const float* omap, const HgsViewTargets* targets, const float* endpoints,
                           const long long* smooth_pairs, const float* scratch, const float* out,
                           const float* grad_out, int skip, float* d_image, float* d_mask_img,
                           float* d_omap, float* d_endpoints);

int hgs_densify_stats(void* stream, int P, const int* radii, const float* dL_dmean2D, int stride, float* max_radii2D,
                      float* xyz_gradient_accum, float* denom);

enum { HGS_K_PREPROCESS_FWD = 0, HGS_K_SCAN, HGS_K_SCATTER, HGS_K_SORT_TILES, HGS_K_BLEND_FWD, HGS_K_BLEND_BWD,
       HGS_K_PREPROCESS_BWD, HGS_K_KNN, HGS_K_SSIM_FWD, HGS_K_SSIM_BWD, HGS_K_STRAND_FWD, HGS_K_STRAND_BWD,
       HGS_K_ORI_FWD, HGS_K_ORI_BWD, HGS_K_ADAM, HGS_K_SMOOTH, HGS_K_HEAD, HGS_K_MISC, HGS_K_COUNT };
int hgs_prof_enable(int on);
double hgs_prof_bracket_overhead_ms(void);
int hgs_prof_collect(double* total_ms, long long* launches);
const char* hgs_prof_kernel_name(int kernel_id);

int hgs_radius_pairs(void* stream, int N, const float* pos, const float* dir, float radius, float min_cos,
                     int bidirectional, int capacity, int* pairs, float* dist, int* count, int sorted_by_x);

int hgs_knn3(void* stream, int N, const float* points, int* idx , float* dist2 );
int hgs_nearest_distance_f64(void* stream, int N, int M, const float* points, const double* refs, double* out);
size_t hgs_pointcloud_normals_scratch_bytes(int N, int K);
int hgs_pointcloud_normals(void* stream, int N, int K, const double* points , double* normals ,
                           int* neighbors , void* scratch, size_t scratch_bytes);
int hgs_strand_walk_ends(void* stream, int n, int n_ep, const long long* pairs, int* deg, void* nodes, int* other, int* len, int* flags);
int hgs_strand_walk_fill(void* stream, int S, const long long* starts, const long long* offsets, const unsigned char* flip,
                         const void* nodes, long long* rows, long long* seg_rows, int* id_to_strand);
int hgs_strand_grow_plan(void* stream, int S, const long long* offsets, const long long* rows, const float* endpoints, int n_ep,
                         const long long* deg, int n_deg, int max_segments, int k_avg, float min_val, int* status, unsigned* keep,
                         float* mean_len);
int hgs_strand_grow_fill(void* stream, int S, const long long* offsets, const long long* rows, const long long* seg_rows, int P,
                         const int* status, const int* rank, const unsigned* keep, int k_avg, const float* endpoints, int n_ep,
                         float growth_length, const float* length_src, const float* f_dc, const float* f_rest, int rest_floats,
                         const float* opacity, const float* mask, const float* width, long long* new_pairs, float* new_endpoints,
                         float* new_f_dc, float* new_f_rest, float* new_opacity, float* new_mask, float* new_width);

size_t hgs_oriented_match_scratch_bytes(int nB);
int hgs_oriented_match(void* stream, int nA, int nB, int K, const double* a_pts, const double* a_dirs, const double* b_pts,
                       const double* b_dirs, const double* thresholds_host, int bidirectional, const double* box_host,
                       uint32_t* mask, void* scratch, size_t scratch_bytes);
int hgs_strand_votes(void* stream, int S, int nB, int K, const double* a_pts, const double* a_dirs, const long long* offsets,
                     const int* b_strand, const double* thresholds_host, int bidirectional, const double* box_host,
                     const void* scratch, int capacity, int* best, int* overflow, int* n_overflow);

size_t hgs_orientation_scratch_bytes(int N, int H, int W, int A, int side);
int hgs_orientation_field(void* stream, int N, int H, int W, const unsigned char* gray, int A, int side, const double* weights,
                          const double* thetas, unsigned char* idx_out, double* var_out, double* maxinv_out, unsigned char* responses,
                          void* scratch, size_t scratch_bytes);
int hgs_orientation_confidence(void* stream, int N, int H, int W, const double* var, const double* maxinv, float* conf_out);

#define HGS_VIEW_STATS_N 10
int hgs_view_stats_num_blocks(int H, int W);
int hgs_view_stats(void* stream, int V, int H, int W, const float* pred, const float* gt, const unsigned char* gt_mask, const float* fg,
                   float fg_threshold, const float* omap, const float* viewmats, const float* gt_theta, const float* confidence,
                   float min_val, double* partials, double* out);

#define HGS_RASTER_MAX_MODELS 64
typedef struct HgsRasterModel {
  long long draw_base;
  long long idx_offset;
  int n_prims, kind;
  int width, lit;
  double ka, kd;
} HgsRasterModel;
size_t hgs_raster_model_bytes(void);
size_t hgs_raster_vertex_bytes(void);
int hgs_raster_tiles(int W, int H);
int hgs_raster_vertices(void* stream, int V, int NV, int W, int H, const double* pw, const double* views, const double* projs,
                        void* vout);
int hgs_raster_count(void* stream, int V, int W, int H, int n_models, const HgsRasterModel* models, long long n_prims,
                     const unsigned* idx, int NV, const void* vout, int* tile_counts, unsigned long long* dropped);
int hgs_raster_fill(void* stream, int V, int W, int H, int n_models, const HgsRasterModel* models, long long n_prims,
                    const unsigned* idx, int NV, const void* vout, const int* tile_counts, const long long* tile_offsets,
                    int* tile_cursor, unsigned* list);
int hgs_raster_resolve(void* stream, int V, int W, int H, int n_models, const HgsRasterModel* models, const unsigned* idx,
                       int NV, const void* vout, const double* pw, const double* nw, const double* col, const double* light_host,
                       const unsigned char* background_host, const int* tile_counts, const long long* tile_offsets,
                       const unsigned* list, unsigned char* rgb, unsigned char* gray);

int hgs_set_segment_policy(int min_len, int max_len, int target_segments);
int hgs_debug_set_wg_trace(void* device_buf_fwd, void* device_buf_bwd);

enum { HGS_GEOM_DEPTHS = 0, HGS_GEOM_CLAMPED, HGS_GEOM_MEANS2D, HGS_GEOM_COV3D, HGS_GEOM_CONIC_OPACITY,
       HGS_GEOM_RGB, HGS_GEOM_TILES_TOUCHED, HGS_GEOM_POINT_OFFSETS, HGS_GEOM_RECT, HGS_GEOM_BLOCK_SUMS,
       HGS_GEOM_NFIELDS };
enum { HGS_IMG_FINAL_T = 0, HGS_IMG_N_CONTRIB, HGS_IMG_RANGES, HGS_IMG_TILE_COUNT, HGS_IMG_TILE_CURSOR,
       HGS_IMG_TILE_MAXC, HGS_IMG_STATUS, HGS_IMG_TILE_ORDER, HGS_IMG_NFIELDS };
enum { HGS_BIN_KEYS = 0, HGS_BIN_POINT_LIST, HGS_BIN_PACKED, HGS_BIN_INV, HGS_BIN_KEYS_TMP, HGS_BIN_NFIELDS };
int hgs_geom_layout(int P, size_t* offsets );
int hgs_image_layout(int W, int H, size_t* offsets );
int hgs_binning_layout(int R, size_t* offsets );

#define HGS_STATUS_WORDS 16
#define HGS_PACKED_FLOATS 12
#define HGS_INST_GRAD_FLOATS 12

#ifdef __cplusplus
}
#endif
#endif
```

Baseline: 4211 iters/s.

## Precompute per-view background pixel-run loss sums and skip background waves

Adds a one-time kernel that evaluates the mask BCE and orientation loss terms for every 64-pixel run of each view, assuming background render values, and caches the per-run sums. During training, an extra workgroup in the SSIM forward kernel builds a bitmask of runs that touch no used tile. The pixel loss kernel then reads the cached sums for those runs instead of loading per-pixel targets and computing the terms. The view index is written after the view slot so the cached table can be indexed. This adds per-view cache memory and a serial mask-building block, and it relies on untouched pixels producing exactly the background values.

```diff
diff --git a/hair-gs_amd/csrc/hgs_api.hip b/hair-gs_amd/csrc/hgs_api.hip
--- a/hair-gs_amd/csrc/hgs_api.hip
+++ b/hair-gs_amd/csrc/hgs_api.hip
@@ -77,6 +77,7 @@
   const uint32_t* src = (const uint32_t*)(table + view);
   uint32_t* dst = (uint32_t*)slot;
   for (int i = threadIdx.x; i < (int)(sizeof(HgsViewTargets) / 4); i += 64) dst[i] = src[i];
+  if (threadIdx.x == 0) dst[sizeof(HgsViewTargets) / 4] = (uint32_t)view;
   if (threadIdx.x == 0 && lr_dst && lr_slot) *lr_dst = *lr_slot;
 }
 
diff --git a/hair-gs_amd/csrc/hgs_losses.hip b/hair-gs_amd/csrc/hgs_losses.hip
--- a/hair-gs_amd/csrc/hgs_losses.hip
+++ b/hair-gs_amd/csrc/hgs_losses.hip
@@ -290,10 +290,59 @@
   m[0] = 0.f; m[1] = -S * iB2; m[2] = 2.f * C1 * inv;
 }
 
+#define HEAD_MAX_TILES 45056
+struct RunMaskJob { const unsigned int* tile_used; unsigned int* masks; int* counts; int tiles_x, tiles_y, W, N; };
+#define RUNMASK_LDS_WORDS (HEAD_MAX_TILES / 32 + 1)
+__device__ __forceinline__ void build_run_masks(const RunMaskJob& jb, unsigned* __restrict__ tbits) {
+  const int n_tiles = jb.tiles_x * jb.tiles_y, n4 = (n_tiles + 3) >> 2, nw = (n_tiles + 31) >> 5;
+  const uint4* tu4 = (const uint4*)jb.tile_used;
+  if (threadIdx.x == 0) tbits[RUNMASK_LDS_WORDS - 1] = 0u;
+  for (int w = threadIdx.x; w < nw; w += 256) {
+    uint4 v[8];
+#pragma unroll
+    for (int u = 0; u < 8; u++) v[u] = tu4[min(8 * w + u, n4 - 1)];
+    unsigned bits = 0u;
+#pragma unroll
+    for (int u = 0; u < 8; u++) {
+      const int t = 32 * w + 4 * u;
+      unsigned nib = (v[u].x != 0u ? 1u : 0u) | (v[u].y != 0u ? 2u : 0u) | (v[u].z != 0u ? 4u : 0u) | (v[u].w != 0u ? 8u : 0u);
+      if (t + 4 > n_tiles) nib &= t < n_tiles ? (1u << (n_tiles - t)) - 1u : 0u;
+      bits |= nib << (4 * u);
+    }
+    tbits[w] = bits;
+  }
+  __syncthreads();
+  const int nblk = (jb.N + 255) >> 8, nwords = (nblk + 7) >> 3;
+  int n_bg = 0;
+  for (int w = threadIdx.x; w < nwords; w += 256) {
+    const int i0 = w * 2048;
+    int y = i0 / jb.W, x = i0 - y * jb.W;
+    unsigned m = 0u;
+    for (int r = 0; r < 32; r++) {
+      int left = min(64, jb.N - (i0 + 64 * r));
+      if (left <= 0) { m |= 1u << r; continue; }
+      unsigned any = 0u;
+      while (left > 0) {
+        const int len = min(left, jb.W - x), row = (y >> 4) * jb.tiles_x;
+        for (int t = x >> 4; t <= (x + len - 1) >> 4; t++) any |= (tbits[(row + t) >> 5] >> ((row + t) & 31)) & 1u;
+        left -= len; x += len;
+        if (x == jb.W) { x = 0; y++; }
+      }
+      if (!any) { m |= 1u << r; n_bg++; }
+    }
+    jb.masks[w] = m;
+  }
+#pragma unroll
+  for (int d = 32; d >= 1; d >>= 1) n_bg += __shfl_xor(n_bg, d, 64);
+  if ((threadIdx.x & 63) == 0) atomicAdd(&tbits[RUNMASK_LDS_WORDS - 1], (unsigned)n_bg);
+  __syncthreads();
+  if (threadIdx.x == 0) { jb.counts[0] = (int)tbits[RUNMASK_LDS_WORDS - 1]; jb.counts[1] = (jb.N + 63) >> 6; }
+}
+
 __global__ __launch_bounds__(256) __attribute__((amdgpu_waves_per_eu(HGS_SSIM_FWD_WAVES, HGS_SSIM_FWD_WAVES))) void ssim_l1_fwd_kernel(int H, int W, SsimGrid gd, SsimWin win, const float* __restrict__ img1,
                                                           const float* __restrict__ img2_, const HgsViewTargets* __restrict__ tgt,
                                                           float* __restrict__ dmap, float* __restrict__ partials,
-                                                          unsigned char* __restrict__ zero_flags) {
+                                                          unsigned char* __restrict__ zero_flags, RunMaskJob rm) {
 #if HGS_SSIM_FWD_ALIAS
   __shared__ float smem[4 * TILE * HP];
   static_assert(4 * TILE * HP >= 2 * TILE * TPW, "filtered planes cover the tile");
@@ -304,6 +353,8 @@
   __shared__ float hz[4][TILE][HP];
 #endif
   __shared__ float red[8];
+  static_assert(2 * TILE * TPW >= RUNMASK_LDS_WORDS, "the tile bitmap of build_run_masks fits the tile's LDS");
+  if (rm.masks && blockIdx.x == gridDim.x - 1) { build_run_masks(rm, (unsigned*)&t[0][0][0]); return; }
   const size_t plane = (size_t)H * W, cp = (size_t)gd.C * plane;
   const HGS_GLOBAL float* im1 = hgs_global(img1);
   const HGS_GLOBAL float* im2 = tgt ? hgs_global(tgt->image) : hgs_global(img2_);
@@ -714,7 +765,6 @@
 #ifndef HGS_PIX_TRACE
 #define HGS_PIX_TRACE 0
 #endif
-#define HEAD_MAX_TILES 45056
 #define HEAD_MAX_FLAGGED 32768
 static_assert(HEAD_MAX_FLAGGED % (32 * 256) == 0, "whole 32-block words per thread of the list builder");
 static_assert(HEAD_MAX_TILES % 32 == 0 && HEAD_MAX_TILES >= 4 * (HEAD_MAX_FLAGGED / 3), "2 x 2 tiles per block of 3 channels");
@@ -867,6 +917,58 @@
   if (threadIdx.x == 0) { lists[0] = all; lists[1] = all_z; }
 }
 
+__device__ __forceinline__ void pix_eval(const HeadFlags& fl, bool has_mask, const HgsViewTargets* __restrict__ tgt, float bg0, float bg1,
+                                         float bg2, float min_val, float xm, float ym, float o0, float o1, float o2, float gt, float cf,
+                                         unsigned char mk, bool grad, float g_mask, float g_ori, float& s, float& cnt, float& b,
+                                         float& gm, float& g0, float& g1, float& g2) {
+  if (fl.bce) {
+    const float x = xm, y = ym;
+    const float en = __expf(-fabsf(x));
+    b = fmaxf(x, 0.f) - x * y + __logf(1.f + en);
+    if (grad) { const float r1 = __builtin_amdgcn_rcpf(1.f + en); gm = g_mask * ((x >= 0.f ? r1 : en * r1) - y); }
+  }
+  if (fl.ori) {
+    OriParams p;
+    p.view = tgt->viewmatrix; p.bg0 = bg0; p.bg1 = bg1; p.bg2 = bg2; p.min_val = min_val; p.has_mask = has_mask;
+    const bool m = p.has_mask ? mk != 0 : (o0 != p.bg0 || o1 != p.bg1 || o2 != p.bg2);
+    if (m) {
+      float px, py, r, n, x, y, yq, th;
+      ori_pixel(p, o0, o1, o2, px, py, r, n, x, y, yq, th);
+      const float hp = 1.57079632679489661923f;
+      s = (hp - fabsf(fabsf(th - gt) - hp)) * cf;
+      cnt = 1.f;
+      if (grad) ori_pixel_grad(p, px, py, r, n, x, yq, th, gt, cf, g_ori / tgt->mask_count, g0, g1, g2);
+    }
+  }
+}
+
+__global__ __launch_bounds__(256) void pix_bg_runs_kernel(int N, HeadFlags fl, float bg0, float bg1, float bg2, float min_val, float mask_bg,
+                                                          const HgsViewTargets* __restrict__ table, int nruns, float* __restrict__ out) {
+  const HgsViewTargets* __restrict__ tgt = table + blockIdx.y;
+  const int i = blockIdx.x * 256 + threadIdx.x;
+  float s = 0.f, cnt = 0.f, b = 0.f;
+  if (i < N) {
+    const bool has_mask = tgt->mask != nullptr;
+    float xm = mask_bg, ym = 0.f, o0 = bg0, o1 = bg1, o2 = bg2, gt = 0.f, cf = 0.f;
+    asm volatile("" : "+v"(xm), "+v"(o0), "+v"(o1), "+v"(o2));
+    unsigned char mk = 0;
+    if (fl.bce) ym = hgs_global(tgt->float_mask)[i];
+    if (fl.ori) {
+      gt = hgs_global(tgt->orientation)[i]; cf = hgs_global(tgt->confidence)[i];
+      if (has_mask) mk = hgs_global(tgt->mask)[i];
+    }
+    float gm = 0.f, g0 = 0.f, g1 = 0.f, g2 = 0.f;
+    pix_eval(fl, has_mask, tgt, bg0, bg1, bg2, min_val, xm, ym, o0, o1, o2, gt, cf, mk, false, 0.f, 0.f, s, cnt, b, gm, g0, g1, g2);
+  }
+#pragma unroll
+  for (int d = 32; d >= 1; d >>= 1) { s += __shfl_xor(s, d, 64); cnt += __shfl_xor(cnt, d, 64); b += __shfl_xor(b, d, 64); }
+  const int run = i >> 6;
+  if ((threadIdx.x & 63) == 0 && run < nruns) {
+    float* o = out + ((size_t)blockIdx.y * nruns + run) * 3;
+    o[0] = s; o[1] = cnt; o[2] = b;
+  }
+}
+
 #define PIX_SIDE_WGS 2
 __global__ __launch_bounds__(256) __attribute__((amdgpu_waves_per_eu(8))) void pix_fwd_kernel(int N, HeadFlags fl, float bg0, float bg1, float bg2, float min_val,
                                                       const float* __restrict__ mask_img, const float* __restrict__ omap,
@@ -876,14 +978,19 @@
                                                       int* __restrict__ lists, HeadReduce h,
                                                       const float* __restrict__ p_ssim, const float* __restrict__ p_smooth,
                                                       float* __restrict__ out, const unsigned int* __restrict__ tile_used,
-                                                      int tiles_x, int tiles_y, int W, float inv_w) {
-  __shared__ float red[4];
+                                                      int tiles_x, int tiles_y, int W, float inv_w,
+                                                      const unsigned int* __restrict__ run_masks, const float* __restrict__ bg_runs,
+                                                      int bg_views, int nruns, int* __restrict__ run_counts) {
+  __shared__ float red[12];
   if (blockIdx.x < PIX_SIDE_WGS) {
 #if HGS_PIX_TRACE
     const unsigned long long t0 = __builtin_amdgcn_s_memrealtime();
 #endif
     if (blockIdx.x == 0) { if (lists) build_block_lists(gd, zero_flags, lists, tile_used, tiles_x, tiles_y); }
-    else head_part1(h, p_ssim, p_smooth, out);
+    else {
+      if (!run_masks && threadIdx.x == 0) { run_counts[0] = 0; run_counts[1] = nruns; }
+      head_part1(h, p_ssim, p_smooth, out);
+    }
 #if HGS_PIX_TRACE
     __syncthreads();
     if (threadIdx.x == 0 && lists) { lists[4 + 2 * gd.total + 2 * blockIdx.x] = (int)(unsigned)t0; lists[4 + 2 * gd.total + 2 * blockIdx.x + 1] = (int)(unsigned)__builtin_amdgcn_s_memrealtime(); }
@@ -892,8 +999,17 @@
   }
   const int blk = blockIdx.x - PIX_SIDE_WGS;
   const int i = blk * 256 + threadIdx.x;
+  const int wave = __builtin_amdgcn_readfirstlane((int)(threadIdx.x >> 6));
+  const bool bgwave = run_masks ? ((run_masks[blk >> 3] >> (4 * (blk & 7) + wave)) & 1u) != 0u : false;
   float s = 0.f, cnt = 0.f, b = 0.f;
-  if (i < N) {
+  if (bgwave) {
+    const int run = 4 * blk + wave;
+    if (run < nruns) {
+      const int view = min(max(((const int*)(tgt + 1))[0], 0), bg_views - 1);
+      const float* e = bg_runs + ((size_t)view * nruns + run) * 3;
+      s = e[0]; cnt = e[1]; b = e[2];
+    }
+  } else if (i < N) {
     const bool has_mask = tgt->mask != nullptr;
     float xm = 0.f, ym = 0.f, o0 = 0.f, o1 = 0.f, o2 = 0.f, gt = 0.f, cf = 0.f;
     unsigned char mk = 0;
@@ -912,33 +1028,23 @@
       used = tile_used[(y >> 4) * tiles_x + (x >> 4)];
     }
     float gm = 0.f, g0 = 0.f, g1 = 0.f, g2 = 0.f;
-    if (fl.bce) {
-      const float x = xm, y = ym;
-      const float en = __expf(-fabsf(x));
-      b = fmaxf(x, 0.f) - x * y + __logf(1.f + en);
-      if (d_unit) { const float r1 = __builtin_amdgcn_rcpf(1.f + en); gm = g_mask * ((x >= 0.f ? r1 : en * r1) - y); }
-    }
-    if (fl.ori) {
-      OriParams p;
-      p.view = tgt->viewmatrix; p.bg0 = bg0; p.bg1 = bg1; p.bg2 = bg2; p.min_val = min_val; p.has_mask = has_mask;
-      const bool m = p.has_mask ? mk != 0 : (o0 != p.bg0 || o1 != p.bg1 || o2 != p.bg2);
-      if (m) {
-        float px, py, r, n, x, y, yq, th;
-        ori_pixel(p, o0, o1, o2, px, py, r, n, x, y, yq, th);
-        const float hp = 1.57079632679489661923f;
-        s = (hp - fabsf(fabsf(th - gt) - hp)) * cf;
-        cnt = 1.f;
-        if (d_unit) ori_pixel_grad(p, px, py, r, n, x, yq, th, gt, cf, g_ori / tgt->mask_count, g0, g1, g2);
-      }
-    }
+    pix_eval(fl, has_mask, tgt, bg0, bg1, bg2, min_val, xm, ym, o0, o1, o2, gt, cf, mk, d_unit != nullptr, g_mask, g_ori, s, cnt, b,
+             gm, g0, g1, g2);
     if (d_unit && used) {
       d_unit[i] = gm; d_unit[(size_t)N + i] = g0; d_unit[2 * (size_t)N + i] = g1; d_unit[3 * (size_t)N + i] = g2;
     }
   }
-  const float bs = block_sum(s, red);
-  const float bc = block_sum(cnt, red);
-  const float bb = block_sum(b, red);
-  if (threadIdx.x == 0) { partials[3 * blk] = bs; partials[3 * blk + 1] = bc; partials[3 * blk + 2] = bb; }
+  if (!bgwave) {
+#pragma unroll
+    for (int d = 32; d >= 1; d >>= 1) { s += __shfl_xor(s, d, 64); cnt += __shfl_xor(cnt, d, 64); b += __shfl_xor(b, d, 64); }
+  }
+  if ((threadIdx.x & 63) == 0) { red[wave] = s; red[4 + wave] = cnt; red[8 + wave] = b; }
+  __syncthreads();
+  if (threadIdx.x == 0) {
+    partials[3 * blk] = (red[0] + red[1]) + (red[2] + red[3]);
+    partials[3 * blk + 1] = (red[4] + red[5]) + (red[6] + red[7]);
+    partials[3 * blk + 2] = (red[8] + red[9]) + (red[10] + red[11]);
+  }
 #if HGS_PIX_TRACE
   if (threadIdx.x == 0 && lists && (blk == 0 || blk == (int)gridDim.x - PIX_SIDE_WGS - 1 || blk == 4000))
     lists[4 + 2 * gd.total + 4 + (blk == 0 ? 0 : (blk == 4000 ? 1 : 2))] = (int)(unsigned)__builtin_amdgcn_s_memrealtime();
@@ -1008,7 +1114,7 @@
   {
     HgsProfScope _prof(s, HGS_K_SSIM_FWD);
     hipLaunchKernelGGL(ssim_l1_fwd_kernel, dim3(ssim_grid_size(ssim_grid(C, H, W), SSIM_FWD_WG_PER_XCD)), dim3(256), 0, s, H, W, ssim_grid(C, H, W), win, img1,
-                       img2, (const HgsViewTargets*)nullptr, dmaps, partials, (unsigned char*)nullptr);
+                       img2, (const HgsViewTargets*)nullptr, dmaps, partials, (unsigned char*)nullptr, RunMaskJob{});
   }
   HGS_CHECK_LAUNCH();
   return 0;
@@ -1077,9 +1183,10 @@
 static inline int head_nb_ssim(const HgsHeadParams* p) { return ((p->W + LT - 1) / LT) * ((p->H + LT - 1) / LT) * 3; }
 static inline int head_nb_pix(const HgsHeadParams* p) { return (int)(((size_t)p->H * p->W + 255) / 256); }
 static inline int head_nb_smooth(const HgsHeadParams* p) { return p->lambda_smooth > 0.f ? (p->n_smooth + 255) / 256 : 0; }
-static inline size_t head_flags_offset(const HgsHeadParams* p) {
+static inline size_t head_runs_offset(const HgsHeadParams* p) {
   return 9 * (size_t)p->H * p->W + 2 * (size_t)head_nb_ssim(p) + 3 * (size_t)head_nb_pix(p) + 2 * (size_t)head_nb_smooth(p) + 8;
 }
+static inline size_t head_flags_offset(const HgsHeadParams* p) { return head_runs_offset(p) + 4 + ((size_t)head_nb_pix(p) + 7) / 8; }
 static inline size_t head_flag_floats(const HgsHeadParams* p) { return ((size_t)head_nb_ssim(p) + 3) / 4 + 4; }
 static inline unsigned char* head_zero_flags(const HgsHeadParams* p, float* scratch) { return (unsigned char*)(scratch + head_flags_offset(p)); }
 static inline int* head_block_lists(const HgsHeadParams* p, float* scratch) {
@@ -1088,6 +1195,24 @@
 }
 size_t hgs_loss_head_scratch_floats(const HgsHeadParams* p) {
   return head_flags_offset(p) + 2 * head_flag_floats(p) + 4 + 2 * (size_t)head_nb_ssim(p) + 12;
+}
+size_t hgs_loss_head_run_counts_offset(const HgsHeadParams* p) { return head_runs_offset(p); }
+int hgs_loss_head_num_runs(const HgsHeadParams* p) { return (int)(((size_t)p->H * p->W + 63) / 64); }
+
+int hgs_loss_head_background_runs(void* stream, const HgsHeadParams* p, const HgsViewTargets* table, int n_views, float* out) {
+  if (!p || !table || !out || n_views <= 0 || p->H <= 0 || p->W <= 0) {
+    hgs_set_error("hgs_loss_head_background_runs: bad arguments (n_views = %d)", n_views);
+    return 1;
+  }
+  if (n_views > 65535) { hgs_set_error("hgs_loss_head_background_runs: %d views, at most 65535 per call", n_views); return 1; }
+  const int N = p->H * p->W;
+  HeadFlags fl;
+  fl.bce = p->lambda_mask > 0.f; fl.ori = p->lambda_orientation > 0.f;
+  hipStream_t s = (hipStream_t)stream;
+  hipLaunchKernelGGL(pix_bg_runs_kernel, dim3(head_nb_pix(p), n_views), dim3(256), 0, s, N, fl, p->bg[0], p->bg[1], p->bg[2], p->min_val,
+                     p->mask_bg, table, hgs_loss_head_num_runs(p), out);
+  HGS_CHECK_LAUNCH();
+  return 0;
 }
 
 int hgs_loss_head_tail(const HgsHeadParams* p, const float* scratch, float* out, HgsHeadTail* tail) {
@@ -1123,6 +1248,13 @@
   }
   const int nbs = head_nb_ssim(p), nbp = head_nb_pix(p), nbm = head_nb_smooth(p);
   if (nbm > 0 && !smooth_partials_ext && (!endpoints || !smooth_pairs)) { hgs_set_error("hgs_loss_head_forward: smoothness term without endpoints"); return 1; }
+  if (p->bg_runs && p->bg_views <= 0) { hgs_set_error("hgs_loss_head_forward: bg_runs given with bg_views = %d", p->bg_views); return 1; }
+  int* run_counts = (int*)(scratch + head_runs_offset(p));
+  RunMaskJob rm{};
+  if (p->bg_runs && p->tile_used && d_extra_unit && (size_t)p->tiles_x * p->tiles_y <= HEAD_MAX_TILES) {
+    rm.tile_used = p->tile_used; rm.masks = (unsigned int*)(run_counts + 4); rm.counts = run_counts;
+    rm.tiles_x = p->tiles_x; rm.tiles_y = p->tiles_y; rm.W = W; rm.N = N;
+  }
   float* dmaps = scratch;
   float* p_ssim = dmaps + 9 * (size_t)N;
   float* p_pix = p_ssim + 2 * (size_t)nbs;
@@ -1133,8 +1265,9 @@
   int* lists = head_block_lists(p, scratch);
   {
     HgsProfScope _prof(s, HGS_K_SSIM_FWD);
-    hipLaunchKernelGGL(ssim_l1_fwd_kernel, dim3(ssim_grid_size(ssim_grid(3, H, W), SSIM_FWD_WG_PER_XCD)), dim3(256), 0, s, H, W, ssim_grid(3, H, W), win, image,
-                       (const float*)nullptr, targets, dmaps, p_ssim, lists ? head_zero_flags(p, scratch) : nullptr);
+    hipLaunchKernelGGL(ssim_l1_fwd_kernel, dim3(ssim_grid_size(ssim_grid(3, H, W), SSIM_FWD_WG_PER_XCD) + (rm.masks ? 1u : 0u)), dim3(256), 0, s, H, W,
+                       ssim_grid(3, H, W), win, image, (const float*)nullptr, targets, dmaps, p_ssim,
+                       lists ? head_zero_flags(p, scratch) : nullptr, rm);
   }
   HeadFlags fl;
   fl.bce = p->lambda_mask > 0.f; fl.ori = p->lambda_orientation > 0.f;
@@ -1150,7 +1283,8 @@
     hipLaunchKernelGGL(pix_fwd_kernel, dim3(nbp + PIX_SIDE_WGS), dim3(256), 0, s, N, fl, p->bg[0], p->bg[1], p->bg[2], p->min_val, mask_img,
                        omap, targets, p_pix, fl.bce ? p->lambda_mask / (float)N : 0.f, fl.ori ? p->lambda_orientation : 0.f,
                        d_extra_unit, ssim_grid(3, H, W), (const unsigned char*)head_zero_flags(p, scratch), lists, h,
-                       (const float*)p_ssim, p_smooth, out, p->tile_used, p->tiles_x, p->tiles_y, W, 1.f / (float)W);
+                       (const float*)p_ssim, p_smooth, out, p->tile_used, p->tiles_x, p->tiles_y, W, 1.f / (float)W,
+                       (const unsigned int*)rm.masks, p->bg_runs, p->bg_views, hgs_loss_head_num_runs(p), run_counts);
   }
   if (!p->defer_tail) {
     HgsHeadTail t;
diff --git a/hair-gs_amd/csrc/hgs_prologue.h b/hair-gs_amd/csrc/hgs_prologue.h
--- a/hair-gs_amd/csrc/hgs_prologue.h
+++ b/hair-gs_amd/csrc/hgs_prologue.h
@@ -12,6 +12,7 @@
     const uint32_t* src = (const uint32_t*)(p.table + p.view);
     uint32_t* dst = (uint32_t*)p.slot;
     for (int i = threadIdx.x; i < (int)(sizeof(HgsViewTargets) / 4); i += 256) dst[i] = src[i];
+    if (threadIdx.x == 0) dst[sizeof(HgsViewTargets) / 4] = (uint32_t)p.view;
     if (threadIdx.x == 0 && p.lr_dst) *p.lr_dst = p.lr;
     if (p.adam_prep) {
       __syncthreads();
diff --git a/hair-gs_amd/hgs_runtime/__init__.py b/hair-gs_amd/hgs_runtime/__init__.py
--- a/hair-gs_amd/hgs_runtime/__init__.py
+++ b/hair-gs_amd/hgs_runtime/__init__.py
@@ -63,6 +63,9 @@
                                          cf, cf, ci, vp, vp, vp, vp, vp]),
     "hgs_cloud_params_backward": (ci, [vp, ci, vp, vp, vp, vp, vp, vp, vp, vp, vp, vp, vp, vp, vp]),
     "hgs_loss_head_scratch_floats": (sz, [vp]),
+    "hgs_loss_head_num_runs": (ci, [vp]),
+    "hgs_loss_head_background_runs": (ci, [vp, vp, vp, ci, vp]),
+    "hgs_loss_head_run_counts_offset": (sz, [vp]),
     "hgs_loss_head_tail": (ci, [vp, vp, vp, vp]),
     "hgs_loss_head_forward": (ci, [vp, vp, vp, vp, vp, vp, vp, vp, vp, vp, vp, vp]),
     "hgs_loss_head_backward": (ci, [vp, vp, vp, vp, vp, vp, vp, vp, vp, vp, vp, ci, vp, vp, vp, vp]),
@@ -123,7 +126,7 @@
     _fields_ = [("H", ci), ("W", ci), ("lambda_dssim", cf), ("lambda_mask", cf), ("lambda_orientation", cf),
                 ("lambda_smooth", cf), ("bg", cf * 3), ("min_val", cf), ("window", cf * 11), ("n_smooth", ci),
                 ("cos_threshold", cf), ("eps", cf), ("n_endpoints", ci), ("defer_tail", ci), ("tile_used", vp),
-                ("tiles_x", ci), ("tiles_y", ci)]
+                ("tiles_x", ci), ("tiles_y", ci), ("bg_runs", vp), ("bg_views", ci), ("mask_bg", cf)]
 
 
 class HeadTail(C.Structure):
@@ -173,11 +176,12 @@
 PARAMS_HAIR, PARAMS_CLOUD = 1, 2
 HEAD_SKIP_PIXELS, HEAD_SKIP_SMOOTH = 1, 2
 VIEW_QUEUE_MAX = 16
+VIEW_SLOT_BYTES = 192
 HEAD_OUT = ["total", "l1", "dssim", "mask", "orientation", "smooth", "ori_count", "smooth_count", "g_ssim", "g_l1", "g_mask",
             "g_ori", "g_smooth", "total_fwd"]
 HEAD_NOUT = 16
 FUSED_PREPROCESS_MAX_TILES = 8192
-ABI_VERSION = 10
+ABI_VERSION = 11
 
 
 def build(verbose=False):
diff --git a/hair-gs_amd/hgs_runtime/strand_step.py b/hair-gs_amd/hgs_runtime/strand_step.py
--- a/hair-gs_amd/hgs_runtime/strand_step.py
+++ b/hair-gs_amd/hgs_runtime/strand_step.py
@@ -8,7 +8,7 @@
 import hgs_runtime as rt
 from hgs_runtime.fused import gaussian_window11
 
-_SLOT_BYTES = C.sizeof(rt.ViewTargets)
+_SLOT_BYTES = rt.VIEW_SLOT_BYTES
 _F_VIEW, _F_PROJ, _F_CAM = (rt.ViewTargets.viewmatrix.offset // 4, rt.ViewTargets.projmatrix.offset // 4,
                             rt.ViewTargets.campos.offset // 4)
 
@@ -79,6 +79,21 @@
         self.counts_clean = False
         self._fill_behind = False
         self.adam_prep = None
+        self._bg_runs = {}
+
+    def background_runs(self, hp):
+        if not self.has_targets:
+            raise rt.HgsError("background sums need a ViewTable built with the views' targets")
+        key = (hp.H, hp.W, hp.lambda_mask > 0, hp.lambda_orientation > 0, tuple(hp.bg), hp.min_val, hp.mask_bg)
+        t = self._bg_runs.get(key)
+        if t is None:
+            L = rt.lib()
+            t = torch.empty((self.n, L.hgs_loss_head_num_runs(C.byref(hp)), 3), dtype=torch.float32, device=self.device)
+            with torch.cuda.device(self.device):
+                rt.check(L.hgs_loss_head_background_runs(rt.current_stream(), C.byref(hp), self.table.data_ptr(), self.n,
+                                                         t.data_ptr()))
+            self._bg_runs[key] = t
+        return t
 
     def select(self, view, lr=0.0, lr_dst=None):
         if not 0 <= int(view) < self.n:
@@ -251,6 +266,11 @@
         hp.tiles_x, hp.tiles_y = (vt.W + 15) // 16, (vt.H + 15) // 16
     else:
         hp.tile_used = None
+    if step.skip_background_runs and hp.tile_used is not None:
+        runs = vt.background_runs(hp)
+        hp.bg_runs, hp.bg_views = runs.data_ptr(), vt.n
+    else:
+        hp.bg_runs, hp.bg_views = None, 0
     scratch = torch.empty((L.hgs_loss_head_scratch_floats(C.byref(hp)),), **f32)
     out = torch.empty((rt.HEAD_NOUT,), **f32)
     d_extra = torch.empty((4, vt.H, vt.W), **f32) if (step.one_pass_pixels and vt.has_mask) else None
@@ -385,7 +405,7 @@
         ctx.save_for_backward(endpoints, width, pairs, xyz, scale, quat, opacity, extra4, shs, planes, radii, geom, binning,
                               img, scratch, out)
         ctx.pair_grads = pair_grads
-        step.last = {"planes": planes, "radii": radii, "terms": out}
+        step.last = {"planes": planes, "radii": radii, "terms": out, "scratch": scratch}
         terms = out.detach()
         ctx.mark_non_differentiable(terms)
         return out[0], terms
@@ -489,12 +509,15 @@
         self.skip_unread_blocks = bool(getattr(opt, "skip_unread_blocks", True))
         self._tile_maxc_offset = None
         self.poison_unwritten = False
+        self.skip_background_runs = (bool(getattr(opt, "skip_background_runs", True))
+                                     and os.environ.get("HGS_SKIP_BG_RUNS", "1") != "0")
         self.fuse_preprocess = bool(getattr(opt, "fuse_preprocess", True)) and os.environ.get("HGS_FUSE_PREPROCESS", "1") != "0"
         self.fuse_param_backward = bool(getattr(opt, "fuse_param_backward", True)) and os.environ.get("HGS_FUSE_PARAM_BACKWARD", "1") != "0"
         self.inline_adam = None
         self.defer_tail = False
         self.last = {}
         self.refresh()
+        self._prepare_background_runs()
 
     def inline_adam_possible(self):
         from hgs_runtime.fused import FusedAdam
@@ -536,6 +559,16 @@
             if self.ep_pairs is None:
                 self.ep_segments = None
         g._adjacency_cache = (g.endpoint_pairs, self.smooth_pairs, E, self.ep_segments, self.ep_pairs)
+
+    def _prepare_background_runs(self):
+        self.head.mask_bg = 0.0
+        if self.skip_background_runs and self.skip_unread_blocks and self.views.has_mask:
+            self.views.background_runs(self.head)
+
+    def background_run_counts(self):
+        off = rt.lib().hgs_loss_head_run_counts_offset(C.byref(self.head))
+        n = self.last["scratch"][off:off + 2].view(torch.int32).tolist()
+        return n[0], n[1]
 
     def loss(self):
         g = self.gaussians
@@ -604,7 +637,7 @@
         ctx.set_materialize_grads(False)
         ctx.save_for_backward(xyz, scaling_raw, rotation_raw, scale, quat, opacity, extra4, shs, planes, radii, geom, binning,
                               img, scratch, out)
-        step.last = {"planes": planes, "radii": radii, "terms": out}
+        step.last = {"planes": planes, "radii": radii, "terms": out, "scratch": scratch}
         terms = out.detach()
         ctx.mark_non_differentiable(terms)
         return out[0], terms
diff --git a/include/hgs.h b/include/hgs.h
--- a/include/hgs.h
+++ b/include/hgs.h
@@ -8,7 +8,7 @@
 extern "C" {
 #endif
 
-#define HGS_ABI_VERSION 10
+#define HGS_ABI_VERSION 11
 #define HGS_TILE 16
 
 int hgs_abi_version(void);
@@ -98,6 +98,7 @@
   float mask_count;
 } HgsViewTargets;
 size_t hgs_view_targets_bytes(void);
+#define HGS_VIEW_SLOT_BYTES 192
 size_t hgs_head_params_bytes(void);
 size_t hgs_strand_fusion_bytes(void);
 #define HGS_ADAM_MAX_TENSORS 8
@@ -213,11 +214,15 @@
   int n_endpoints;
   int defer_tail;
   const unsigned int* tile_used; int tiles_x, tiles_y;
+  const float* bg_runs; int bg_views; float mask_bg;
 } HgsHeadParams;
 enum { HGS_HEAD_TOTAL = 0, HGS_HEAD_L1, HGS_HEAD_DSSIM, HGS_HEAD_MASK, HGS_HEAD_ORIENTATION, HGS_HEAD_SMOOTH,
        HGS_HEAD_ORI_COUNT, HGS_HEAD_SMOOTH_COUNT, HGS_HEAD_G_SSIM, HGS_HEAD_G_L1, HGS_HEAD_G_MASK, HGS_HEAD_G_ORI,
        HGS_HEAD_G_SMOOTH, HGS_HEAD_TOTAL_FWD, HGS_HEAD_NOUT = 16 };
 size_t hgs_loss_head_scratch_floats(const HgsHeadParams* p);
+int hgs_loss_head_num_runs(const HgsHeadParams* p);
+int hgs_loss_head_background_runs(void* stream, const HgsHeadParams* p, const HgsViewTargets* table, int n_views, float* out);
+size_t hgs_loss_head_run_counts_offset(const HgsHeadParams* p);
 int hgs_loss_head_tail(const HgsHeadParams* p, const float* scratch, float* out, HgsHeadTail* tail);
 int hgs_loss_head_forward(void* stream, const HgsHeadParams* p, const float* image, const float* mask_img,
                           const float* omap, const HgsViewTargets* targets, const float* endpoints,
```

Result: slower. 3786 iters/s (-10.1%).
